# yubster4525/image_compression_2

Measured on AMD Instinct MI355X. Metric: images/sec encode+decode 256px, higher is better.
Workload: dtype f16 (synthesis) / split-bf16 (encoder); 1 GPU; batch=32 256x256 encode+8bit quantize+decode, SG3-T-256 generator; global_batch=32, per_gpu_batch=32, resolution=256, generator=stylegan3-t-256 (random init), encoder=HVAE_VGG_Encoder(img_resolution=1024), quantization_bits=8, parallelism=dp1 (batch-sharded, RCCL metric all_reduce)

## Files before the change

image_compression_2_amd/_native.py:

```python
from __future__ import annotations

import ctypes
import os
import sys
import threading

import torch

_HERE = os.path.dirname(os.path.abspath(__file__))
LIB_PATH = os.path.join(_HERE, "libic2ops.so")
if os.environ.get("IC2_DEV") == "1" and os.environ.get("IC2_DEV_LIB"):
    LIB_PATH = os.environ["IC2_DEV_LIB"]

F32, BF16, F16, BF16X3, F16X2 = 0, 1, 2, 3, 4
F16_IEEE = 5
ACT_LINEAR, ACT_LRELU = 0, 1
NHWC, NCHW, NHWC16 = 0, 1, 2

_P = ctypes.c_void_p
_I = ctypes.c_int
_I64 = ctypes.c_int64
_F = ctypes.c_float

_SIGS = {
    "ic2_abi_version": [],
    "ic2_dev_mode": [],
    "ic2_conv_plan": [_I, _I, _I, _I, _I, _I, _I, _I, _I, _I, _I, _I],
    "ic2_quantize_uniform": [_P, _I64, _I, _P, _P, _P],
    "ic2_quantize_codebook_argmin": [_P, _I64, _P, _I, _P, _P, _P, _P],
    "ic2_codebook_lookup": [_P, _I64, _P, _I, _P, _P, _P],
    "ic2_code_record": [_P, _I, _I, _I, _P, _I64, _P, _P],
    "ic2_gumbel_softmax_quantize": [_P, _I64, _P, _I, _P, _F, _I, ctypes.c_uint64, ctypes.c_uint64, _P, _P, _P, _P,
                                    _P],
    "ic2_gumbel_softmax_quantize_dseed": [_P, _I64, _P, _I, _P, _F, _I, _P, ctypes.c_uint64, _P, _P, _P, _P, _P],
    "ic2_bias_act": [_P, _P, _P, _I, _I64, _I64, _I64, _I, _F, _F, _F, _P],
    "ic2_upfirdn2d": [_P, _P, _I, _I64, _I, _I, _I, _I, _P, _I, _I, _I, _I, _I, _I, _I, _I, _I, _I, _I, _I, _F, _P],
    "ic2_filtered_lrelu": [_P, _P, _I, _I64, _I64, _I, _I, _I, _I, _P, _I, _P, _I, _P, _I, _I, _I, _I, _I, _I, _F, _F,
                           _F, _I, _P],
    "ic2_flrelu_nhwc": [_P, _P, _I, _I, _I, _I, _I, _I, _I, _I, _P, _I, _P, _I, _P, _I, _I, _I, _I, _I, _I, _F, _F, _F,
                        _I, _P, _P],
    "ic2_flrelu_nhwc16": [_P, _P, _I, _I, _I, _I, _I, _I, _I, _I, _P, _I, _P, _I, _P, _I, _I, _I, _I, _I, _I, _F, _F,
                          _F, _I, _P, _P],
    "ic2_fc": [_P, _I64, _P, _P, _P, _I, _I, _I, _F, _F, _I, _F, _F, _P],
    "ic2_pack_weight": [_P, _I, _I, _I, _I, _I, _I, _I, _F, _P, _I, _P, _P],
    "ic2_modconv_prep": [_P, _P, _I, _I, _I, _I, _I, _I, _F, _F, _P, _P, _P, _P],
    "ic2_modconv_prep_batched": [_P, _I64, _I, _I, _I, _P, _P],
    "ic2_conv_igemm": [_P, _P, _P, _I, _I, _I, _I, _I, _I, _I, _I, _I, _I, _I, _I, _I, _P, _P, _I, _F, _F, _F, _F, _I,
                       _P],
    "ic2_conv_igemm_ws_bytes": [_I, _I, _I, _I, _I, _I, _I, _I, _I],
    "ic2_conv_igemm_ws": [_P, _P, _P, _I, _I, _I, _I, _I, _I, _I, _I, _I, _I, _I, _I, _I, _P, _P, _I, _F, _F, _F, _F,
                          _I, _P, _I64, _P],
    "ic2_pack_weight_wino": [_P, _I, _I, _I, _I, _I, _F, _P, _I, _P],
    "ic2_pack_weight_adjoint": [_P, _I, _I, _I, _I, _I, _I, _P, _I, _P],
    "ic2_conv_wino": [_P, _P, _P, _I, _I, _I, _I, _I, _I, _I, _I, _I, _I, _I, _P, _P, _I, _F, _F, _F, _F, _I, _P],
    "ic2_conv_wino_plan": [_I, _I, _I, _I, _I, _I],
    "ic2_conv_wino_preferred": [_I, _I, _I, _I, _I, _I, _I, _I, _I],
    "ic2_conv_wino_stamps": [_P, _I64],
    "ic2_synth_input_features": [_P, _P, _P, _P, _I, _I, _I, _I, _F, _F, _P, _I, _P],
    "ic2_nchw_to_nhwc": [_P, _P, _I, _I, _I, _I, _I, _I, _P, _P],
    "ic2_from_rgb_conv": [_P, _I, _P, _I, _P, _P, _I, _I, _I, _I, _P],
    "ic2_from_rgb_conv_x3": [_P, _I, _P, _I, _P, _P, _I, _I, _I, _I, _P],
    "ic2_from_rgb_conv_f16": [_P, _I, _P, _I, _P, _P, _I, _I, _I, _I, _P],
    "ic2_nhwc_to_nchw": [_P, _I, _P, _I, _I, _I, _I, _I, _P],
    "ic2_group_norm_stats_floats": [_I, _I, _I],
    "ic2_group_norm_stats": [_P, _I, _I, _I, _I, _I, _I, _F, _P, _P],
    "ic2_gn_lrelu_pool": [_P, _P, _I, _I, _I, _I, _I, _I, _I, _I, _P, _P, _P, _F, _I, _P],
    "ic2_global_avg_pool_floats": [_I, _I, _I, _I],
    "ic2_global_avg_pool": [_P, _I, _I, _I, _I, _I, _P, _P],
    "ic2_reparameterize": [_P, _P, _I, _I, _I, _I, _I, _P, _P, _P, _P],
    "ic2_uint8_sse_scratch_doubles": [_I64],
    "ic2_uint8_sse": [_P, _P, _I64, _I64, _P, _P, _P],
    "ic2_resize_bilinear": [_P, _P, _I64, _I, _I, _I, _I, _P],
    "ic2_rc_bound": [_I64, _I64],
    "ic2_rc_encode": [_P, _I64, _I, _I, _I, _P, _I64, _P, _I],
    "ic2_rc_decode": [_P, _P, _I64, _I, _I, _I, _P, _I],
    "ic2_conv_wgrad_ws_floats": [_I, _I, _I, _I, _I, _I, _I, _I],
    "ic2_conv_wgrad": [_P, _P, _P, _I, _I, _I, _I, _I, _I, _I, _I, _I, _P, _I64, _P],
    "ic2_conv_wgrad_oihw": [_P, _P, _P, _I, _I, _I, _I, _I, _I, _I, _I, _I, _I, _I, _P, _I64, _P],
    "ic2_gn_lrelu_pool_bwd_floats": [_I, _I, _I, _I, _I],
    "ic2_gn_lrelu_pool_bwd": [_P, _P, _P, _I, _I, _I, _I, _I, _I, _I, _I, _I, _P, _P, _P, _F, _I, _P, _P, _P, _I64,
                              _P],
    "ic2_gn_lrelu_pool_bwd_db": [_P, _P, _P, _I, _I, _I, _I, _I, _I, _I, _I, _I, _P, _P, _P, _F, _I, _P, _P, _P, _P,
                                 _I64, _P],
    "ic2_gap_bwd": [_P, _P, _I, _I, _I, _I, _I, _P],
    "ic2_flrelu_bwd_ydot_floats": [_I, _I, _I, _I, _I],
    "ic2_flrelu_bwd_nhwc_ex": [_P, _I, _P, _I, _P, _I, _I, _I, _I, _I, _I, _I, _P, _I, _P, _I, _I, _I, _I, _I, _I, _I,
                               _F, _F, _F, _I, _P, _P, _P, _I64, _P],
    "ic2_scale_bwd_part_floats": [_I, _I, _I],
    "ic2_colsum_div": [_P, _I, _I, _I, _P, _P, _P],
    "ic2_scale_bwd_nhwc": [_P, _P, _P, _P, _I, _I, _I, _I, _P, _I64, _P],
    "ic2_scale_nhwc": [_P, _P, _P, _I, _I, _I, _I, _P],
    "ic2_conv3x3_gn_stats_floats": [_I, _I, _I, _I, _I, _I, _I, _I, _I, _I],
    "ic2_conv3x3_gn_fwd": [_P, _P, _P, _I, _I, _I, _I, _I, _I, _I, _I, _I, _I, _P, _I, _F, _P, _I64, _P, _I64, _I,
                           _P],
    "ic2_conv3x3_gn_fwd_scaled": [_P, _P, _P, _I, _I, _I, _I, _I, _I, _I, _I, _I, _I, _P, _F, _I, _F, _P, _I64, _P,
                                  _I64, _I, _P],
    "ic2_conv3x3_gnin_supported": [_I, _I, _I, _I, _I, _I, _I, _I, _I],
    "ic2_conv3x3_gn_fuses": [_I, _I, _I, _I, _I, _I, _I, _I, _I, _I, _I, _I],
    "ic2_gn_affine_table": [_P, _P, _P, _I, _I, _I, _I, _P, _P],
    "ic2_conv3x3_gnin_gn_fwd": [_P, _P, _F, _P, _P, _I, _I, _I, _I, _I, _I, _I, _I, _I, _I, _P, _I, _F, _P, _I64, _P,
                                _I64, _I, _P],
    "ic2_flrelu_bwd_nhwc": [_P, _I, _P, _I, _P, _I, _I, _I, _I, _I, _I, _P, _I, _P, _I, _I, _I, _I, _I, _I, _I, _F, _F,
                            _F, _I, _P],
}
_RESTYPE = {"ic2_conv_plan": ctypes.c_char_p, "ic2_conv_wino_plan": ctypes.c_char_p, "ic2_conv_igemm_ws_bytes": _I64, "ic2_group_norm_stats_floats": _I64, "ic2_global_avg_pool_floats": _I64,
            "ic2_uint8_sse_scratch_doubles": _I64, "ic2_rc_bound": _I64, "ic2_conv_wgrad_ws_floats": _I64,
            "ic2_gn_lrelu_pool_bwd_floats": _I64, "ic2_conv3x3_gn_stats_floats": _I64,
            "ic2_flrelu_bwd_ydot_floats": _I64, "ic2_scale_bwd_part_floats": _I64}

_lib = None
_lock = threading.Lock()


class NativeUnavailable(RuntimeError):
    pass


def load():
    global _lib
    if _lib is not None:
        return _lib
    with _lock:
        if _lib is not None:
            return _lib
        if not os.path.exists(LIB_PATH):
            raise NativeUnavailable(
                f"{LIB_PATH} is missing: build it with `python -m image_compression_2_amd.build_native` "
                "(there is no CPU fallback for the product path)")
        lib = ctypes.CDLL(LIB_PATH)
        lib.ic2_last_error.restype = ctypes.c_char_p
        lib.ic2_last_error.argtypes = []
        for name, args in _SIGS.items():
            fn = getattr(lib, name)
            fn.argtypes = args
            fn.restype = _RESTYPE.get(name, _I)
        _lib = lib
    return _lib


def exported_symbols():
    return ["ic2_last_error"] + list(_SIGS)


def call(name, *args):
    lib = load()
    rc = getattr(lib, name)(*args)
    if rc != 0:
        msg = lib.ic2_last_error().decode(errors="replace")
        raise RuntimeError(f"{name} failed (code {rc}): {msg}")
    return rc


def query(name, *args):
    return getattr(load(), name)(*args)


def conv_plan(dtype, out_dtype, out_layout, n, h, w, cin_p, cout_p, cout_valid, kh, kw, pad):
    return query("ic2_conv_plan", dtype, out_dtype, out_layout, n, h, w, cin_p, cout_p, cout_valid, kh, kw,
                 pad).decode()


def conv_igemm(x, w, y, dtype, out_dtype, n, h, w_, cin_p, cout_p, cout_valid, kh, kw, pad, ho, wo, oscale, bias,
               act, slope, act_gain, clamp, out_mul, out_layout, stream, device):
    nbytes = int(query("ic2_conv_igemm_ws_bytes", dtype, n, h, w_, cin_p, cout_p, kh, kw, pad))
    ws = torch.empty([max(nbytes, 16) // 4], dtype=torch.float32, device=device) if nbytes > 0 else None
    return call("ic2_conv_igemm_ws", x, w, y, dtype, out_dtype, n, h, w_, cin_p, cout_p, cout_valid, kh, kw, pad, ho,
                wo, oscale, bias, act, slope, act_gain, clamp, out_mul, out_layout, ptr(ws), nbytes, stream)


def wino_preferred(dtype, n, h, w, cin_p, cout_p, kh, kw, pad):
    return bool(query("ic2_conv_wino_preferred", dtype, n, h, w, cin_p, cout_p, kh, kw, pad))


def wino_plan(n, h, w, cin_p, cout_p, pad):
    return query("ic2_conv_wino_plan", n, h, w, cin_p, cout_p, pad).decode()


def conv_wino(x, u, y, dtype, out_dtype, n, h, w_, cin_p, cout_p, cout_valid, pad, ho, wo, oscale, bias, act, slope,
              act_gain, clamp, out_mul, out_layout, stream):
    return call("ic2_conv_wino", x, u, y, dtype, out_dtype, n, h, w_, cin_p, cout_p, cout_valid, pad, ho, wo, oscale,
                bias, act, slope, act_gain, clamp, out_mul, out_layout, stream)


_flops_hook = None


def note_flops(alg_flops):
    if _flops_hook is not None:
        _flops_hook(alg_flops)


def knob(name, default):
    v = os.environ.get(name)
    if os.environ.get("IC2_DEV") != "1":
        if v is not None:
            print(f"[ic2] {name}={v} ignored: development knobs need IC2_DEV=1", file=sys.stderr)
        return default
    return default if v is None else type(default)(v)


def require_gpu(*tensors):
    for t in tensors:
        if t is None:
            continue
        if not t.is_cuda:
            raise RuntimeError("image_compression_2_amd runs on ROCm devices only (got a CPU tensor); "
                               "the CPU restatement lives in oracle/ and is test infrastructure")
        if not t.is_contiguous():
            raise RuntimeError("expected a contiguous tensor")


class AutogradUnsupported(RuntimeError):
    pass


def grad_inputs(tensors=(), modules=()):
    if not torch.is_grad_enabled():
        return []
    req = [t for t in tensors if isinstance(t, torch.Tensor) and t.requires_grad]
    return req + [p for m in modules for p in m.parameters() if p.requires_grad]


class _RefuseBackward(torch.autograd.Function):

    @staticmethod
    def forward(ctx, what, n_out, *args):
        ctx.what = what
        return tuple(a.detach() for a in args[:n_out])

    @staticmethod
    def backward(ctx, *grads):
        raise AutogradUnsupported(
            f"{ctx.what}: backward through the HIP path is not implemented for this module (training, SURVEY.md "
            "8(f) #3; the reference trains only the encoder, through a frozen generator).  Freeze the module with "
            ".requires_grad_(False) or detach its inputs")


def refuse_backward(what, outputs, tensors=(), modules=()):
    req = grad_inputs(tensors, modules)
    if not req:
        return outputs
    single = isinstance(outputs, torch.Tensor)
    outs = [outputs] if single else list(outputs)
    fl = [i for i, o in enumerate(outs) if isinstance(o, torch.Tensor) and o.is_floating_point()]
# ... 64 lines not shown
```

image_compression_2_amd/csrc/conv_common.h:

```cpp
#pragma once
#include "common.h"

namespace ic2 {

typedef __attribute__((ext_vector_type(8))) __bf16 bf16x8;
typedef __attribute__((ext_vector_type(8))) _Float16 f16x8;
typedef __attribute__((ext_vector_type(4))) float f32x4;

template <bool F16>
__device__ __forceinline__ f32x4 mfma32(bf16x8 a, bf16x8 b, f32x4 c) {
  if constexpr (F16)
    return __builtin_amdgcn_mfma_f32_16x16x32_f16(__builtin_bit_cast(f16x8, a), __builtin_bit_cast(f16x8, b), c, 0, 0, 0);
  else
    return __builtin_amdgcn_mfma_f32_16x16x32_bf16(a, b, c, 0, 0, 0);
}
__host__ __device__ inline bool is16(int dtype) { return dtype == IC2_BF16 || dtype == IC2_F16; }

struct IgemmArgs {
  const void* x;
  const void* w;
  void* y;
  const float* oscale;
  const float* bias;
  float* ws;
  int n, h, w_, cin_p, cout_p, cout_valid, kh, kw, pad, ho, wo;
  int M;
  int K;
  int nq;
  int tiles_o;
  int nblocks;
  int group;
  int korder;
  int o_base;
  int tile_base;
  int act;
  float slope, act_gain, clamp, out_mul;
  int out_layout, out_dtype;
  double* gn_part;
  int gn_groups, gn_c;
  const float* in_gn;
  float in_slope;
  int x_pix, x_hb32;
  int wx_twp, wx_th, wx_ns, wx_hp, wx_nh, wx_tx, wx_ty;
  int out_ieee;
};
__device__ __forceinline__ int ig_xb32(const IgemmArgs& a, int b) { return b >= a.x_hb32 ? b - a.x_hb32 : b; }

__device__ __forceinline__ float4 ig_load_oscale(const IgemmArgs& a, int nn, int ob) {
  return a.oscale && ob < a.cout_p ? *reinterpret_cast<const float4*>(a.oscale + (int64_t)nn * a.cout_p + ob)
                                   : make_float4(1.f, 1.f, 1.f, 1.f);
}
__device__ __forceinline__ float4 ig_load_bias(const IgemmArgs& a, int ob) {
  return a.bias && ob < a.cout_p ? *reinterpret_cast<const float4*>(a.bias + ob) : make_float4(0.f, 0.f, 0.f, 0.f);
}
__device__ __forceinline__ void ig_preloads_done() { __builtin_amdgcn_s_waitcnt(0x0F70); }

__device__ __forceinline__ void ig_store4v(const IgemmArgs& a, int p, int nn, int pix, int ob, const float (&acc)[4],
                                           float4 sc, float4 bi, float (*vout)[4] = nullptr) {
  const float scv[4] = {sc.x, sc.y, sc.z, sc.w}, biv[4] = {bi.x, bi.y, bi.z, bi.w};
  float v[4];
#pragma unroll
  for (int r = 0; r < 4; ++r) {
    float t = acc[r] * scv[r] + biv[r];
    if (a.act) t = lrelu_gain_clamp(t, a.slope, a.act_gain, a.clamp);
    v[r] = t * a.out_mul;
  }
  if (vout != nullptr) {
#pragma unroll
    for (int r = 0; r < 4; ++r) (*vout)[r] = v[r];
  }
  if (a.out_layout != IC2_LAYOUT_NCHW) {
    const int64_t e = a.out_layout == IC2_LAYOUT_NHWC
                          ? (int64_t)p * a.cout_p + ob
                          : (((int64_t)nn * (a.cout_p >> 4) + (ob >> 4)) * ((int64_t)a.ho * a.wo) + pix) * 16 + (ob & 15);
    if (a.out_dtype == IC2_BF16) {
      uint2 pk;
      pk.x = (uint32_t)f2bf(v[0]) | ((uint32_t)f2bf(v[1]) << 16);
      pk.y = (uint32_t)f2bf(v[2]) | ((uint32_t)f2bf(v[3]) << 16);
      *reinterpret_cast<uint2*>(reinterpret_cast<bf16_t*>(a.y) + e) = pk;
    } else if (a.out_dtype == IC2_F16) {
      typedef _Float16 h2 __attribute__((ext_vector_type(2)));
      float s_[4];
#pragma unroll
      for (int r = 0; r < 4; ++r) s_[r] = a.out_ieee ? v[r] : __builtin_amdgcn_fmed3f(v[r], -65504.f, 65504.f);
      const h2 q0 = h2{(_Float16)s_[0], (_Float16)s_[1]}, q1 = h2{(_Float16)s_[2], (_Float16)s_[3]};
      if (vout != nullptr) {
        (*vout)[0] = (float)q0.x; (*vout)[1] = (float)q0.y; (*vout)[2] = (float)q1.x; (*vout)[3] = (float)q1.y;
      }
      uint2 pk;
      pk.x = __builtin_bit_cast(uint32_t, q0);
      pk.y = __builtin_bit_cast(uint32_t, q1);
      *reinterpret_cast<uint2*>(reinterpret_cast<uint16_t*>(a.y) + e) = pk;
    } else {
      *reinterpret_cast<float4*>(reinterpret_cast<float*>(a.y) + e) = make_float4(v[0], v[1], v[2], v[3]);
    }
  } else {
    float* yo = reinterpret_cast<float*>(a.y);
    const int hw = a.ho * a.wo;
#pragma unroll
    for (int r = 0; r < 4; ++r)
      if (ob + r < a.cout_valid) yo[((int64_t)nn * a.cout_valid + ob + r) * hw + pix] = v[r];
  }
}
__device__ __forceinline__ void ig_store4(const IgemmArgs& a, int p, int nn, int pix, int ob, const float (&acc)[4]) {
  ig_store4v(a, p, nn, pix, ob, acc, ig_load_oscale(a, nn, ob), ig_load_bias(a, ob));
}

__device__ __forceinline__ int xcd_remap(int b, int nblocks) {
  const int xcd = b & 7, loc = b >> 3;
  const int q8 = nblocks >> 3, r8 = nblocks & 7;
  return (xcd < r8 ? xcd * (q8 + 1) : r8 * (q8 + 1) + (xcd - r8) * q8) + loc;
}

constexpr uint32_t kOob = 0x7ffffff0u;
constexpr int kRsrcWord3 = 0x00020000;

}
```

image_compression_2_amd/csrc/flrelu.h:

```cpp
#pragma once
#include "common.h"

namespace ic2 {

struct FlrArgs {
  const void* x;
  void* y;
  const float* bias;
  const float* post_scale;
  int64_t xsn, xsy, xsx, xsc;
  int64_t xcb;
  int64_t ysn, ysy, ysx, ysc;
  int c, c_p;
  int in_h, in_w, out_h, out_w;
  int py0, px0;
  int tiles_x, tiles_y, cblocks, nimg;
  int order;
  int out_f16;
  float slope, lim;
  float gdg[12];
  float gu[24];
  float gd[12];
  float guh[24];
  float gdgl[12];
};

void f16_round_taps(const float* exact, float* out, int n, int stride_groups);

int flrelu_mfma_launch(FlrArgs a, int in_f16, int up, int down, int tu, int td, int delta, int n, hipStream_t s);

}
```

image_compression_2_amd/csrc/flrelu.hip:

```cpp
#include "flrelu.h"

#include <cmath>

#include <cstdlib>
#include <type_traits>

namespace ic2 {

typedef float f2v __attribute__((ext_vector_type(2)));

template <int U, int D, int TU, int TD, int TOY, int TOX>
struct FlrGeom {
  static constexpr int RAY = (TOY - 1) * D + TD;
  static constexpr int RAX = (TOX - 1) * D + TD;
  static constexpr int NINY = (RAY + TU - 2) / U + 1;
  static constexpr int NINX = (RAX + TU - 2) / U + 1;
  static constexpr int NINXP = NINX | 1;
};

template <typename T, bool CHLAST>
__device__ __forceinline__ f2v load2(const T* p, int64_t sc, bool ok, bool ok2);
template <> __device__ __forceinline__ f2v load2<float, true>(const float* p, int64_t, bool ok, bool) {
  const float2 v = *reinterpret_cast<const float2*>(ok ? (const void*)p : zero_line());
  return f2v{v.x, v.y};
// ... 201 lines not shown
  return 2;
}

template <typename TI, typename TO, bool CHLAST, int U, int D, int TU, int TD, int DL>
static int launch_geom(const FlrArgs& a, int geom, int grid, hipStream_t s) {
#define IC2_FLR_LAUNCH(TY, TX, CPB, NT)                                                                            \
  hipLaunchKernelGGL((flrelu_kernel<TI, TO, CHLAST, U, D, TU, TD, DL, TY, TX, CPB, NT>), dim3(grid), dim3(NT), 0, s, a)
  constexpr bool tuned = CHLAST && std::is_same<TI, bf16_t>::value;
  if constexpr (tuned) {
    switch (geom) {
      case 1: IC2_FLR_LAUNCH(16, 8, 16, 256); return IC2_OK;
      case 2: IC2_FLR_LAUNCH(16, 16, 16, 256); return IC2_OK;
      case 3: IC2_FLR_LAUNCH(8, 16, 16, 256); return IC2_OK;
      case 4: IC2_FLR_LAUNCH(12, 16, 16, 256); return IC2_OK;
      case 5: IC2_FLR_LAUNCH(16, 16, 8, 128); return IC2_OK;
      default: break;
    }
  }
  if (geom != 0) return IC2_E_UNSUPPORTED;
  IC2_FLR_LAUNCH(24, 8, 16, 256);
  return IC2_OK;
#undef IC2_FLR_LAUNCH
}

template <typename TI, typename TO, bool CHLAST, int U, int D, int TU, int TD>
static int launch_delta(const FlrArgs& a, int delta, int geom, int grid, hipStream_t s) {
  switch (delta) {
    case 0: return launch_geom<TI, TO, CHLAST, U, D, TU, TD, 0>(a, geom, grid, s);
    case 1: return launch_geom<TI, TO, CHLAST, U, D, TU, TD, 1>(a, geom, grid, s);
    case 2: if constexpr (U > 2) return launch_geom<TI, TO, CHLAST, U, D, TU, TD, 2>(a, geom, grid, s); break;
    case 3: if constexpr (U > 3) return launch_geom<TI, TO, CHLAST, U, D, TU, TD, 3>(a, geom, grid, s); break;
  }
  return IC2_E_UNSUPPORTED;
}

template <typename TI, typename TO, bool CHLAST>
static int launch_cfg(const FlrArgs& a, int up, int down, int tu, int td, int delta, int geom, int grid,
                      hipStream_t s) {
  if (up == 2 && down == 2 && tu == 12 && td == 12)
    return launch_delta<TI, TO, CHLAST, 2, 2, 12, 12>(a, delta, geom, grid, s);
  if (up == 4 && down == 2 && tu == 24 && td == 12)
    return launch_delta<TI, TO, CHLAST, 4, 2, 24, 12>(a, delta, geom, grid, s);
  return IC2_E_UNSUPPORTED;
}

static float f16_nearest(float v) { return (float)(_Float16)v; }
static float f16_step(float r, bool up) {
  uint16_t b = __builtin_bit_cast(uint16_t, (_Float16)r);
  const bool neg = b & 0x8000u;
  if ((b & 0x7fffu) == 0) return up ? 5.96046448e-8f : -5.96046448e-8f;
  b = (up != neg) ? b + 1 : b - 1;
  return (float)__builtin_bit_cast(_Float16, b);
}
void f16_round_taps(const float* exact, float* out, int n, int stride_groups) {
  for (int t = 0; t < n; ++t) out[t] = f16_nearest(exact[t]);
  for (int g = 0; g < stride_groups; ++g) {
    for (int it = 0; it < n; ++it) {
      double e = 0.0;
      for (int t = g; t < n; t += stride_groups) e += (double)out[t] - (double)exact[t];
      double best = std::fabs(e);
      int bi = -1;
      float bc = 0.f;
      for (int t = g; t < n; t += stride_groups) {
        if (exact[t] == 0.f) continue;
        for (int dir = 0; dir < 2; ++dir) {
          const float c = f16_step(out[t], dir == 0);
          if (((double)c - exact[t]) * ((double)out[t] - exact[t]) > 0.0) continue;
          const double e2 = std::fabs(e - (double)out[t] + (double)c);
          if (e2 < best) { best = e2; bi = t; bc = c; }
        }
      }
      if (bi < 0) break;
      out[bi] = bc;
    }
  }
}

static int flrelu_common(const void* x, void* y, int dtype_in, int dtype_out, bool chlast, int n, int c, int c_p,
                         int in_h, int in_w, int out_h, int out_w, const float* fu, int fu_taps, const float* fd,
                         int fd_taps, const float* b, int up, int down, int px0, int px1, int py0, int py1,
                         float gain, float slope, float clamp, int flip, const float* post_scale, void* stream,
                         const char* name, bool in_blocked = false) {
  IC2_CHECK_ARG(x && y, "%s: null pointer", name);
  IC2_CHECK_ARG(n > 0 && c > 0 && in_h > 0 && in_w > 0 && up >= 1 && down >= 1, "%s: bad geometry", name);
  IC2_CHECK_ARG(fu_taps >= 1 && fd_taps >= 1 && fu_taps <= 24 && fd_taps <= 12, "%s: unsupported taps", name);
  const int ew = (in_w * up + (px0 + px1) - (fu_taps - 1) - (fd_taps - 1) + (down - 1)) / down;
  const int eh = (in_h * up + (py0 + py1) - (fu_taps - 1) - (fd_taps - 1) + (down - 1)) / down;
  IC2_CHECK_ARG(out_h == eh && out_w == ew, "%s: output %dx%d, expected %dx%d", name, out_h, out_w, eh, ew);
  IC2_CHECK_ARG(out_h > 0 && out_w > 0, "%s: empty output", name);
  const int dx = ((px0 % up) + up) % up, dy = ((py0 % up) + up) % up;
  if (dx != dy) {
    set_error("%s: px0 and py0 differ mod up", name);
    return IC2_E_UNSUPPORTED;
  }
  if (!(slope >= 0.f && slope <= 1.f && gain > 0.f)) {
    set_error("%s: fused path needs 0 <= slope <= 1 and gain > 0", name);
    return IC2_E_UNSUPPORTED;
  }
  FlrArgs a;
  a.x = x; a.y = y; a.bias = b; a.post_scale = post_scale;
  a.xcb = 16;
  if (in_blocked) {
    a.xsc = 1; a.xsx = 16; a.xsy = (int64_t)in_w * 16; a.xsn = (int64_t)in_h * in_w * c_p;
    a.xcb = (int64_t)in_h * in_w * 16;
    a.ysc = 1; a.ysx = c_p; a.ysy = (int64_t)out_w * c_p; a.ysn = (int64_t)out_h * out_w * c_p;
  } else if (chlast) {
    a.xsc = 1; a.xsx = c_p; a.xsy = (int64_t)in_w * c_p; a.xsn = (int64_t)in_h * in_w * c_p;
    a.ysc = 1; a.ysx = c_p; a.ysy = (int64_t)out_w * c_p; a.ysn = (int64_t)out_h * out_w * c_p;
  } else {
    a.xsx = 1; a.xsy = in_w; a.xsc = (int64_t)in_h * in_w; a.xsn = (int64_t)c * in_h * in_w;
    a.ysx = 1; a.ysy = out_w; a.ysc = (int64_t)out_h * out_w; a.ysn = (int64_t)c * out_h * out_w;
  }
  a.c = chlast ? c_p : c;
  a.c_p = c_p;
  a.in_h = in_h; a.in_w = in_w; a.out_h = out_h; a.out_w = out_w;
  a.py0 = py0; a.px0 = px0;
  hipStream_t s = as_stream(stream);
  static const bool use_mfma = knob("IC2_FLR_MFMA", 1) != 0;
  const bool mfma_ok = chlast && (dtype_in == IC2_BF16 || dtype_in == IC2_F16) &&
                       (dtype_out == IC2_BF16 || dtype_out == IC2_F16) && b == nullptr && dx == dy;
  a.out_f16 = dtype_out == IC2_F16;
  if ((use_mfma || dtype_in == IC2_F16) && mfma_ok) {
    float gu[24] = {}, gd[12] = {}, gdg[12] = {};
    for (int t = 0; t < fu_taps; ++t) gu[t] = (fu ? (flip ? fu[t] : fu[fu_taps - 1 - t]) : 1.f) * (float)up;
    for (int t = 0; t < fd_taps; ++t) gd[t] = fd ? (flip ? fd[t] : fd[fd_taps - 1 - t]) : 1.f;
    for (int t = 0; t < fd_taps; ++t) gdg[t] = gd[t] * gain;
    for (int t = 0; t < 24; ++t) a.gu[t] = 0.f;
    for (int t = 0; t < 12; ++t) a.gd[t] = a.gdg[t] = 0.f;
    f16_round_taps(gu, a.gu, fu_taps, up);
    f16_round_taps(gd, a.gd, fd_taps, 1);
    f16_round_taps(gdg, a.gdg, fd_taps, 1);
    a.slope = slope;
    a.lim = clamp >= 0.f ? clamp / gain : INFINITY;
    for (int t = 0; t < 24; ++t) a.guh[t] = 0.f;
    for (int t = 0; t < 12; ++t) a.gdgl[t] = 0.f;
    if (clamp >= 0.f) {
      float guh[24] = {}, gdgl[12] = {};
      for (int t = 0; t < fu_taps; ++t) guh[t] = gu[t] / a.lim;
      for (int t = 0; t < fd_taps; ++t) gdgl[t] = gdg[t] * a.lim;
      f16_round_taps(guh, a.guh, fu_taps, up);
      f16_round_taps(gdgl, a.gdgl, fd_taps, 1);
    }
    if (flrelu_mfma_launch(a, dtype_in == IC2_F16, up, down, fu_taps, fd_taps, dx, n, s) == IC2_OK) {
      IC2_CHECK_LAUNCH(name);
      return IC2_OK;
    }
  }
  if (in_blocked) {
    set_error("%s: channel-blocked input needs the MFMA instance (f16/bf16 in, bf16/f16 out, no bias, up 2/4 with 6*up "
              "taps, down 2 / 12 taps)", name);
    return IC2_E_UNSUPPORTED;
  }
  if (dtype_in == IC2_F16) {
    set_error("%s: f16 input needs the MFMA instance (NHWC, bf16/f16 out, no bias, up 2/4 with 6*up taps, down 2 / 12 taps)",
              name);
    return IC2_E_UNSUPPORTED;
  }
  const int geom = flr_pick(chlast && dtype_in == IC2_BF16 && dtype_out == IC2_BF16, up);
  const FlrGeomSel fv = kFlrGeoms[geom];
  a.tiles_x = (int)ceil_div(out_w, fv.tox);
  a.tiles_y = (int)ceil_div(out_h, fv.toy);
  a.cblocks = (int)ceil_div(a.c, fv.cpb);
  a.nimg = n;
  a.slope = slope;
  a.lim = clamp >= 0.f ? clamp / gain : INFINITY;
  for (int t = 0; t < 24; ++t) a.gu[t] = 0.f;
  for (int t = 0; t < 12; ++t) a.gd[t] = 0.f;
  for (int t = 0; t < fu_taps; ++t) a.gu[t] = (fu ? (flip ? fu[t] : fu[fu_taps - 1 - t]) : 1.f) * (float)up;
  for (int t = 0; t < fd_taps; ++t) a.gd[t] = fd ? (flip ? fd[t] : fd[fd_taps - 1 - t]) : 1.f;
  for (int t = 0; t < 12; ++t) a.gdg[t] = a.gd[t] * gain;
  const int64_t grid = (int64_t)n * a.tiles_y * a.tiles_x * a.cblocks;
  IC2_CHECK_ARG(grid < (1LL << 31), "%s: grid too large", name);
  int rc;
  if (dtype_in == IC2_BF16 && dtype_out == IC2_BF16)
    rc = chlast ? launch_cfg<bf16_t, bf16_t, true>(a, up, down, fu_taps, fd_taps, dx, geom, (int)grid, s)
                : launch_cfg<bf16_t, bf16_t, false>(a, up, down, fu_taps, fd_taps, dx, geom, (int)grid, s);
  else if (dtype_in == IC2_F32 && dtype_out == IC2_F32)
    rc = chlast ? launch_cfg<float, float, true>(a, up, down, fu_taps, fd_taps, dx, geom, (int)grid, s)
                : launch_cfg<float, float, false>(a, up, down, fu_taps, fd_taps, dx, geom, (int)grid, s);
  else {
    set_error("%s: unsupported dtype pair %d -> %d", name, dtype_in, dtype_out);
    return IC2_E_INVALID;
  }
  if (rc != IC2_OK) {
    set_error("%s: no fused instance for up=%d down=%d taps=%d/%d", name, up, down, fu_taps, fd_taps);
    return rc;
  }
  IC2_CHECK_LAUNCH(name);
  return IC2_OK;
}

}

using namespace ic2;

extern "C" int ic2_filtered_lrelu(const void* x, void* y, int dtype, int64_t n, int64_t c, int in_h, int in_w,
                                  int out_h, int out_w, const float* fu, int fu_taps, const float* fd, int fd_taps,
                                  const float* b, int up, int down, int px0, int px1, int py0, int py1, float gain,
                                  float slope, float clamp, int flip, void* stream) {
  IC2_CHECK_ARG(n < (1 << 30) && c < (1 << 30), "filtered_lrelu: sizes too large");
  return flrelu_common(x, y, dtype, dtype, false, (int)n, (int)c, (int)c, in_h, in_w, out_h, out_w, fu, fu_taps, fd,
                       fd_taps, b, up, down, px0, px1, py0, py1, gain, slope, clamp, flip, nullptr, stream,
                       "filtered_lrelu");
}

extern "C" int ic2_flrelu_nhwc(const void* x, void* y, int dtype_in, int dtype_out, int n, int c_p, int in_h,
                               int in_w, int out_h, int out_w, const float* fu, int fu_taps, const float* fd,
                               int fd_taps, const float* b, int up, int down, int px0, int px1, int py0, int py1,
                               float gain, float slope, float clamp, int flip, const float* post_scale,
                               void* stream) {
  IC2_CHECK_ARG(c_p % 16 == 0, "flrelu_nhwc: c_p must be a multiple of 16");
  return flrelu_common(x, y, dtype_in, dtype_out, true, n, c_p, c_p, in_h, in_w, out_h, out_w, fu, fu_taps, fd,
                       fd_taps, b, up, down, px0, px1, py0, py1, gain, slope, clamp, flip, post_scale, stream,
                       "flrelu_nhwc");
}

extern "C" int ic2_flrelu_nhwc16(const void* x, void* y, int dtype_in, int dtype_out, int n, int c_p, int in_h,
                                 int in_w, int out_h, int out_w, const float* fu, int fu_taps, const float* fd,
                                 int fd_taps, const float* b, int up, int down, int px0, int px1, int py0, int py1,
                                 float gain, float slope, float clamp, int flip, const float* post_scale,
                                 void* stream) {
  IC2_CHECK_ARG(c_p % 16 == 0, "flrelu_nhwc16: c_p must be a multiple of 16");
  IC2_CHECK_ARG(dtype_in == IC2_F16 || dtype_in == IC2_BF16, "flrelu_nhwc16: f16 or bf16 input");
  return flrelu_common(x, y, dtype_in, dtype_out, true, n, c_p, c_p, in_h, in_w, out_h, out_w, fu, fu_taps, fd,
                       fd_taps, b, up, down, px0, px1, py0, py1, gain, slope, clamp, flip, post_scale, stream,
                       "flrelu_nhwc16", true);
}
```

image_compression_2_amd/csrc/flrelu_mfma.h:

```cpp
#pragma once
#include "flrelu.h"

namespace ic2 {

typedef _Float16 fm_h2 __attribute__((ext_vector_type(2)));
typedef _Float16 fm_h4 __attribute__((ext_vector_type(4)));
typedef _Float16 fm_h8 __attribute__((ext_vector_type(8)));
typedef short fm_s4 __attribute__((ext_vector_type(4)));
typedef float fm_f4 __attribute__((ext_vector_type(4)));
typedef float fm_f2 __attribute__((ext_vector_type(2)));
typedef uint32_t v2u32_t __attribute__((ext_vector_type(2)));

constexpr int FM_TAPS = 276;
constexpr int FM_TAPS_CL = 476;
constexpr uint32_t FM_OOB = 0x7ffffff0u;


__device__ __forceinline__ fm_s4 fm_tr_read(const uint32_t* p) {
  return __builtin_amdgcn_ds_read_tr16_b64_v4i16((__attribute__((address_space(3))) fm_s4*)p);
}

__device__ __forceinline__ void fm_dma16(__amdgpu_buffer_rsrc_t rs, uint32_t voff, const uint32_t* lds_dst) {
  const uint32_t m0 = __builtin_amdgcn_readfirstlane(
      (uint32_t)(uintptr_t)(__attribute__((address_space(3))) const uint32_t*)lds_dst);
  asm volatile("s_nop 4\n\tbuffer_load_dwordx4 %0, %1, 0 offen lds" ::"v"(voff), "s"(rs), "{m0}"(m0) : "memory");
}

__device__ __forceinline__ uint32_t fm_h2u(float a, float b) {
  return __builtin_bit_cast(uint32_t, fm_h2{(_Float16)a, (_Float16)b});
}
__device__ __forceinline__ uint2 fm_pack4(float a, float b, float c, float d) {
  return make_uint2(fm_h2u(a, b), fm_h2u(c, d));
}
__device__ __forceinline__ fm_h4 fm_h4_of(uint2 u) { return __builtin_bit_cast(fm_h4, u); }
__device__ __forceinline__ fm_h8 fm_h8_of(uint2 lo, uint2 hi) {
  return __builtin_bit_cast(fm_h8, make_uint4(lo.x, lo.y, hi.x, hi.y));
}

__device__ __forceinline__ int fm_xcd_remap(int b, int nblocks) {
  const int xcd = b & 7, loc = b >> 3;
  const int q8 = nblocks >> 3, r8 = nblocks & 7;
  return (xcd < r8 ? xcd * (q8 + 1) : r8 * (q8 + 1) + (xcd - r8) * q8) + loc;
}

inline int fm_strip_segments(int64_t nstrips, int tiles_y, int resident, bool tune) {
  int64_t nseg = (2 * (int64_t)resident + nstrips - 1) / nstrips;
  nseg = nseg < 1 ? 1 : (nseg > tiles_y ? tiles_y : nseg);
  if (tune && tiles_y <= 40) {
    int64_t best = -1, pick = nseg;
    for (int64_t sg = nseg; sg <= tiles_y && sg <= nseg + 16; ++sg) {
      const int64_t len = (tiles_y + sg - 1) / sg, segs = (tiles_y + len - 1) / len;
      const int64_t cost = (nstrips * segs + resident - 1) / resident * (len + 1);
      if (best < 0 || cost < best) best = cost, pick = segs;
    }
    nseg = pick;
  }
  return (int)nseg;
}

}
```

image_compression_2_amd/csrc/flrelu_mfma.hip:

```cpp
#include "flrelu_mfma.h"

#include <algorithm>
#include <cstdlib>
#include <type_traits>

namespace ic2 {

template <int U>
struct FmGeom {
  static constexpr int TU = 6 * U, TD = 12;
  static constexpr int TO = 16;
  static constexpr int RA = (TO - 1) * 2 + TD;
  static constexpr int NIN = (RA + TU - 2) / U + 1;
  static constexpr int NB = (RA + 15) / 16;
  static constexpr int IN_PITCH = NIN * 8;
  static constexpr int IN_DW = (NIN * NIN * 2 + 63) / 64 * 256;
  static constexpr int V_PITCH = NIN * 8 + 2;
  static constexpr int V_DW = 16 * V_PITCH;
  static constexpr int D_XP = 10;
  static constexpr int D_PITCH = 16 * D_XP + 8;
  static constexpr int D_DW = 16 * D_PITCH;
  static constexpr int LDS_DW = IN_DW + V_DW + D_DW + FM_TAPS;
  static constexpr int VD_DW = V_DW > D_DW ? V_DW : D_DW;
  static constexpr int LDS_DW_ALIAS = IN_DW + VD_DW + FM_TAPS;
// ... 569 lines not shown
          for (int tt = 0; tt < NBX; ++tt) {
            uint2 p, m;
            if constexpr (ABL & 2) { p = make_uint2(fm_h2u(u[tt][0], u[tt][1]), fm_h2u(u[tt][2], u[tt][3])); m = p; }
            else fm_act_split(fm_h2u(u[tt][0], u[tt][1]), fm_h2u(u[tt][2], u[tt][3]), nslope2, p, m);
            q[tt] = fm_h8_of(p, m);
          }
          __builtin_amdgcn_sched_barrier(0);
#pragma unroll
          for (int bi = 0; bi < 3; ++bi)
#pragma unroll
            for (int ob = 0; ob < NOB; ++ob)
              d[ob] = __builtin_amdgcn_mfma_f32_16x16x32_f16(q[2 * ob + bi], gdq[bi],
                                                             bi == 0 ? fm_f4{0.f, 0.f, 0.f, 0.f} : d[ob], 0, 0, 0);
        } else {
          uint2 au[NBX];
#pragma unroll
          for (int tt = 0; tt < NBX; ++tt)
            au[tt] = fm_act_h4(fm_h2u(u[tt][0], u[tt][1]), fm_h2u(u[tt][2], u[tt][3]), slope2, nlim2, lim2);
          __builtin_amdgcn_sched_barrier(0);
#pragma unroll
          for (int ob = 0; ob < NOB; ++ob)
            d[ob] = __builtin_amdgcn_mfma_f32_16x16x32_f16(fm_h8_of(au[2 * ob], au[2 * ob + 1]), gdh01,
                                                           fm_f4{0.f, 0.f, 0.f, 0.f}, 0, 0, 0);
#pragma unroll
          for (int ob = 0; ob < NOB; ++ob)
            d[ob] = __builtin_amdgcn_mfma_f32_16x16x32_f16(fm_h8_of(au[2 * ob + 2], make_uint2(0u, 0u)), gdh2, d[ob],
                                                           0, 0, 0);
        }
        __builtin_amdgcn_sched_barrier(0);
#pragma unroll
        for (int ob = 0; ob < NOB; ++ob)
          *reinterpret_cast<uint2*>(d_img + row * G::D_PITCH + (16 * ob + li) * G::D_XP + 2 * g) =
              fm_pack4(d[ob][0], d[ob][1], d[ob][2], d[ob][3]);
      }
      if constexpr (!(ABL & 1)) __syncthreads();
      if constexpr (!(ABL & 32)) {
        fm_s4 da[OCW];
#pragma unroll
        for (int i = 0; i < OCW; ++i)
          da[i] = fm_tr_read(d_img + (4 * g + tq) * G::D_PITCH + (wave + NW * i) * G::D_XP + 2 * tp);
        __builtin_amdgcn_sched_barrier(0);
#pragma unroll
        for (int i = 0; i < OCW; ++i)
          acc[i] = __builtin_amdgcn_mfma_f32_16x16x16f16(__builtin_bit_cast(fm_h4, da[i]), gdv[b], acc[i], 0, 0, 0);
        __builtin_amdgcn_sched_barrier(0);
      }
    }

    const float ps[4] = {psv.x, psv.y, psv.z, psv.w};
    const __amdgpu_buffer_rsrc_t ors = __builtin_amdgcn_make_buffer_rsrc(
        (void*)(yout + (int64_t)n * a.out_h * a.out_w * a.c_p + c0), 0, FM_OOB, 0x00020000);
    const int gy = oy0 + li;
#pragma unroll
    for (int i = 0; i < OCW; ++i) {
      const int gx = ox0 + wave + NW * i;
      uint32_t off = (gy < a.out_h && gx < a.out_w) ? (uint32_t)(((gy * a.out_w + gx) * a.c_p + 4 * g) * 2) : FM_OOB;
      if constexpr ((ABL & 64) != 0)
        off = (gy < a.out_h && gx < a.out_w)
                  ? (uint32_t)((((c0 >> 4) * a.out_h + gy) * a.out_w + gx) * 32 + 8 * g) - (uint32_t)(c0 * 2)
                  : FM_OOB;
      const uint2 v = fm_out4(a.out_f16, acc[i][0] * ps[0], acc[i][1] * ps[1], acc[i][2] * ps[2], acc[i][3] * ps[3]);
      if constexpr (!(ABL & 8))
        __builtin_amdgcn_raw_buffer_store_b64(__builtin_bit_cast(v2u32_t, v), ors, off, 0, 0);
    }
  }
}

template <int U>
struct FmGeom3 {
  using G2 = FmGeom2<U, 32>;
  static constexpr int NINX = G2::NINX;
  static constexpr int S = 16 / U;
  static constexpr int NG = U + 1;
  static constexpr int IN_PITCH = NINX * 8;
  static constexpr int GCH = S * NINX * 2;
  static constexpr int NGI = (GCH + 63) / 64;
  static constexpr int GRP_DW = NGI * 256;
  static constexpr int RING_DW = NG * GRP_DW;
  static constexpr int LDS_DW = RING_DW + G2::V_DW + G2::DT_DW + 16;
  static_assert(U * S == 16 && NINX % 2 == 1, "geometry");
  static_assert((NG - 1) * GRP_DW + (S - 1) * IN_PITCH + 8 * 8 * ((NINX + 7) / 8) <= RING_DW, "ring bounds");
};

#ifndef IC2_FM3_ABL
#define IC2_FM3_ABL 0
#endif
#ifndef FM3_EARLY
#define FM3_EARLY 1
#endif
#ifndef FM3_DEFER_ST
#define FM3_DEFER_ST 0
#endif
template <int U, int DELTA, int NW, bool CL>
__global__ void __launch_bounds__(64 * NW, 32 / NW) flrelu_mfma3_kernel(FlrArgs a, int nitems, int nseg, int seg_len) {
  constexpr int TOX = 32, NT = 64 * NW, RR = 16 / NW, OCW = TOX / NW;
  using G2 = FmGeom2<U, TOX>;
  using G = FmGeom3<U>;
  constexpr int NINX = G::NINX, NBX = G2::NBX, NOB = G2::NOB, S = G::S, NG = G::NG;
  __shared__ __attribute__((aligned(16))) uint32_t lds[G::LDS_DW];
  uint32_t* const ring = lds;
  uint32_t* const v_img = lds + G::RING_DW;
  uint32_t* const d_img = v_img + G2::V_DW;
  float* const taps = reinterpret_cast<float*>(d_img);
  uint32_t* const ps_lds = d_img + G2::DT_DW;

  const int tid = threadIdx.x;
  const int lane = tid & 63;
  const int wave = __builtin_amdgcn_readfirstlane(tid >> 6);
  const int g = lane >> 4, li = lane & 15;
  const int tq = li >> 2, tp = li & 3;
  const int qoff = (4 * g + tq) / S, roff = (4 * g + tq) % S;

  for (int i = tid; i < FM_TAPS_CL; i += NT) {
    float v = 0.f;
    if (i >= 48 && i < 72) v = a.gu[i - 48];
    else if (i >= 148 && i < 160) v = a.gd[i - 148];
    else if (i >= 228 && i < 240) v = a.gdg[i - 228];
    else if (i >= 328 && i < 352) v = a.guh[i - 328];
    else if (i >= 428 && i < 440) v = a.gdgl[i - 428];
    taps[i] = v;
  }

  const int slot = fm_xcd_remap(blockIdx.x, gridDim.x);
  const uint16_t* xin = reinterpret_cast<const uint16_t*>(a.x);
  auto item_geom = [&](int w, int& n, int& ox0, int& c0, int& t0, int& nt) {
    const int cb = w % a.cblocks;
    w /= a.cblocks;
    const int seg = w % nseg;
    w /= nseg;
    const int tx = w % a.tiles_x;
    n = w / a.tiles_x;
    ox0 = tx * TOX;
    c0 = cb * 16;
    t0 = seg * seg_len;
    nt = min(seg_len, a.tiles_y - t0);
  };
  const int xsy = (int)a.xsy, xsx = (int)a.xsx;
  const int my_dma = wave < G::NGI ? (G::NGI - 1 - wave) / NW + 1 : 0;
  static_assert((G::NGI + NW - 1) / NW <= 2, "ring group DMA per wave");
  auto load_group = [&](int n, int iy0, int sx0, int c0, int q) __attribute__((always_inline)) {
    const __amdgpu_buffer_rsrc_t rs = __builtin_amdgcn_make_buffer_rsrc(
        (void*)(xin + n * a.xsn + (c0 >> 4) * a.xcb), 0, FM_OOB, 0x00020000);
    uint32_t* const dst = ring + (q % NG) * G::GRP_DW;
    int ln = lane;
    asm volatile("" : "+v"(ln));
#pragma unroll
    for (int i = 0; i < (G::NGI + NW - 1) / NW; ++i) {
      const int k = wave + NW * i;
      if (k < G::NGI) {
        const int e = k * 64 + ln;
        const int pix = e >> 1;
        const int row = pix / NINX, x = pix - row * NINX;
        const int iy = iy0 + q * S + row, ix = sx0 + x;
        const bool ok = e < G::GCH && (unsigned)iy < (unsigned)a.in_h && (unsigned)ix < (unsigned)a.in_w;
        const uint32_t off = ok ? (uint32_t)((iy * xsy + ix * xsx + (e & 1) * 8) * 2) : FM_OOB;
        fm_dma16(rs, off, dst + k * 256);
      }
    }
  };
  auto load_item = [&](int w) __attribute__((always_inline)) {
    int n, ox0, c0, t0, nt;
    item_geom(w, n, ox0, c0, t0, nt);
    const int iy0 = (32 * t0 + DELTA - a.py0) / U, sx0 = (ox0 * 2 - a.px0 + DELTA) / U;
#pragma unroll
    for (int q = 0; q < NG; ++q) load_group(n, iy0, sx0, c0, q);
    if (a.post_scale != nullptr && wave == NW - 1 && lane < 4) {
      const __amdgpu_buffer_rsrc_t prs = __builtin_amdgcn_make_buffer_rsrc(
          (void*)(a.post_scale + (int64_t)n * a.c_p + c0), 0, 64, 0x00020000);
      fm_dma16(prs, lane * 16, ps_lds);
    }
  };
  if (slot < nitems) load_item(slot);
  __syncthreads();

  fm_h4 gmy, gmx[NBX];
  {
    float v[4];
#pragma unroll
    for (int j = 0; j < 4; ++j) v[j] = taps[48 + U * (4 * g + j) + DELTA - li];
    gmy = fm_h4_of(fm_pack4(v[0], v[1], v[2], v[3]));
  }
#pragma unroll
  for (int t = 0; t < NBX; ++t) {
    const int w0 = fm_win<U, DELTA, NINX>(16 * t);
    float v[4];
#pragma unroll
    for (int j = 0; j < 4; ++j) v[j] = taps[(CL ? 328 : 48) + U * (w0 + 4 * g + j) + DELTA - (16 * t + li)];
    gmx[t] = fm_h4_of(fm_pack4(v[0], v[1], v[2], v[3]));
  }
  fm_h8 gdh01, gdh2, gdq[3];
  {
    auto tap = [&](int blk, int j) { return taps[(CL ? 428 : 228) + 16 * blk + 4 * g + j - 2 * li]; };
    float v[8];
#pragma unroll
    for (int j = 0; j < 4; ++j) {
      v[j] = tap(0, j);
      v[4 + j] = tap(1, j);
    }
    gdh01 = fm_h8_of(fm_pack4(v[0], v[1], v[2], v[3]), fm_pack4(v[4], v[5], v[6], v[7]));
#pragma unroll
    for (int j = 0; j < 4; ++j) {
      v[j] = tap(2, j);
      v[4 + j] = 0.f;
    }
    gdh2 = fm_h8_of(fm_pack4(v[0], v[1], v[2], v[3]), fm_pack4(v[4], v[5], v[6], v[7]));
#pragma unroll
    for (int bi = 0; bi < 3; ++bi) {
#pragma unroll
      for (int j = 0; j < 4; ++j) {
        v[j] = tap(bi, j);
        v[4 + j] = -tap(bi, j);
      }
      gdq[bi] = fm_h8_of(fm_pack4(v[0], v[1], v[2], v[3]), fm_pack4(v[4], v[5], v[6], v[7]));
    }
  }
  fm_h4 gdv[3];
#pragma unroll
  for (int b = 0; b < 3; ++b) {
    float v[4];
#pragma unroll
    for (int j = 0; j < 4; ++j) v[j] = taps[148 + 16 * b + 4 * g + j - 2 * li];
    gdv[b] = fm_h4_of(fm_pack4(v[0], v[1], v[2], v[3]));
  }
  const float slope = a.slope, lim = CL ? 1.f : a.lim;
  const uint32_t slope2 = fm_h2u(slope, slope), lim2 = fm_h2u(lim, lim), nlim2 = fm_h2u(-lim, -lim);
  const uint32_t nslope2 = fm_h2u(-slope, -slope);
  bf16_t* yout = reinterpret_cast<bf16_t*>(a.y);
  __syncthreads();

  bool first = true;
  for (int w = slot; w < nitems; w += gridDim.x) {
    int n, ox0, c0, t0, nt;
    item_geom(w, n, ox0, c0, t0, nt);
    const int iy0 = (32 * t0 + DELTA - a.py0) / U, sx0 = (ox0 * 2 - a.px0 + DELTA) / U;
    const bool has_next = w + (int)gridDim.x < nitems;
    if (first) asm volatile("s_waitcnt vmcnt(0)" ::: "memory");
    else asm volatile("s_waitcnt vmcnt(%0)" ::"n"(OCW) : "memory");
    first = false;
    __syncthreads();
    float4 psv = make_float4(1.f, 1.f, 1.f, 1.f);
    if (a.post_scale) psv = *reinterpret_cast<const float4*>(ps_lds + 4 * g);
    const float ps[4] = {psv.x, psv.y, psv.z, psv.w};
    const __amdgpu_buffer_rsrc_t ors = __builtin_amdgcn_make_buffer_rsrc(
        (void*)(yout + (int64_t)n * a.out_h * a.out_w * a.c_p + c0), 0, FM_OOB, 0x00020000);
    const int kend = 2 * nt;

    fm_f4 acc_a[OCW], acc_b[OCW];
    auto store_tile = [&](int tt) __attribute__((always_inline)) {
      const int gy = 16 * (t0 + tt) + li;
#pragma unroll
      for (int i = 0; i < OCW; ++i) {
        const int gx = ox0 + wave + NW * i;
        const uint32_t off =
            (gy < a.out_h && gx < a.out_w) ? (uint32_t)(((gy * a.out_w + gx) * a.c_p + 4 * g) * 2) : FM_OOB;
        const uint2 v = fm_out4(a.out_f16, acc_a[i][0] * ps[0], acc_a[i][1] * ps[1], acc_a[i][2] * ps[2], acc_a[i][3] * ps[3]);
        __builtin_amdgcn_raw_buffer_store_b64(__builtin_bit_cast(v2u32_t, v), ors, (IC2_FM3_ABL & 64) ? FM_OOB : off, 0, 0);
      }
    };
    auto block = [&](int k, auto mode_c) __attribute__((always_inline)) {
      constexpr int MODE = decltype(mode_c)::value;
      if constexpr (!(IC2_FM3_ABL & 8)) {
        constexpr int NC = (NINX + NW - 1) / NW;
        const int q = k + qoff;
        const uint32_t* rowp = ring + (q % NG) * G::GRP_DW + roff * G::IN_PITCH + 2 * tp + wave * 8;
        fm_s4 xa[NC];
        fm_f4 vt[NC];
#pragma unroll
        for (int i = 0; i < NC; ++i) xa[i] = fm_tr_read(rowp + i * NW * 8);
        __builtin_amdgcn_sched_barrier(0);
#pragma unroll
        for (int i = 0; i < NC; ++i)
          vt[i] = __builtin_amdgcn_mfma_f32_16x16x16f16(__builtin_bit_cast(fm_h4, xa[i]), gmy,
                                                        fm_f4{0.f, 0.f, 0.f, 0.f}, 0, 0, 0);
        __builtin_amdgcn_sched_barrier(0);
        uint32_t* const vp = v_img + li * G2::V_PITCH + 2 * g + wave * 8;
#pragma unroll
        for (int i = 0; i < NC; ++i)
          if (i < NC - 1 || wave + NW * i < NINX)
            *reinterpret_cast<uint2*>(vp + i * NW * 8) = fm_pack4(vt[i][0], vt[i][1], vt[i][2], vt[i][3]);
      }
      if constexpr (!(IC2_FM3_ABL & 32)) __syncthreads();
      if (k == kend && has_next) load_item(w + gridDim.x);
      const bool dma = !(IC2_FM3_ABL & 2) && k + 2 <= kend;
      if (FM3_EARLY && dma) load_group(n, iy0, sx0, c0, k + U + 1);
      if constexpr (FM3_DEFER_ST && MODE == 1) {
        if (k >= 3) store_tile((k - 3) >> 1);
      }
#pragma unroll
      for (int rr = 0; rr < ((IC2_FM3_ABL & 4) ? 0 : RR); ++rr) {
        const int row = wave + NW * rr;
        fm_s4 vb[NBX];
#pragma unroll
        for (int tt = 0; tt < NBX; ++tt) {
          const int w0 = fm_win<U, DELTA, NINX>(16 * tt);
          vb[tt] = fm_tr_read(v_img + row * G2::V_PITCH + (w0 + 4 * g + tq) * 8 + 2 * tp);
        }
        __builtin_amdgcn_sched_barrier(0);
        fm_f4 u[NBX];
#pragma unroll
        for (int tt = 0; tt < NBX; ++tt)
          u[tt] = __builtin_amdgcn_mfma_f32_16x16x16f16(gmx[tt], __builtin_bit_cast(fm_h4, vb[tt]),
                                                        fm_f4{0.f, 0.f, 0.f, 0.f}, 0, 0, 0);
        __builtin_amdgcn_sched_barrier(0);
        fm_f4 d[NOB];
        if constexpr (CL) {
          fm_h8 qv[NBX];
#pragma unroll
          for (int tt = 0; tt < NBX; ++tt) {
            uint2 p, m;
            fm_act_split(fm_h2u(u[tt][0], u[tt][1]), fm_h2u(u[tt][2], u[tt][3]), nslope2, p, m);
            qv[tt] = fm_h8_of(p, m);
          }
          __builtin_amdgcn_sched_barrier(0);
#pragma unroll
          for (int bi = 0; bi < 3; ++bi)
#pragma unroll
            for (int ob = 0; ob < NOB; ++ob)
              d[ob] = __builtin_amdgcn_mfma_f32_16x16x32_f16(qv[2 * ob + bi], gdq[bi],
                                                             bi == 0 ? fm_f4{0.f, 0.f, 0.f, 0.f} : d[ob], 0, 0, 0);
        } else {
          uint2 au[NBX];
#pragma unroll
          for (int tt = 0; tt < NBX; ++tt)
            au[tt] = fm_act_h4(fm_h2u(u[tt][0], u[tt][1]), fm_h2u(u[tt][2], u[tt][3]), slope2, nlim2, lim2);
          __builtin_amdgcn_sched_barrier(0);
#pragma unroll
          for (int ob = 0; ob < NOB; ++ob)
            d[ob] = __builtin_amdgcn_mfma_f32_16x16x32_f16(fm_h8_of(au[2 * ob], au[2 * ob + 1]), gdh01,
                                                           fm_f4{0.f, 0.f, 0.f, 0.f}, 0, 0, 0);
#pragma unroll
          for (int ob = 0; ob < NOB; ++ob)
            d[ob] = __builtin_amdgcn_mfma_f32_16x16x32_f16(fm_h8_of(au[2 * ob + 2], make_uint2(0u, 0u)), gdh2, d[ob],
                                                           0, 0, 0);
        }
        __builtin_amdgcn_sched_barrier(0);
#pragma unroll
        for (int ob = 0; ob < NOB; ++ob)
          *reinterpret_cast<uint2*>(d_img + row * G2::D_PITCH + (16 * ob + li) * G2::D_XP + 2 * g) =
              fm_pack4(d[ob][0], d[ob][1], d[ob][2], d[ob][3]);
      }
      if (!(IC2_FM3_ABL & 1) && k >= 1 && k < kend) {
        const bool st = (MODE == 1 && k >= 3) || (FM3_DEFER_ST && MODE == 2 && k >= 4);
        const int nd = FM3_EARLY && dma ? my_dma : 0;
        if (nd == 0) {
          if (st) asm volatile("s_waitcnt vmcnt(%0)" ::"n"(OCW) : "memory");
          else asm volatile("s_waitcnt vmcnt(0)" ::: "memory");
        } else if (nd == 1) {
          if (st) asm volatile("s_waitcnt vmcnt(%0)" ::"n"(OCW + 1) : "memory");
          else asm volatile("s_waitcnt vmcnt(1)" ::: "memory");
        } else {
          if (st) asm volatile("s_waitcnt vmcnt(%0)" ::"n"(OCW + 2) : "memory");
          else asm volatile("s_waitcnt vmcnt(2)" ::: "memory");
        }
      }
      if constexpr (!(IC2_FM3_ABL & 32)) __syncthreads();
      if (!FM3_EARLY && dma) load_group(n, iy0, sx0, c0, k + U + 1);
      if constexpr (!(IC2_FM3_ABL & 16)) {
        fm_s4 da[OCW];
#pragma unroll
        for (int i = 0; i < OCW; ++i)
          da[i] = fm_tr_read(d_img + (4 * g + tq) * G2::D_PITCH + (wave + NW * i) * G2::D_XP + 2 * tp);
        __builtin_amdgcn_sched_barrier(0);
        if constexpr (MODE == 0) {
#pragma unroll
          for (int i = 0; i < OCW; ++i)
            acc_b[i] = __builtin_amdgcn_mfma_f32_16x16x16f16(__builtin_bit_cast(fm_h4, da[i]), gdv[0],
                                                             fm_f4{0.f, 0.f, 0.f, 0.f}, 0, 0, 0);
        } else if constexpr (MODE == 1) {
#pragma unroll
          for (int i = 0; i < OCW; ++i)
            acc_a[i] = __builtin_amdgcn_mfma_f32_16x16x16f16(__builtin_bit_cast(fm_h4, da[i]), gdv[1], acc_b[i], 0, 0, 0);
        } else {
#pragma unroll
          for (int i = 0; i < OCW; ++i)
            acc_a[i] = __builtin_amdgcn_mfma_f32_16x16x16f16(__builtin_bit_cast(fm_h4, da[i]), gdv[2], acc_a[i], 0, 0, 0);
          if (k < kend) {
#pragma unroll
            for (int i = 0; i < OCW; ++i)
              acc_b[i] = __builtin_amdgcn_mfma_f32_16x16x16f16(__builtin_bit_cast(fm_h4, da[i]), gdv[0],
                                                               fm_f4{0.f, 0.f, 0.f, 0.f}, 0, 0, 0);
          }
        }
        __builtin_amdgcn_sched_barrier(0);
      }
    };

    block(0, std::integral_constant<int, 0>{});
    for (int t = 0; t < nt; ++t) {
      block(2 * t + 1, std::integral_constant<int, 1>{});
      block(2 * t + 2, std::integral_constant<int, 2>{});
      if (!FM3_DEFER_ST || t == nt - 1) store_tile(t);
    }
  }
}

template <int U, int DELTA, bool CL>
static void fm3_launch_cl(FlrArgs a, int n, hipStream_t s) {
  constexpr int TOX = 32, NW = 8;
  a.tiles_x = (int)ceil_div(a.out_w, TOX);
  a.tiles_y = (int)ceil_div(a.out_h, 16);
  a.cblocks = a.c_p / 16;
  static int resident = 0;
  if (resident == 0) {
    int dev = 0, cus = 0, per_cu = 0;
    (void)hipGetDevice(&dev);
    (void)hipDeviceGetAttribute(&cus, hipDeviceAttributeMultiprocessorCount, dev);
    (void)hipOccupancyMaxActiveBlocksPerMultiprocessor(&per_cu, flrelu_mfma3_kernel<U, DELTA, NW, CL>, 64 * NW, 0);
    resident = (cus > 0 ? cus : 256) * (per_cu > 0 ? per_cu : 1);
  }
  static const int segs_mode = knob("IC2_FLR_SEGS", 1);
  const int64_t nstrips = (int64_t)n * a.tiles_x * a.cblocks;
  int nseg = fm_strip_segments(nstrips, a.tiles_y, resident, segs_mode == 1);
  const int seg_len = (int)ceil_div(a.tiles_y, nseg);
  nseg = (int)ceil_div(a.tiles_y, seg_len);
  const int nitems = (int)(nstrips * nseg);
  const int grid = nitems < resident ? nitems : resident;
  hipLaunchKernelGGL((flrelu_mfma3_kernel<U, DELTA, NW, CL>), dim3((unsigned)grid), dim3(64 * NW), 0, s, a, nitems,
                     nseg, seg_len);
}

template <int U, int DELTA, bool CL, int ABL>
static void fm2_launch_cl(FlrArgs a, int n, hipStream_t s) {
  constexpr int TOX = 32, NW = 8;
  a.tiles_x = (int)ceil_div(a.out_w, TOX);
  a.tiles_y = (int)ceil_div(a.out_h, 16);
  a.cblocks = a.c_p / 16;
  static const int order = knob("IC2_FLR_ORDER", 0);
  a.order = order;
  const int ntiles = n * a.tiles_y * a.tiles_x * a.cblocks;
  static int resident = 0;
  if (resident == 0) {
    int dev = 0, cus = 0, per_cu = 0;
    (void)hipGetDevice(&dev);
    (void)hipDeviceGetAttribute(&cus, hipDeviceAttributeMultiprocessorCount, dev);
    (void)hipOccupancyMaxActiveBlocksPerMultiprocessor(&per_cu, flrelu_mfma2_kernel<U, DELTA, TOX, NW, CL, ABL>, 64 * NW, 0);
    resident = (cus > 0 ? cus : 256) * (per_cu > 0 ? per_cu : 1);
  }
  const int grid = ntiles < resident ? ntiles : resident;
  hipLaunchKernelGGL((flrelu_mfma2_kernel<U, DELTA, TOX, NW, CL, ABL>), dim3((unsigned)grid), dim3(64 * NW), 0, s, a, ntiles);
}

template <int U, int DELTA>
static void fm2_launch(FlrArgs a, int n, hipStream_t s) {
  static const bool split = knob("IC2_FLR_CLSPLIT", 1) != 0;
  static const bool strip = knob("IC2_FLR_STRIP", 1) != 0;
  const bool cl = split && a.lim >= 0.0625f && a.lim <= 4096.f;
  if (strip) {
    if (cl) fm3_launch_cl<U, DELTA, true>(a, n, s);
    else fm3_launch_cl<U, DELTA, false>(a, n, s);
  } else if (cl) {
    fm2_launch_cl<U, DELTA, true, 0>(a, n, s);
  } else {
    fm2_launch_cl<U, DELTA, false, 0>(a, n, s);
  }
}

template <int U, int DELTA, bool IN_F16, bool ALIAS, int NW>
static void fm_launch_alias(const FlrArgs& a, int ntiles, hipStream_t s) {
  static int resident = 0;
  if (resident == 0) {
    int dev = 0, cus = 0, per_cu = 0;
    (void)hipGetDevice(&dev);
    (void)hipDeviceGetAttribute(&cus, hipDeviceAttributeMultiprocessorCount, dev);
    (void)hipOccupancyMaxActiveBlocksPerMultiprocessor(&per_cu, flrelu_mfma_kernel<U, DELTA, IN_F16, ALIAS, NW>, 64 * NW,
                                                       0);
    resident = (cus > 0 ? cus : 256) * (per_cu > 0 ? per_cu : 1);
  }
  const int grid = ntiles < resident ? ntiles : resident;
  hipLaunchKernelGGL((flrelu_mfma_kernel<U, DELTA, IN_F16, ALIAS, NW>), dim3((unsigned)grid), dim3(64 * NW), 0, s, a,
                     ntiles);
}

template <int U, int DELTA, bool IN_F16>
static void fm_launch_one(const FlrArgs& a, int ntiles, hipStream_t s) {
  fm_launch_alias<U, DELTA, IN_F16, false, 4>(a, ntiles, s);
}

template <bool IN_F16>
static void fm_launch(const FlrArgs& a, int up, int delta, int ntiles, hipStream_t s) {
  if (up == 2) {
    if (delta == 0) fm_launch_one<2, 0, IN_F16>(a, ntiles, s);
    else fm_launch_one<2, 1, IN_F16>(a, ntiles, s);
  } else {
    switch (delta) {
      case 0: fm_launch_one<4, 0, IN_F16>(a, ntiles, s); break;
      case 1: fm_launch_one<4, 1, IN_F16>(a, ntiles, s); break;
      case 2: fm_launch_one<4, 2, IN_F16>(a, ntiles, s); break;
      default: fm_launch_one<4, 3, IN_F16>(a, ntiles, s); break;
    }
  }
}

int flrelu_mfma_launch(FlrArgs a, int in_f16, int up, int down, int tu, int td, int delta, int n, hipStream_t s) {
  if (down != 2 || td != 12 || tu != 6 * up || (up != 2 && up != 4) || a.bias != nullptr || a.c_p % 16 != 0)
    return IC2_E_UNSUPPORTED;
  if ((int64_t)a.in_h * a.in_w * a.c_p * 2 >= (int64_t)FM_OOB) return IC2_E_UNSUPPORTED;
  if (a.xsc != 1 || a.xsx % 8 != 0) return IC2_E_UNSUPPORTED;
  if ((int64_t)a.out_h * a.out_w * a.c_p * 2 >= (int64_t)FM_OOB) return IC2_E_UNSUPPORTED;
  static const bool wide = knob("IC2_FLR_WIDE", 1) != 0;
  static const bool wide_all = knob("IC2_FLR_WIDE_ALL", 1) != 0;
  if (in_f16 && wide && (wide_all || ceil_div(a.out_w, 32) * 32 <= ceil_div(a.out_w, 16) * 16) &&
      (int64_t)n * ceil_div(a.out_h, 16) * ceil_div(a.out_w, 32) * (a.c_p / 16) < (1LL << 31)) {
    if (up == 2) {
      if (delta == 0) fm2_launch<2, 0>(a, n, s);
      else fm2_launch<2, 1>(a, n, s);
    } else {
      switch (delta) {
        case 0: fm2_launch<4, 0>(a, n, s); break;
        case 1: fm2_launch<4, 1>(a, n, s); break;
        case 2: fm2_launch<4, 2>(a, n, s); break;
        default: fm2_launch<4, 3>(a, n, s); break;
      }
    }
    return IC2_OK;
  }
  a.tiles_x = (int)ceil_div(a.out_w, 16);
  a.tiles_y = (int)ceil_div(a.out_h, 16);
  a.cblocks = a.c_p / 16;
  const int64_t grid = (int64_t)n * a.tiles_y * a.tiles_x * a.cblocks;
  if (grid >= (1LL << 31)) return IC2_E_UNSUPPORTED;
  if (in_f16) fm_launch<true>(a, up, delta, (int)grid, s);
  else fm_launch<false>(a, up, delta, (int)grid, s);
  return IC2_OK;
}

}
```

image_compression_2_amd/csrc/igemm.hip:

```cpp
#include "conv_common.h"

#include <cstdlib>

namespace ic2 {

template <bool BF16, int BO, int BP, int WGO, int WGP, int NSTAGE>
struct IgCfg {
  static constexpr int NW = WGO * WGP;
  static constexpr int ESZ = BF16 ? 2 : 4;
  static constexpr int EPC = 16 / ESZ;
  static constexpr int ROWB = 32 * ESZ;
  static constexpr int WB = BO * ROWB, XB = BP * ROWB;
  static constexpr int NIW_T = WB / 1024, NIX_T = XB / 1024;
  static constexpr int NIW = (NIW_T + NW - 1) / NW, NIX = (NIX_T + NW - 1) / NW;
  static constexpr int PER = NIW + NIX;
  static constexpr int TO = BO / WGO, TP = BP / WGP;
  static constexpr int I = TO / 16, J = TP / 16;
  static constexpr int STAGEB = WB + XB;
  __device__ static __forceinline__ int swz(int row) { return BF16 ? ((row >> 1) & 3) : ((row >> 1) & 7); }
  __device__ static __forceinline__ int off(int row, int ch) { return row * ROWB + ((ch ^ swz(row)) << 4); }
};

template <int I, int J>
__device__ __forceinline__ void ig_epilogue(const IgemmArgs& a, const f32x4 (&acc)[I][J], int obase, int pbase, int fr,
// ... 471 lines not shown
                      int ntiles = -1) {
  a.o_base = o_base;
  a.tiles_o = ((o_end < 0 ? a.cout_p : o_end) - o_base + G8<OG>::BO - 1) / G8<OG>::BO;
  a.nq = a.K / 64;
  a.nblocks = (int)(ceil_div(a.M, G8<OG>::BP) * a.tiles_o);
  a.tile_base = tile_base;
  const unsigned grid = (unsigned)(ntiles < 0 ? a.nblocks - tile_base : ntiles);
  if constexpr (OG == 2)
    hipLaunchKernelGGL(F16 ? igemm8_og2_f16_kernel : igemm8_og2_kernel, dim3(grid, splits), dim3(512), 0, s, a);
  else
    hipLaunchKernelGGL(F16 ? igemm8_og1_f16_kernel : igemm8_og1_kernel, dim3(grid, splits), dim3(512), 0, s, a);
}

template <int I, int J, int WGO, int WGP, int TW, int NS, bool HB = false>
struct H4 {
  static constexpr int BO = 16 * I * WGO, BP = 16 * J * WGP, TH = BP / TW;
  static constexpr int HW = TW + 2, HH = TH + 2, NH = HH * HW;
  static constexpr int NHI = (NH + 15) / 16;
  static constexpr int HPW = (NHI + 3) / 4;
  static constexpr int HALO_B = NHI * 1024;
  static constexpr int WS_B = BO * 64;
  static constexpr int NWI = (BO / 16 + 3) / 4;
  static constexpr int LDS_B = NS * WS_B + 2 * HALO_B + (HB ? 1024 : 0);
  static_assert(BP % TW == 0 && TW % 16 == 0, "pixel tile");
  static_assert((BO / 16) % 4 == 0 || BO == 96, "weight slab rows over the 4 waves");
  static_assert(HB || HPW <= 8, "halo DMA spread over the first 8 taps");
  static_assert(LDS_B <= 80 * 1024, "two workgroups per CU");
};
__device__ __forceinline__ int h4_off(int row, int chunk) { return row * 64 + ((chunk ^ (((row >> 2) & 1) << 1)) << 4); }

#ifndef IC2_HG4_ABL
#define IC2_HG4_ABL 0
#endif
#ifndef IC2_HG4_PAIR
#define IC2_HG4_PAIR 1
#endif

template <int I, int J, int WGO, int WGP, int TW, int NS, bool HB = false, bool F16 = false, int TPB = 1,
          bool GN = false, bool PAIR = false>
__device__ __forceinline__ void hg4_body(const IgemmArgs& a, int tiles_x, int tiles_y) {
  using G = H4<I, J, WGO, WGP, TW, NS, HB>;
  static_assert(!PAIR || (TPB == 2 && HB), "PAIR: two taps per barrier step with the halo burst");
  static_assert((G::BO / 16) % 4 == 0 || (TPB == 2 && NS == 4), "uneven weight DMAs need the L = 1 multi-tap loop");
  constexpr int LA = NS - 1;
  constexpr int NWI = G::NWI, HPW = G::HPW;
  __shared__ __attribute__((aligned(16))) char lds[G::LDS_B];
  char* const wsl = lds;
  char* const hal = lds + NS * G::WS_B;
  const int tid = threadIdx.x;
  const int lane = tid & 63;
  const int wid = __builtin_amdgcn_readfirstlane(tid >> 6);
  const int og = wid / WGP, pg = wid % WGP;
  const int fr = lane & 15, fh = lane >> 4;

  const int logical = xcd_remap(blockIdx.x, a.nblocks);
  const int o_tile = logical % a.tiles_o;
  int pt = logical / a.tiles_o;
  const int tx = pt % tiles_x;
  pt /= tiles_x;
  const int ty = pt % tiles_y;
  const int nn = pt / tiles_y;
  const int o0 = o_tile * G::BO;
  const int oy0 = ty * G::TH, ox0 = tx * TW;

  const char* __restrict__ xg = reinterpret_cast<const char*>(a.x);
  const char* __restrict__ wg = reinterpret_cast<const char*>(a.w);
  const int lrow = lane >> 2, pch = lane & 3;

  uint32_t w_off[NWI];
#pragma unroll
  for (int k = 0; k < NWI; ++k) {
    const int row = (wid + 4 * k) * 16 + lrow;
    const int o = o0 + row;
    w_off[k] = (row < G::BO && o < a.cout_p) ? (uint32_t)(o * a.K * 2 + ((pch ^ (((row >> 2) & 1) << 1)) << 4)) : kOob;
  }
  uint32_t h_off[HPW];
#pragma unroll
  for (int k = 0; k < HPW; ++k) {
    const int g = wid + 4 * k;
    const int hp = g * 16 + lrow;
    const int hy = hp / G::HW, hx = hp - (hp / G::HW) * G::HW;
    const int iy = oy0 - a.pad + hy, ix = ox0 - a.pad + hx;
    const bool ok = g < G::NHI && hp < G::NH && (unsigned)iy < (unsigned)a.h && (unsigned)ix < (unsigned)a.w_;
    h_off[k] = ok ? (uint32_t)((((nn * a.h + iy) * a.w_ + ix) * a.x_pix + ((pch ^ (((hp >> 2) & 1) << 1)) << 3)) * 2)
                  : kOob;
  }
  int brow[J];
#pragma unroll
  for (int j = 0; j < J; ++j) {
    const int pb = pg * J + j;
    brow[j] = (pb * 16 / TW) * G::HW + (pb * 16) % TW + fr;
  }
  const int obase = og * 16 * I;
  const bool live = o0 + obase < a.cout_p;
  const int CB = a.cin_p >> 5;
  const int nq = CB * 9;
  constexpr int SPB = PAIR ? 18 : 9;
  const int HBK = PAIR ? CB >> 1 : CB;
  auto step_of = [&](int t, int& hbk, int& cb, int& tap) {
    if constexpr (PAIR) {
      hbk = t / 18;
      const int r = t - hbk * 18;
      tap = r >> 1;
      cb = hbk + (r & 1) * (CB >> 1);
    } else {
      cb = t / 9;
      tap = t - cb * 9;
      hbk = cb;
    }
  };

  auto issue_w = [&](int t) {
    int hbk_, cb, tap;
    step_of(t, hbk_, cb, tap);
    const __amdgpu_buffer_rsrc_t rs = __builtin_amdgcn_make_buffer_rsrc(
        (void*)(wg + ((int64_t)tap * a.cin_p + cb * 32) * 2), 0, t < nq ? kOob : 0, kRsrcWord3);
    char* dst = wsl + (t % NS) * G::WS_B;
#pragma unroll
    for (int k = 0; k < NWI; ++k)
      if ((G::BO / 16) % 4 == 0 || wid + 4 * k < G::BO / 16)
        __builtin_amdgcn_raw_ptr_buffer_load_lds(
            rs, (__attribute__((address_space(3))) void*)(dst + (wid + 4 * k) * 1024), 16, w_off[k], 0, 0, 0);
  };
  auto issue_hb = [&](int cb) {
    const __amdgpu_buffer_rsrc_t rs =
        __builtin_amdgcn_make_buffer_rsrc((void*)(xg + (int64_t)ig_xb32(a, cb) * 64), 0, kOob, kRsrcWord3);
#pragma unroll
    for (int k = 0; k < HPW; ++k) {
      char* dst = wid + 4 * k < G::NHI ? hal + (cb & 1) * G::HALO_B + (wid + 4 * k) * 1024 : hal + 2 * G::HALO_B;
      __builtin_amdgcn_raw_ptr_buffer_load_lds(rs, (__attribute__((address_space(3))) void*)dst, 16, h_off[k], 0, 0, 0);
    }
  };
  auto issue_h1 = [&](int cb, int k) {
    const __amdgpu_buffer_rsrc_t rs =
        __builtin_amdgcn_make_buffer_rsrc((void*)(xg + (int64_t)ig_xb32(a, cb) * 64), 0, kOob, kRsrcWord3);
    __builtin_amdgcn_raw_ptr_buffer_load_lds(
        rs, (__attribute__((address_space(3))) void*)(hal + (cb & 1) * G::HALO_B + (wid + 4 * k) * 1024), 16, h_off[k],
        0, 0, 0);
  };

  f32x4 acc[I][J];
#pragma unroll
  for (int i = 0; i < I; ++i)
#pragma unroll
    for (int j = 0; j < J; ++j) acc[i][j] = f32x4{0.f, 0.f, 0.f, 0.f};

#pragma unroll
  for (int k = 0; k < HPW; ++k)
    if (wid + 4 * k < G::NHI) issue_h1(0, k);
  if constexpr (TPB > 1) {
    static_assert(HB && NS % TPB == 0 && NS >= 2 * TPB && (TPB == 2 || TPB == 3), "TPB: halo burst, ring of steps");
    constexpr int L = NS / TPB - 1;
    const int nst = (nq + TPB - 1) / TPB;
    auto burst_at = [&](int st) {
      const int t0 = TPB * st, cb0 = t0 / SPB;
      return t0 - cb0 * SPB < TPB && cb0 + 1 < HBK;
    };
#pragma unroll
    for (int t = 0; t < TPB * L; ++t) issue_w(t);
    asm volatile("s_waitcnt vmcnt(%0)" ::"n"((L - 1) * TPB * NWI) : "memory");
    bf16x8 af[TPB][I], bfr[TPB][J];
    for (int s = 0; s < nst; ++s) {
      if constexpr (!(IC2_HG4_ABL & 2)) __builtin_amdgcn_s_barrier();
      __builtin_amdgcn_sched_barrier(0);
      const int t0 = TPB * s;
      if (!(IC2_HG4_ABL & 16) || s == 0) {
#pragma unroll
        for (int u = 0; u < TPB; ++u) issue_w(t0 + u + TPB * L);
      }
      const bool burst = burst_at(s);
      if (burst) issue_hb(t0 / SPB + 1);
      __builtin_amdgcn_sched_barrier(0);
#pragma unroll
      for (int u = 0; u < TPB; ++u) {
        if ((IC2_HG4_ABL & 4) && s > 0) break;
        const int t = t0 + u;
        int hbk, cb, tap;
        step_of(t, hbk, cb, tap);
        const int sh = (tap / 3) * G::HW + tap % 3;
        const char* hb = hal + (hbk & 1) * G::HALO_B;
        const char* wl = wsl + (t % NS) * G::WS_B;
        if (!PAIR || u == 0) {
#pragma unroll
          for (int j = 0; j < J; ++j) bfr[u][j] = *reinterpret_cast<const bf16x8*>(hb + h4_off(brow[j] + sh, fh));
        }
#pragma unroll
        for (int i = 0; i < I; ++i) af[u][i] = *reinterpret_cast<const bf16x8*>(wl + h4_off(obase + i * 16 + fr, fh));
      }
      __builtin_amdgcn_sched_barrier(0);
      __builtin_amdgcn_s_setprio(1);
      if (live) {
#pragma unroll
        for (int u = 0; u < TPB; ++u) {
          if (u == 0 || t0 + u < nq) {
#pragma unroll
            for (int i = 0; i < I; ++i)
#pragma unroll
              for (int j = 0; j < J; ++j) {
                if constexpr (IC2_HG4_ABL & 8) asm volatile("" ::"v"(af[u][i]), "v"(bfr[PAIR ? 0 : u][j]));
                else acc[i][j] = mfma32<F16>(af[u][i], bfr[PAIR ? 0 : u][j], acc[i][j]);
              }
          }
        }
      }
      __builtin_amdgcn_s_setprio(0);
      __builtin_amdgcn_sched_barrier(0);
      const bool recent = burst || (L > 1 && s > 0 && burst_at(s - 1));
      if constexpr (!(IC2_HG4_ABL & 1)) {
        if (recent) asm volatile("s_waitcnt vmcnt(%0)" ::"n"((L - 1) * TPB * NWI + HPW) : "memory");
        else asm volatile("s_waitcnt vmcnt(%0)" ::"n"((L - 1) * TPB * NWI) : "memory");
      }
    }
  } else {
#pragma unroll
  for (int t = 0; t < LA; ++t) issue_w(t);
  asm volatile("s_waitcnt vmcnt(%0)" ::"n"((LA - 1) * NWI) : "memory");
  for (int t = 0; t < nq; ++t) {
    __builtin_amdgcn_s_barrier();
// ... 472 lines not shown
#pragma unroll
        for (int r = 0; r < GL; ++r)
#pragma unroll
          for (int off = 1; off < 16; off <<= 1) {
            gs[i][r] += __shfl_xor(gs[i][r], off, 64);
            gq[i][r] += __shfl_xor(gq[i][r], off, 64);
          }
      __syncthreads();
      float* red = reinterpret_cast<float*>(halo);
      if (fr == 0) {
#pragma unroll
        for (int i = 0; i < C::OB; ++i)
#pragma unroll
          for (int r = 0; r < GL; ++r) {
            const int g = (16 * i + 4 * fh) / CPG + r;
            red[wave * 32 + g] = gs[i][r];
            red[(8 + wave) * 32 + g] = gq[i][r];
          }
      }
      __syncthreads();
      if (tid < 32) {
        double sg = 0.0, qg = 0.0;
#pragma unroll
        for (int w8 = 0; w8 < 8; ++w8) {
          sg += (double)red[w8 * 32 + tid];
          qg += (double)red[(8 + w8) * 32 + tid];
        }
        double* o = a.gn_part + (((int64_t)nn * 32 + tid) * (tiles_x * tiles_y) + (ty * tiles_x + tx)) * 2;
        o[0] = sg;
        o[1] = qg;
      }
    }
  }
}

template <int CINP, int COUTP, bool GN = false, bool F16 = false>
static void launch_hconv(const IgemmArgs& a, hipStream_t s) {
  constexpr int TH = CINP > 64 ? 4 : 8;
  const int tiles_x = (int)ceil_div(a.wo, 32), tiles_y = (int)ceil_div(a.ho, TH);
  const int ntiles = a.n * tiles_x * tiles_y;
  static int resident = 0;
  if (resident == 0) {
    int dev = 0, cus = 0, per_cu = 0;
    (void)hipGetDevice(&dev);
    (void)hipDeviceGetAttribute(&cus, hipDeviceAttributeMultiprocessorCount, dev);
    (void)hipOccupancyMaxActiveBlocksPerMultiprocessor(&per_cu, hconv_kernel<CINP, COUTP, TH, GN, F16>, 512, 0);
    resident = (cus > 0 ? cus : 256) * (per_cu > 0 ? per_cu : 1);
  }
  const int grid = ntiles < resident ? ntiles : resident;
  hipLaunchKernelGGL((hconv_kernel<CINP, COUTP, TH, GN, F16>), dim3((unsigned)grid), dim3(512), 0, s, a, tiles_x,
                     tiles_y, ntiles);
}

static bool hconv_eligible(int dtype, int64_t M, int cin_p, int cout_p, int kh, int kw) {
  static const bool on = knob("IC2_HCONV", 1) != 0;
  return on && is16(dtype) && kh == 3 && kw == 3 && (cin_p == 32 || cin_p == 64 || cin_p == 96) &&
         (cout_p == 32 || cout_p == 64) && M >= 65536;
}

template <bool F16>
__device__ __forceinline__ float h2f(uint32_t bits16) {
  if constexpr (F16) return (float)__builtin_bit_cast(_Float16, (uint16_t)bits16);
  else return __uint_as_float(bits16 << 16);
}

template <int L, int CV, bool F16 = false>
__global__ void __launch_bounds__(256) torgb_kernel(IgemmArgs a) {
  const int tid = blockIdx.x * 256 + threadIdx.x;
  const int sub = threadIdx.x & (L - 1);
  const int hw = a.ho * a.wo;
  float wv[CV][16];
  const uint16_t* wg = reinterpret_cast<const uint16_t*>(a.w);
#pragma unroll
  for (int o = 0; o < CV; ++o)
#pragma unroll
    for (int k = 0; k < 16; ++k) wv[o][k] = h2f<F16>(wg[(int64_t)o * a.cin_p + sub * 16 + k]);
  float bi[CV];
#pragma unroll
  for (int o = 0; o < CV; ++o) bi[o] = a.bias ? a.bias[o] : 0.f;
  const uint16_t* xg = reinterpret_cast<const uint16_t*>(a.x);
  float* yo = reinterpret_cast<float*>(a.y);
  const int stride = gridDim.x * (256 / L);
  for (int p = tid / L; p < a.M; p += stride) {
    const uint4* src = reinterpret_cast<const uint4*>(xg + (int64_t)p * a.cin_p + sub * 16);
    const uint4 u0 = src[0], u1 = src[1];
    const uint32_t w32[8] = {u0.x, u0.y, u0.z, u0.w, u1.x, u1.y, u1.z, u1.w};
    float acc[CV];
#pragma unroll
    for (int o = 0; o < CV; ++o) acc[o] = 0.f;
#pragma unroll
    for (int k = 0; k < 8; ++k) {
      const float lo = h2f<F16>(w32[k] & 0xffffu), hi = h2f<F16>(w32[k] >> 16);
#pragma unroll
      for (int o = 0; o < CV; ++o) acc[o] = fmaf(wv[o][2 * k + 1], hi, fmaf(wv[o][2 * k], lo, acc[o]));
    }
#pragma unroll
    for (int m = 1; m < L; m <<= 1)
#pragma unroll
      for (int o = 0; o < CV; ++o) acc[o] += __shfl_xor(acc[o], m, 64);
    if (sub == 0) {
      const int nn = p / hw, pix = p - nn * hw;
#pragma unroll
      for (int o = 0; o < CV; ++o) {
        if (o >= a.cout_valid) break;
        float t = acc[o] * (a.oscale ? a.oscale[(int64_t)nn * a.cout_p + o] : 1.f) + bi[o];
        if (a.act) t = lrelu_gain_clamp(t, a.slope, a.act_gain, a.clamp);
        yo[((int64_t)nn * a.cout_valid + o) * hw + pix] = t * a.out_mul;
      }
    }
  }
}

static bool torgb_eligible(int dtype, int cin_p, int cout_valid, int kh, int kw, int pad, int out_layout,
                           int out_dtype) {
  static const bool on = knob("IC2_TORGB", 1) != 0;
  return on && is16(dtype) && kh == 1 && kw == 1 && pad == 0 && cout_valid <= 4 && out_layout == IC2_LAYOUT_NCHW &&
         out_dtype == IC2_F32 && (cin_p == 32 || cin_p == 64 || cin_p == 128);
}

template <bool F16>
static void launch_torgb(const IgemmArgs& a, hipStream_t s) {
  const int L = a.cin_p / 16;
  const int64_t need = ceil_div((int64_t)a.M * L, 256);
  const unsigned grid = (unsigned)(need < 8192 ? need : 8192);
  if (L == 2) hipLaunchKernelGGL((torgb_kernel<2, 4, F16>), dim3(grid), dim3(256), 0, s, a);
  else if (L == 4) hipLaunchKernelGGL((torgb_kernel<4, 4, F16>), dim3(grid), dim3(256), 0, s, a);
  else hipLaunchKernelGGL((torgb_kernel<8, 4, F16>), dim3(grid), dim3(256), 0, s, a);
}

static int g8_tail_first(int64_t M, int cout_p) {
  const int64_t g6 = ceil_div(M, 256) * ((cout_p + 255) / 256);
  return (int)(g6 - g6 % 256);
}
template <bool F16>
static void launch_igemm16(const IgemmArgs& a, hipStream_t s, const IgPlan& pl, bool split384, int cout_p) {
  switch (pl.tile) {
    case 6:
      if (pl.tail) {
        const int full = g8_tail_first(a.M, a.cout_p);
        launch_g8<2, F16>(a, s, 0, -1, 1, 0, full);
        launch_g8<2, F16>(a, s, 0, -1, 2, full, -1);
      } else {
        launch_g8<2, F16>(a, s, 0, -1, pl.splits);
      }
      break;
    case 7:
      if (split384) {
        launch_g8<2, F16>(a, s, 0, cout_p - 128, pl.splits);
        launch_g8<1, F16>(a, s, cout_p - 128, cout_p, pl.splits);
      } else {
        launch_g8<1, F16>(a, s, 0, -1, pl.splits);
      }
      break;
    case 1: launch_igemm<true, 256, 256, 2, 4, 4, F16>(a, pl.splits, s); break;
    case 2: launch_igemm<true, 32, 256, 1, 4, 4, F16>(a, pl.splits, s); break;
    case 3: launch_igemm<true, 128, 256, 2, 4, 4, F16>(a, pl.splits, s); break;
    case 5: launch_igemm<true, 64, 256, 1, 4, 4, F16>(a, pl.splits, s); break;
    default: launch_igemm<true, 128, 128, 2, 2, 4, F16>(a, pl.splits, s); break;
  }
}
template <bool F16>
static void launch_hconv_cfg(const IgemmArgs& a, hipStream_t s, int cin_p, int cout_p) {
  if (cin_p == 32 && cout_p == 32) launch_hconv<32, 32, false, F16>(a, s);
  else if (cin_p == 32) launch_hconv<32, 64, false, F16>(a, s);
  else if (cin_p == 64 && cout_p == 32) launch_hconv<64, 32, false, F16>(a, s);
  else if (cin_p == 64) launch_hconv<64, 64, false, F16>(a, s);
  else if (cout_p == 32) launch_hconv<96, 32, false, F16>(a, s);
  else launch_hconv<96, 64, false, F16>(a, s);
}

static int x_pix_of(int dtype, int cin_p) {
  return dtype == IC2_BF16X3 ? cin_p / 3 * 2 : dtype == IC2_F16X2 ? cin_p / 2 : cin_p;
}
static int x_hb32_of(int dtype, int cin_p) { return dtype == IC2_BF16X3 ? cin_p / 96 : dtype == IC2_F16X2 ? cin_p / 64 : 0; }

enum ConvKind { CK_TORGB, CK_HG4, CK_HCONV, CK_IGEMM };
struct ConvChoice {
  ConvKind kind;
  IgPlan pl;
  bool split384;
};

static ConvChoice conv_choice(int dtype, int out_layout, int out_dtype, int n, int h, int w_, int cin_p, int cout_p,
                              int cout_valid, int kh, int kw, int pad) {
  const int ho = h + 2 * pad - kh + 1, wo = w_ + 2 * pad - kw + 1;
  const int64_t M = (int64_t)n * ho * wo;
  const int64_t x_elems = (int64_t)n * h * w_ * x_pix_of(dtype, cin_p);
  ConvChoice c;
  const bool x3 = dtype == IC2_BF16X3 || dtype == IC2_F16X2;
  const bool x8 = dtype != IC2_F16X2 || (cin_p / 2) % 64 == 0;
  if (x3) dtype = dtype == IC2_F16X2 ? IC2_F16 : IC2_BF16;
  c.pl = ig_plan(dtype, M, cout_p, cin_p, kh, kw, x_elems, x8);
  c.split384 = false;
  if (!x3 && torgb_eligible(dtype, cin_p, cout_valid, kh, kw, pad, out_layout, out_dtype)) {
    c.kind = CK_TORGB;
    c.pl.splits = 1;
    return c;
  }
  static const int hg4_over_hconv = knob("IC2_HG4_HCONV", -1);
  const bool hg4_ok = hg4_eligible(dtype, cin_p, cout_p, kh, kw, x_elems, n, ho, wo);
  const bool hg4_pref = hg4_over_hconv == 1 || (hg4_over_hconv < 0 && cin_p >= 96);
  if (hg4_ok && hg4_pref) c.kind = CK_HG4;
  else if (!x3 && hconv_eligible(dtype, M, cin_p, cout_p, kh, kw)) c.kind = CK_HCONV;
  else if (hg4_ok) c.kind = CK_HG4;
  else c.kind = CK_IGEMM;
  if (c.kind != CK_IGEMM) {
    c.pl.splits = 1;
    return c;
  }
  static const bool split = knob("IC2_IGEMM_SPLIT", 1) != 0;
  c.split384 = is16(dtype) && c.pl.tile == 7 && split && cout_p % 256 == 128 && cout_p > 128 &&
               ceil_div(M, 256) >= 240;
  return c;
}

static const char* conv_choice_name(const ConvChoice& c, int dtype, int n, int ho, int wo, int cin_p, int cout_p) {
  static thread_local char buf[64];
  switch (c.kind) {
    case CK_TORGB: return "torgb";
    case CK_HCONV:
      snprintf(buf, sizeof(buf), "hconv_%d_%d", cin_p, cout_p);
      return buf;
    case CK_HG4: {
      const H4Plan p = h4_plan(n, ho, wo, cout_p);
      snprintf(buf, sizeof(buf), "hg4_o%d_w%s", p.bo, !p.tw32 ? "16_s4" : p.bo == 64 ? "32_p3" : "32_p2");
      return buf;
    }
    default: break;
  }
  if (dtype == IC2_F32) {
    snprintf(buf, sizeof(buf), "igemm_f32_128x128%s", c.pl.splits > 1 ? "_splitk" : "");
    return buf;
  }
  if (c.pl.tile == 6) return c.pl.splits > 1 ? "igemm8_og2_splitk" : c.pl.tail ? "igemm8_og2_tail" : "igemm8_og2";
  if (c.pl.tile == 7) return c.split384 ? "igemm8_og2+og1" : "igemm8_og1";
  snprintf(buf, sizeof(buf), "igemm_%dx%d%s", c.pl.bo, c.pl.bp, c.pl.splits > 1 ? "_splitk" : "");
  return buf;
}

static int conv_chunk_n(int dtype, int n, int h, int w_, int cin_p) {
  const int64_t per_img = (int64_t)h * w_ * x_pix_of(dtype, cin_p) * (dtype == IC2_F32 ? 4 : 2);
  if ((int64_t)n * per_img < (int64_t)kOob || per_img >= (int64_t)kOob) return n;
  const int64_t c = ((int64_t)kOob - 1) / per_img;
  const int64_t chunks = ceil_div(n, c);
  return (int)ceil_div(n, chunks);
}

}

using namespace ic2;

extern "C" const char* ic2_conv_plan(int dtype, int out_dtype, int out_layout, int n, int h, int w_, int cin_p,
                                     int cout_p, int cout_valid, int kh, int kw, int pad) {
  const int ho = h + 2 * pad - kh + 1, wo = w_ + 2 * pad - kw + 1;
  if (n <= 0 || ho <= 0 || wo <= 0 || cin_p <= 0 || cout_p <= 0) return "invalid";
  const int nc = conv_chunk_n(dtype, n, h, w_, cin_p);
  const ConvChoice c = conv_choice(dtype, out_layout, out_dtype, nc, h, w_, cin_p, cout_p, cout_valid, kh, kw, pad);
  const char* name = conv_choice_name(c, dtype, nc, ho, wo, cin_p, cout_p);
  if (dtype != IC2_F16 && dtype != IC2_F16X2) return name;
  static thread_local char f16_name[80];
  snprintf(f16_name, sizeof(f16_name), "%s_f16", name);
  return f16_name;
}

extern "C" int64_t ic2_conv_igemm_ws_bytes(int dtype, int n, int h, int w_, int cin_p, int cout_p, int kh, int kw,
                                           int pad) {
  const int ho = h + 2 * pad - kh + 1, wo = w_ + 2 * pad - kw + 1;
  if (n <= 0 || h <= 0 || w_ <= 0 || ho <= 0 || wo <= 0 || cin_p <= 0 || cout_p <= 0 || kh <= 0 || kw <= 0) return 0;
  const int nc = conv_chunk_n(dtype, n, h, w_, cin_p);
  const ConvChoice c = conv_choice(dtype, IC2_LAYOUT_NHWC, dtype, nc, h, w_, cin_p, cout_p, cout_p, kh, kw, pad);
  if (c.kind != CK_IGEMM || (c.pl.splits == 1 && !c.pl.tail)) return 0;
  return (int64_t)(c.pl.tail ? 2 : c.pl.splits) * nc * ho * wo * cout_p * 4;
}

extern "C" int ic2_conv_igemm_ws(const void* x, const void* w, void* y, int dtype, int out_dtype, int n, int h, int w_,
                                 int cin_p, int cout_p, int cout_valid, int kh, int kw, int pad, int ho, int wo,
                                 const float* oscale, const float* bias, int act, float slope, float act_gain,
                                 float clamp, float out_mul, int out_layout, void* workspace, int64_t ws_bytes,
                                 void* stream) {
  IC2_CHECK_ARG(x && w && y, "conv_igemm: null pointer");
  IC2_CHECK_ARG(dtype == IC2_F32 || dtype == IC2_BF16 || dtype == IC2_F16 || dtype == IC2_BF16X3 || dtype == IC2_F16X2,
                "conv_igemm: bad dtype %d", dtype);
  IC2_CHECK_ARG(dtype != IC2_BF16X3 || (cin_p % 96 == 0 && out_layout == IC2_LAYOUT_NHWC),
                "conv_igemm: split-bf16 input needs cin_p = 3 x a multiple of 32 and NHWC output (cin_p=%d)", cin_p);
  IC2_CHECK_ARG(dtype != IC2_F16X2 || (cin_p % 64 == 0 && out_layout == IC2_LAYOUT_NHWC),
                "conv_igemm: split-weight f16 input needs cin_p = 2 x a multiple of 32 and NHWC output (cin_p=%d)", cin_p);
  IC2_CHECK_ARG(out_dtype == IC2_F32 || out_dtype == IC2_BF16 ||
                    ((out_dtype == IC2_F16 || out_dtype == IC2_F16_IEEE) && out_layout != IC2_LAYOUT_NCHW),
                "conv_igemm: bad out dtype %d", out_dtype);
  IC2_CHECK_ARG(cin_p > 0 && cin_p % 32 == 0 && cout_p > 0 && cout_p % 32 == 0,
                "conv_igemm: channel strides must be positive multiples of 32 (cin_p=%d cout_p=%d)", cin_p, cout_p);
  IC2_CHECK_ARG(n > 0 && h > 0 && w_ > 0 && kh > 0 && kw > 0 && pad >= 0, "conv_igemm: bad geometry");
  IC2_CHECK_ARG(ho == h + 2 * pad - kh + 1 && wo == w_ + 2 * pad - kw + 1,
                "conv_igemm: output size %dx%d does not match input %dx%d, k=%dx%d, pad=%d", ho, wo, h, w_, kh, kw, pad);
  IC2_CHECK_ARG(out_layout == IC2_LAYOUT_NHWC || out_layout == IC2_LAYOUT_NHWC16 ||
                    (out_layout == IC2_LAYOUT_NCHW && out_dtype == IC2_F32 && cout_valid > 0 && cout_valid <= cout_p),
                "conv_igemm: NCHW output needs f32 and 0 < cout_valid <= cout_p (layout %d)", out_layout);
  IC2_CHECK_ARG(((uintptr_t)oscale | (uintptr_t)bias | (uintptr_t)workspace) % 16 == 0,
                "conv_igemm: oscale/bias/workspace must be 16-byte aligned");
  const int nc = conv_chunk_n(dtype, n, h, w_, cin_p);
  if (nc < n) {
    const int64_t x_img = (int64_t)h * w_ * x_pix_of(dtype, cin_p) * (dtype == IC2_F32 ? 4 : 2);
    const int64_t y_img = out_layout == IC2_LAYOUT_NCHW ? (int64_t)cout_valid * ho * wo * 4
                                                        : (int64_t)ho * wo * cout_p * (out_dtype == IC2_F32 ? 4 : 2);
    for (int n0 = 0; n0 < n; n0 += nc) {
      const int nn = n - n0 < nc ? n - n0 : nc;
      const int rc = ic2_conv_igemm_ws(reinterpret_cast<const char*>(x) + n0 * x_img, w,
                                       reinterpret_cast<char*>(y) + n0 * y_img, dtype, out_dtype, nn, h, w_, cin_p,
                                       cout_p, cout_valid, kh, kw, pad, ho, wo,
                                       oscale ? oscale + (int64_t)n0 * cout_p : nullptr, bias, act, slope, act_gain,
                                       clamp, out_mul, out_layout, workspace, ws_bytes, stream);
      if (rc != IC2_OK) return rc;
    }
    return IC2_OK;
  }
  const int64_t M = (int64_t)n * ho * wo;
  IC2_CHECK_ARG(M < (1LL << 30), "conv_igemm: too many output pixels");
  const int out_ieee = out_dtype == IC2_F16_IEEE;
  if (out_ieee) out_dtype = IC2_F16;
  IgemmArgs a;
  a.x = x; a.w = w; a.y = y; a.oscale = oscale; a.bias = bias; a.ws = reinterpret_cast<float*>(workspace);
  a.n = n; a.h = h; a.w_ = w_; a.cin_p = cin_p; a.cout_p = cout_p; a.cout_valid = cout_valid;
  a.kh = kh; a.kw = kw; a.pad = pad; a.ho = ho; a.wo = wo;
  a.M = (int)M; a.K = kh * kw * cin_p; a.nq = a.K / 32;
  a.act = act; a.slope = slope; a.act_gain = act_gain; a.clamp = clamp; a.out_mul = out_mul;
  a.out_layout = out_layout; a.out_dtype = out_dtype; a.out_ieee = out_ieee;
  a.gn_part = nullptr; a.gn_groups = 0; a.gn_c = 0;
  a.in_gn = nullptr; a.in_slope = 0.f;
  a.x_pix = x_pix_of(dtype, cin_p);
  a.x_hb32 = x_hb32_of(dtype, cin_p);
  const int kdt = dtype == IC2_BF16X3 ? IC2_BF16 : dtype == IC2_F16X2 ? IC2_F16 : dtype;
  static const int group = [] {
    const int g = knob("IC2_IGEMM_GROUP", 1);
    return g >= 1 ? g : 1;
  }();
  a.group = group;
  static const int korder = knob("IC2_IGEMM_KORDER", 1);
  a.korder = korder;
  a.o_base = 0;
  hipStream_t s = as_stream(stream);
  ConvChoice c = conv_choice(dtype, out_layout, out_dtype, n, h, w_, cin_p, cout_p, cout_valid, kh, kw, pad);
  dtype = kdt;
  IgPlan& pl = c.pl;
  if (pl.splits > 1 && (workspace == nullptr || ws_bytes < (int64_t)pl.splits * M * cout_p * 4)) pl.splits = 1;
  if (pl.tail && (workspace == nullptr || ws_bytes < 2 * M * cout_p * 4 || a.group != 1)) pl.tail = 0;
  switch (c.kind) {
    case CK_TORGB:
      if (dtype == IC2_F16) launch_torgb<true>(a, s);
      else launch_torgb<false>(a, s);
      break;
    case CK_HG4: hg4_dispatch(a, s, dtype == IC2_F16); break;
    case CK_HCONV:
      if (dtype == IC2_F16) launch_hconv_cfg<true>(a, s, cin_p, cout_p);
      else launch_hconv_cfg<false>(a, s, cin_p, cout_p);
      break;
    case CK_IGEMM:
      if (dtype == IC2_F32) launch_igemm<false, 128, 128, 2, 2, 2>(a, pl.splits, s);
      else if (dtype == IC2_F16) launch_igemm16<true>(a, s, pl, c.split384, cout_p);
      else launch_igemm16<false>(a, s, pl, c.split384, cout_p);
      if (pl.splits > 1 || pl.tail) {
        const int p_lo = pl.tail ? g8_tail_first(M, cout_p) / ((cout_p + 255) / 256) * 256 : 0;
        const int64_t total = (M - p_lo) * (cout_p / 4);
        const int grid = (int)(ceil_div(total, 256) < 4096 ? ceil_div(total, 256) : 4096);
        hipLaunchKernelGGL(igemm_splitk_reduce_kernel, dim3(grid), dim3(256), 0, s, a, pl.tail ? 2 : pl.splits, p_lo);
      }
      break;
  }
  IC2_CHECK_LAUNCH("conv_igemm");
  return IC2_OK;
}

namespace ic2 {
bool conv_gn_in_supported(int dtype, int n, int h, int w_, int cin_p, int cout_p, int kh, int kw, int pad) {
  const int ho = h + 2 * pad - kh + 1, wo = w_ + 2 * pad - kw + 1;
  if (dtype != IC2_BF16 || cin_p != 64 || ho <= 0 || wo <= 0) return false;
  return hconv_eligible(dtype, (int64_t)n * ho * wo, cin_p, cout_p, kh, kw);
}

static int conv_chunk_n(int dtype, int n, int h, int w_, int cin_p);

static bool x3_gn_hg4(int dtype, int n, int h, int w_, int cin_p, int cout_p, int cout_valid, int kh, int kw, int pad,
                      int groups, H4Plan* plan) {
  const int ho = h + 2 * pad - kh + 1, wo = w_ + 2 * pad - kw + 1;
  if (ho <= 0 || wo <= 0 || groups != 32 || cout_valid != cout_p || (cout_p != 64 && cout_p != 128)) return false;
  const int nc = conv_chunk_n(dtype, n, h, w_, cin_p);
  const ConvChoice c = conv_choice(dtype, IC2_LAYOUT_NHWC, IC2_F32, nc, h, w_, cin_p, cout_p, cout_valid, kh, kw, pad);
  if (c.kind != CK_HG4) return false;
  const H4Plan p = h4_plan(nc, ho, wo, cout_p);
  if (!p.tw32 || p.bo != cout_p) return false;
  if (plan) *plan = p;
  return true;
}

static int x3_gn_th(int cout_p) {
  static const bool t12 = knob("IC2_X3_GN_T12", 1) != 0;
  return cout_p == 64 && t12 ? 12 : 8;
}
static int64_t x3_gn_part_doubles(int dtype, int n, int h, int w_, int cin_p, int cout_p, int cout_valid, int kh, int kw,
                                  int pad, int groups) {
  if (!x3_gn_hg4(dtype, n, h, w_, cin_p, cout_p, cout_valid, kh, kw, pad, groups, nullptr)) return 0;
  const int ho = h + 2 * pad - kh + 1, wo = w_ + 2 * pad - kw + 1;
  return (int64_t)n * groups * ceil_div(wo, 32) * ceil_div(ho, x3_gn_th(cout_p)) * 2;
}

bool conv_gn_fuses(int dtype, int n, int h, int w_, int cin_p, int cout_p, int cout_valid, int kh, int kw, int pad,
                   int groups, int fuse_mode) {
  static const bool x3_env = knob("IC2_X3_GN", 1) == 1;
  if (dtype == IC2_BF16X3 || dtype == IC2_F16X2)
    return (fuse_mode > 0 || (fuse_mode < 0 && x3_env)) &&
           x3_gn_hg4(dtype, n, h, w_, cin_p, cout_p, cout_valid, kh, kw, pad, groups, nullptr);
  const int ho = h + 2 * pad - kh + 1, wo = w_ + 2 * pad - kw + 1;
  if (ho <= 0 || wo <= 0) return false;
  static const bool fuse_env = knob("IC2_CONV_GN", 0) == 1;
  const bool fuse_req = fuse_mode < 0 ? fuse_env : fuse_mode > 0;
  return fuse_req && dtype == IC2_BF16 && hconv_eligible(dtype, (int64_t)n * ho * wo, cin_p, cout_p, kh, kw) &&
         groups == 32 && cout_valid == cout_p;
}

int conv_gn_fused(const void* x, const void* w, void* y, int dtype, int n, int h, int w_, int cin_p, int cout_p,
                  int cout_valid, int kh, int kw, int pad, const float* bias, int groups, double* part,
                  int64_t part_doubles, void* workspace, int64_t ws_bytes, int fuse_mode, hipStream_t s,
                  const float* in_gn, float in_slope, float out_mul) {
  const int ho = h + 2 * pad - kh + 1, wo = w_ + 2 * pad - kw + 1;
  const int64_t M = (int64_t)n * ho * wo;
  if (dtype == IC2_BF16X3 || dtype == IC2_F16X2) {
    const int ydt = dtype == IC2_F16X2 ? IC2_F16 : IC2_F32;
    H4Plan p;
    const bool fuse = conv_gn_fuses(dtype, n, h, w_, cin_p, cout_p, cout_valid, kh, kw, pad, groups, fuse_mode) &&
                      in_gn == nullptr && bias != nullptr && part != nullptr &&
                      x3_gn_hg4(dtype, n, h, w_, cin_p, cout_p, cout_valid, kh, kw, pad, groups, &p) &&
                      part_doubles >= x3_gn_part_doubles(dtype, n, h, w_, cin_p, cout_p, cout_valid, kh, kw, pad, groups);
    if (in_gn != nullptr) {
      set_error("conv3x3_gnin_gn_fwd: no input GroupNorm fusion in the split modes");
      return -2;
    }
    if (!fuse) {
      const int rc = ic2_conv_igemm_ws(x, w, y, dtype, ydt, n, h, w_, cin_p, cout_p, cout_valid, kh, kw, pad, ho, wo,
                                       nullptr, bias, 0, 0.f, 1.f, -1.f, out_mul, IC2_LAYOUT_NHWC, workspace,
                                       ws_bytes, s);
      return rc == IC2_OK ? 0 : -1;
    }
    IgemmArgs a;
    a.x = x; a.w = w; a.y = y; a.oscale = nullptr; a.bias = bias; a.ws = nullptr;
    a.n = n; a.h = h; a.w_ = w_; a.cin_p = cin_p; a.cout_p = cout_p; a.cout_valid = cout_valid;
    a.kh = kh; a.kw = kw; a.pad = pad; a.ho = ho; a.wo = wo;
    a.M = (int)M; a.K = kh * kw * cin_p; a.nq = a.K / 32;
    a.act = 0; a.slope = 0.f; a.act_gain = 1.f; a.clamp = -1.f; a.out_mul = out_mul;
    a.out_layout = IC2_LAYOUT_NHWC; a.out_dtype = ydt; a.out_ieee = 0;
    a.gn_part = part; a.gn_groups = groups; a.gn_c = cout_valid;
    a.group = 1; a.korder = 0; a.o_base = 0;
    a.in_gn = nullptr; a.in_slope = 0.f;
    a.x_pix = x_pix_of(dtype, cin_p);
    a.x_hb32 = x_hb32_of(dtype, cin_p);
    const bool f16 = dtype == IC2_F16X2;
    const int nc = conv_chunk_n(dtype, n, h, w_, cin_p);
    const int64_t ntile = ceil_div(wo, 32) * ceil_div(ho, x3_gn_th(cout_p));
    for (int i0 = 0; i0 < n; i0 += nc) {
      const int cnt = n - i0 < nc ? n - i0 : nc;
      a.x = reinterpret_cast<const char*>(x) + (int64_t)i0 * h * w_ * a.x_pix * 2;
      a.y = reinterpret_cast<char*>(y) + (int64_t)i0 * ho * wo * cout_p * (ydt == IC2_F16 ? 2 : 4);
      a.gn_part = part + (int64_t)i0 * groups * ntile * 2;
      a.n = cnt;
      a.M = (int)((int64_t)cnt * ho * wo);
      if (p.bo == 64 && x3_gn_th(64) == 12)
        launch_hg4<4, 6, 1, 4, 32>(a, s, f16 ? hg4_o64_w32_t12_gn_kernel_f16 : hg4_o64_w32_t12_gn_kernel);
      else if (p.bo == 64) launch_hg4<4, 4, 1, 4, 32>(a, s, f16 ? hg4_o64_w32_p3_gn_kernel_f16 : hg4_o64_w32_p3_gn_kernel);
      else launch_hg4<8, 4, 1, 4, 32>(a, s, f16 ? hg4_o128_w32_p2_gn_kernel_f16 : hg4_o128_w32_p2_gn_kernel);
    }
    return (int)ntile;
  }
  const bool hconv = hconv_eligible(dtype, M, cin_p, cout_p, kh, kw);
  const int th = cin_p > 64 ? 4 : 8;
  const int64_t nch = ceil_div(wo, 32) * ceil_div(ho, th);
  static const bool fuse_env = knob("IC2_CONV_GN", 0) == 1;
  const bool fuse_req = fuse_mode < 0 ? fuse_env : fuse_mode > 0;
  const bool fuse = fuse_req && hconv && dtype == IC2_BF16 && part != nullptr && part_doubles >= (int64_t)n * groups * nch * 2 &&
                    groups == 32 && cout_valid == cout_p && bias != nullptr;
  if (in_gn != nullptr && !conv_gn_in_supported(dtype, n, h, w_, cin_p, cout_p, kh, kw, pad)) {
    set_error("conv3x3_gn_fwd: input GroupNorm fusion needs the halo conv (bf16, cin_p 64)");
    return -2;
  }
  if (!fuse && in_gn == nullptr) {
    const int rc = ic2_conv_igemm_ws(x, w, y, dtype, dtype, n, h, w_, cin_p, cout_p, cout_valid, kh, kw, pad, ho, wo,
                                     nullptr, bias, 0, 0.f, 1.f, -1.f, 1.f, IC2_LAYOUT_NHWC, workspace, ws_bytes, s);
    return rc == IC2_OK ? 0 : -1;
  }
  IgemmArgs a;
  a.x = x; a.w = w; a.y = y; a.oscale = nullptr; a.bias = bias; a.ws = nullptr;
  a.n = n; a.h = h; a.w_ = w_; a.cin_p = cin_p; a.cout_p = cout_p; a.cout_valid = cout_valid;
  a.kh = kh; a.kw = kw; a.pad = pad; a.ho = ho; a.wo = wo;
  a.M = (int)M; a.K = kh * kw * cin_p; a.nq = a.K / 32;
  a.act = 0; a.slope = 0.f; a.act_gain = 1.f; a.clamp = -1.f; a.out_mul = 1.f;
  a.out_layout = IC2_LAYOUT_NHWC; a.out_dtype = dtype; a.out_ieee = 0;
  a.gn_part = fuse ? part : nullptr; a.gn_groups = groups; a.gn_c = cout_valid;
  a.group = 1;
  a.korder = 0;
  a.o_base = 0;
  a.in_gn = in_gn; a.in_slope = in_slope;
  a.x_pix = cin_p; a.x_hb32 = 0;
  if (fuse) {
    if (cin_p == 32 && cout_p == 32) launch_hconv<32, 32, true>(a, s);
    else if (cin_p == 32) launch_hconv<32, 64, true>(a, s);
    else if (cin_p == 64 && cout_p == 32) launch_hconv<64, 32, true>(a, s);
    else if (cin_p == 64) launch_hconv<64, 64, true>(a, s);
    else if (cout_p == 32) launch_hconv<96, 32, true>(a, s);
    else launch_hconv<96, 64, true>(a, s);
    return (int)nch;
  }
  if (cin_p == 32 && cout_p == 32) launch_hconv<32, 32>(a, s);
  else if (cin_p == 32) launch_hconv<32, 64>(a, s);
  else if (cin_p == 64 && cout_p == 32) launch_hconv<64, 32>(a, s);
  else launch_hconv<64, 64>(a, s);
  return 0;
}

int64_t conv_gn_fused_part_doubles(int dtype, int n, int h, int w_, int cin_p, int cout_p, int kh, int kw, int pad,
                                   int groups) {
  if (dtype == IC2_BF16X3 || dtype == IC2_F16X2)
    return x3_gn_part_doubles(dtype, n, h, w_, cin_p, cout_p, cout_p, kh, kw, pad, groups);
  const int ho = h + 2 * pad - kh + 1, wo = w_ + 2 * pad - kw + 1;
  if (dtype != IC2_BF16 || !hconv_eligible(dtype, (int64_t)n * ho * wo, cin_p, cout_p, kh, kw)) return 0;
  const int th = cin_p > 64 ? 4 : 8;
  return (int64_t)n * groups * ceil_div(wo, 32) * ceil_div(ho, th) * 2;
}
}

extern "C" int ic2_conv_igemm(const void* x, const void* w, void* y, int dtype, int out_dtype, int n, int h, int w_,
                              int cin_p, int cout_p, int cout_valid, int kh, int kw, int pad, int ho, int wo,
                              const float* oscale, const float* bias, int act, float slope, float act_gain,
                              float clamp, float out_mul, int out_layout, void* stream) {
  return ic2_conv_igemm_ws(x, w, y, dtype, out_dtype, n, h, w_, cin_p, cout_p, cout_valid, kh, kw, pad, ho, wo, oscale,
                           bias, act, slope, act_gain, clamp, out_mul, out_layout, nullptr, 0, stream);
}
```

image_compression_2_amd/csrc/wino.hip:

```cpp
#include "conv_common.h"

namespace ic2 {

constexpr int WX_BO = 128, WX_NW = 8, WX_NS = 3;
constexpr int WX_SLAB = 4 * WX_BO * 64;
constexpr int WX_HROWS = 384, WX_HALO = WX_HROWS * 64;
constexpr int WX_HPW = WX_HROWS / 16 / WX_NW;
constexpr int WX_SLACK = 8 * 1024;
constexpr int WX_LDS = WX_NS * WX_SLAB + 2 * WX_HALO + WX_SLACK;
static_assert(WX_LDS <= 160 * 1024, "LDS");

typedef __attribute__((ext_vector_type(4))) uint32_t wx_u4;
__device__ __forceinline__ f16x8 wx_sub(f16x8 a, f16x8 b) {
  const wx_u4 x = __builtin_bit_cast(wx_u4, a), y = __builtin_bit_cast(wx_u4, b);
  wx_u4 r;
#pragma unroll
  for (int i = 0; i < 4; ++i) asm("v_pk_add_f16 %0, %1, %2 neg_lo:[0,1] neg_hi:[0,1]" : "=v"(r[i]) : "v"(x[i]), "v"(y[i]));
  return __builtin_bit_cast(f16x8, r);
}
__device__ __forceinline__ f16x8 wx_add(f16x8 a, f16x8 b) {
  const wx_u4 x = __builtin_bit_cast(wx_u4, a), y = __builtin_bit_cast(wx_u4, b);
  wx_u4 r;
#pragma unroll
  for (int i = 0; i < 4; ++i) asm("v_pk_add_f16 %0, %1, %2" : "=v"(r[i]) : "v"(x[i]), "v"(y[i]));
  return __builtin_bit_cast(f16x8, r);
}

__device__ __forceinline__ int wx_off(int row, int chunk) { return row * 64 + ((chunk ^ (((row >> 2) & 1) << 1)) << 4); }
__device__ __forceinline__ int wx_hoff(int line, int hp, int idx, int chunk) {
  return (line * hp + idx) * 64 + ((chunk ^ (((idx >> 2) & 1) << 1)) << 4);
}

#ifndef IC2_WX_ABL
#define IC2_WX_ABL 0
#endif
#ifndef IC2_WX_STAMP
#define IC2_WX_STAMP 0
#endif
#ifndef IC2_WX_SCHED
#define IC2_WX_SCHED 0
#endif
#ifndef IC2_WX_PRIO
#define IC2_WX_PRIO 0
#endif

__global__ void __launch_bounds__(512, 1) wino_fx_f16_kernel(IgemmArgs a) {
  __shared__ __attribute__((aligned(16))) char lds[WX_LDS];
  char* const wsl = lds;
  char* const hal = lds + WX_NS * WX_SLAB;
  const int tid = threadIdx.x;
  const int lane = tid & 63;
  const int wid = __builtin_amdgcn_readfirstlane(tid >> 6);
  const int half = wid >> 2;
  const int pg = wid & 3;
  const int fr = lane & 15, fh = lane >> 4;

  const int logical = xcd_remap(blockIdx.x, a.nblocks);
  const int per_group = a.group * (a.nblocks / a.tiles_o);
  const int gi = logical / per_group, grem = logical - gi * per_group;
  const int o_tile = gi * a.group + grem % a.group;
  int pt = grem / a.group;
  const int tx = pt % a.wx_tx;
  pt /= a.wx_tx;
  const int ty = pt % a.wx_ty;
  const int nn = pt / a.wx_ty;
  const int o0 = o_tile * WX_BO;
  const int twp = a.wx_twp, hp = a.wx_hp;
  const int oy0 = ty * a.wx_th, px0 = tx * twp;

  const char* __restrict__ xg = reinterpret_cast<const char*>(a.x);
  const char* __restrict__ ug = reinterpret_cast<const char*>(a.w);
  const int lrow = lane >> 2, pch = lane & 3;

  uint32_t w_off[2][2];
#pragma unroll
  for (int h = 0; h < 2; ++h)
#pragma unroll
    for (int k = 0; k < 2; ++k) {
      const int row = (wid + WX_NW * k) * 16 + lrow;
      const int nu = row >> 6, ol = h * 64 + (row & 63), o = o0 + ol;
      w_off[h][k] =
          o < a.cout_p ? (uint32_t)(((ol * 12 + nu) * a.cin_p) * 2 + ((pch ^ (((row >> 2) & 1) << 1)) << 4)) : kOob;
    }
  const char* const ug0 = ug + (int64_t)o0 * 12 * a.cin_p * 2;
  uint32_t h_off[WX_HPW];
#pragma unroll
  for (int k = 0; k < WX_HPW; ++k) {
    const int l = (wid + WX_NW * k) * 16 + lrow;
    const int line = l / hp, idx = l - line * hp;
    const int iy = oy0 - a.pad + (line >> 1), ix = 2 * px0 - a.pad + 2 * idx + (line & 1);
    const bool ok = l < a.wx_nh && (unsigned)iy < (unsigned)a.h && (unsigned)ix < (unsigned)a.w_;
    h_off[k] = ok ? (uint32_t)((((nn * a.h + iy) * a.w_ + ix) * a.cin_p + ((pch ^ (((idx >> 2) & 1) << 1)) << 3)) * 2)
                  : kOob;
  }
  int boff[2][3];
  const int ns = a.wx_ns;
#pragma unroll
  for (int jb = 0; jb < 2; ++jb) {
    const int b = pg * 2 + jb;
    const int rr = min(b / ns, a.wx_th - 1), t = (b % ns) * 16 + fr;
#pragma unroll
    for (int m = 0; m < 3; ++m) {
      const int j = half + m;
      boff[jb][m] = wx_hoff(rr * 2 + (j & 1), hp, t + (j >> 1), fh);
    }
  }
  const int ky_step = 2 * hp * 64;
  const int aoff = wx_off(fr, fh) + half * 2 * 64 * 64;
  const int CB = a.cin_p >> 5;

  auto issue_hs = [&](int cb, int j) {
    const __amdgpu_buffer_rsrc_t rs = __builtin_amdgcn_make_buffer_rsrc(
        (void*)(ug0 + ((int64_t)(4 * (j >> 1)) * a.cin_p + cb * 32) * 2), 0, cb < CB ? kOob : 0, kRsrcWord3);
    char* dst = wsl + j * (WX_SLAB / 2);
#pragma unroll
    for (int k = 0; k < 2; ++k)
      __builtin_amdgcn_raw_ptr_buffer_load_lds(
          rs, (__attribute__((address_space(3))) void*)(dst + (wid + WX_NW * k) * 1024), 16, w_off[j & 1][k], 0, 0, 0);
  };
  auto issue_hp = [&](int cb, int k) {
    const __amdgpu_buffer_rsrc_t rs =
        __builtin_amdgcn_make_buffer_rsrc((void*)(xg + (int64_t)cb * 64), 0, cb < CB ? kOob : 0, kRsrcWord3);
    __builtin_amdgcn_raw_ptr_buffer_load_lds(
        rs, (__attribute__((address_space(3))) void*)(hal + (cb & 1) * WX_HALO + (wid + WX_NW * k) * 1024), 16,
        h_off[k], 0, 0, 0);
  };

  f32x4 acc[2][8][2];
#pragma unroll
  for (int nl = 0; nl < 2; ++nl)
#pragma unroll
    for (int i = 0; i < 8; ++i)
#pragma unroll
      for (int jb = 0; jb < 2; ++jb) acc[nl][i][jb] = f32x4{0.f, 0.f, 0.f, 0.f};

  f16x8 d[2][3];
  f16x8 v[2][2];
  auto read_d = [&](const char* hl) {
#pragma unroll
    for (int jb = 0; jb < 2; ++jb)
#pragma unroll
      for (int m = 0; m < 3; ++m) d[jb][m] = *reinterpret_cast<const f16x8*>(hl + boff[jb][m]);
  };
  auto make_v = [&]() {
    if (half == 0) {
#pragma unroll
      for (int jb = 0; jb < 2; ++jb) {
        v[0][jb] = wx_sub(d[jb][0], d[jb][2]);
        v[1][jb] = wx_add(d[jb][1], d[jb][2]);
      }
    } else {
#pragma unroll
      for (int jb = 0; jb < 2; ++jb) {
        v[0][jb] = wx_sub(d[jb][1], d[jb][0]);
        v[1][jb] = wx_sub(d[jb][0], d[jb][2]);
      }
    }
  };

  issue_hp(0, 0);
  issue_hp(0, 1);
  issue_hp(0, 2);
#pragma unroll
  for (int j = 0; j < 5; ++j) issue_hs(0, j);
  issue_hp(1, 0);
  if constexpr (IC2_WX_SCHED == 2) {
    asm volatile("s_waitcnt vmcnt(5)" ::: "memory");
  } else {
    issue_hp(1, 1);
    asm volatile("s_waitcnt vmcnt(6)" ::: "memory");
  }
  __builtin_amdgcn_s_barrier();
  read_d(hal);
  bf16x8 af[2][4];
  auto read_a = [&](const char* wl, int nl) {
#pragma unroll
    for (int i = 0; i < 4; ++i) af[nl][i] = *reinterpret_cast<const bf16x8*>(wl + (nl * 64 + i * 16) * 64);
  };
  if (half == 1) __builtin_amdgcn_s_barrier();
  __builtin_amdgcn_sched_barrier(0);

  uint64_t st[7] = {0, 0, 0, 0, 0, 0, 0};
  uint64_t t_prev = 0, t_loop = 0;
  auto stamp = [&](int k) {
    if constexpr (IC2_WX_STAMP) {
      const uint64_t t = __builtin_amdgcn_s_memtime();
      st[k] += t - t_prev;
      t_prev = t;
    }
  };
  if constexpr (IC2_WX_STAMP) t_loop = t_prev = __builtin_amdgcn_s_memtime();
  for (int cb = 0; cb < CB; ++cb) {
    const char* hb_cur = hal + (cb & 1) * WX_HALO;
    const char* hb_nxt = hal + ((cb + 1) & 1) * WX_HALO;
#pragma unroll
    for (int j = 0; j < 6; ++j) {
      const int ky = j >> 1, hx = j & 1;
      const char* wl = wsl + j * (WX_SLAB / 2) + aoff;
      auto r_dma = [&]() {
        if (!(IC2_WX_ABL & 1) || cb == 0) issue_hs(cb + (j + 5) / 6, (j + 5) % 6);
        if constexpr (IC2_WX_SCHED == 2) {
          if (j == 0) issue_hp(cb + 1, 1);
          if (j == 1) issue_hp(cb + 1, 2);
          if (j == 5) issue_hp(cb + 2, 0);
        } else {
// ... 192 lines not shown
  int64_t best_rounds = -1;
  for (int ns = 1; ns <= 8; ns *= 2)
    for (int th = 1; th * ns <= 8; ++th) {
      if (force_th && th != force_th) continue;
      for (int twp = 1; twp <= 16 * ns; ++twp) {
        if (force_twp && twp != force_twp) continue;
        const int hp = twp + 1, nh = (th + 2) * 2 * hp;
        if (nh > WX_HROWS) break;
        WxTile t;
        t.twp = twp; t.th = th; t.ns = ns; t.hp = hp; t.nh = nh;
        t.tx = (int)ceil_div(pairs, twp);
        t.ty = (int)ceil_div(ho, th);
        t.to = (int)ceil_div(cout_p, WX_BO);
        t.blocks = (int64_t)n * t.tx * t.ty * t.to;
        const int64_t rounds = ceil_div(t.blocks, 256);
        const bool full = twp % 16 == 0, best_full = best.twp % 16 == 0;
        if (best_rounds < 0 || rounds < best_rounds ||
            (rounds == best_rounds && (t.blocks < best.blocks || (t.blocks == best.blocks && full && !best_full)))) {
          best = t;
          best_rounds = rounds;
        }
      }
    }
  return best;
}

static int wx_chunk_n(int n, int h, int w_, int cin_p) {
  const int64_t per_img = (int64_t)h * w_ * cin_p * 2;
  if ((int64_t)n * per_img < (int64_t)kOob || per_img >= (int64_t)kOob) return n;
  const int64_t c = ((int64_t)kOob - 1) / per_img;
  return (int)ceil_div(n, ceil_div(n, c));
}

static void* g_wx_stamp = nullptr;
static int64_t g_wx_stamp_bytes = 0;

}

using namespace ic2;

extern "C" int ic2_conv_wino_stamps(void* buf, int64_t bytes) {
  IC2_CHECK_ARG(IC2_WX_STAMP, "conv_wino_stamps: not a stamp build (IC2_WX_STAMP)");
  g_wx_stamp = buf;
  g_wx_stamp_bytes = bytes;
  return IC2_OK;
}

extern "C" int ic2_pack_weight_wino(const float* w, int cout, int cin, int cout_p, int cin_p, int prenorm,
                                    float scale, void* u_out, int dtype, void* stream) {
  IC2_CHECK_ARG(w && u_out && cout > 0 && cin > 0 && cout_p >= cout && cin_p >= cin, "pack_weight_wino: bad arguments");
  IC2_CHECK_ARG(dtype == IC2_F16, "pack_weight_wino: only f16 U (dtype %d)", dtype);
  hipLaunchKernelGGL(pack_wino_kernel, dim3(cout_p), dim3(256), 0, as_stream(stream), w, cout, cin, cout_p, cin_p,
                     prenorm, scale, (_Float16*)u_out);
  IC2_CHECK_LAUNCH("pack_weight_wino");
  return IC2_OK;
}

extern "C" int ic2_conv_wino_preferred(int dtype, int n, int h, int w_, int cin_p, int cout_p, int kh, int kw,
                                       int pad) {
  static const int mode = knob("IC2_WINO", 1);
  const int ho = h + 2 * pad - kh + 1, wo = w_ + 2 * pad - kw + 1;
  const bool legal = dtype == IC2_F16 && kh == 3 && kw == 3 && n > 0 && ho > 0 && wo > 0 && cin_p % 32 == 0 &&
                     cout_p % 32 == 0 && (int64_t)cout_p * 12 * cin_p * 2 < (int64_t)kOob;
  if (!legal || mode == 0) return 0;
  if (mode == 2) return 1;
  return cin_p >= 256 && cout_p >= 256 && ho >= 50 && wo >= 50;
}

extern "C" const char* ic2_conv_wino_plan(int n, int h, int w_, int cin_p, int cout_p, int pad) {
  const int ho = h + 2 * pad - 2, wo = w_ + 2 * pad - 2;
  if (n <= 0 || ho <= 0 || wo <= 0 || cin_p <= 0 || cin_p % 32 || cout_p <= 0 || cout_p % 32) return "invalid";
  const WxTile t = wx_tile(wx_chunk_n(n, h, w_, cin_p), ho, wo, cout_p);
  static thread_local char buf[64];
  snprintf(buf, sizeof(buf), "wino_fx_o128_p%dx%d_f16", t.twp, t.th);
  return buf;
}

extern "C" int ic2_conv_wino(const void* x, const void* u, void* y, int dtype, int out_dtype, int n, int h, int w_,
                             int cin_p, int cout_p, int cout_valid, int pad, int ho, int wo, const float* oscale,
                             const float* bias, int act, float slope, float act_gain, float clamp, float out_mul,
                             int out_layout, void* stream) {
  IC2_CHECK_ARG(x && u && y, "conv_wino: null pointer");
  IC2_CHECK_ARG(dtype == IC2_F16, "conv_wino: f16 operands only (dtype %d)", dtype);
  IC2_CHECK_ARG(out_dtype == IC2_F32 || out_dtype == IC2_BF16 ||
                    ((out_dtype == IC2_F16 || out_dtype == IC2_F16_IEEE) && out_layout != IC2_LAYOUT_NCHW),
                "conv_wino: bad out dtype %d", out_dtype);
  IC2_CHECK_ARG(cin_p > 0 && cin_p % 32 == 0 && cout_p > 0 && cout_p % 32 == 0,
                "conv_wino: channel strides must be positive multiples of 32 (cin_p=%d cout_p=%d)", cin_p, cout_p);
  IC2_CHECK_ARG(n > 0 && h > 0 && w_ > 0 && pad >= 0, "conv_wino: bad geometry");
  IC2_CHECK_ARG(ho == h + 2 * pad - 2 && wo == w_ + 2 * pad - 2 && ho > 0 && wo > 0,
                "conv_wino: output size %dx%d does not match input %dx%d, k=3x3, pad=%d", ho, wo, h, w_, pad);
  IC2_CHECK_ARG(out_layout == IC2_LAYOUT_NHWC || out_layout == IC2_LAYOUT_NHWC16 ||
                    (out_layout == IC2_LAYOUT_NCHW && out_dtype == IC2_F32 && cout_valid > 0 && cout_valid <= cout_p),
                "conv_wino: NCHW output needs f32 and 0 < cout_valid <= cout_p (layout %d)", out_layout);
  IC2_CHECK_ARG(((uintptr_t)oscale | (uintptr_t)bias) % 16 == 0, "conv_wino: oscale/bias must be 16-byte aligned");
  IC2_CHECK_ARG((int64_t)cout_p * 12 * cin_p * 2 < (int64_t)kOob, "conv_wino: weights too large");
  const int nc = wx_chunk_n(n, h, w_, cin_p);
  if (nc < n) {
    const int64_t x_img = (int64_t)h * w_ * cin_p * 2;
    const int64_t y_img = out_layout == IC2_LAYOUT_NCHW ? (int64_t)cout_valid * ho * wo * 4
                                                        : (int64_t)ho * wo * cout_p * (out_dtype == IC2_F32 ? 4 : 2);
    for (int n0 = 0; n0 < n; n0 += nc) {
      const int nn = n - n0 < nc ? n - n0 : nc;
      const int rc = ic2_conv_wino(reinterpret_cast<const char*>(x) + n0 * x_img, u,
                                   reinterpret_cast<char*>(y) + n0 * y_img, dtype, out_dtype, nn, h, w_, cin_p, cout_p,
                                   cout_valid, pad, ho, wo, oscale ? oscale + (int64_t)n0 * cout_p : nullptr, bias, act,
                                   slope, act_gain, clamp, out_mul, out_layout, stream);
      if (rc != IC2_OK) return rc;
    }
    return IC2_OK;
  }
  const WxTile t = wx_tile(n, ho, wo, cout_p);
  IC2_CHECK_ARG(t.blocks > 0 && t.blocks < (1LL << 31), "conv_wino: bad tile plan");
  const int out_ieee = out_dtype == IC2_F16_IEEE;
  if (out_ieee) out_dtype = IC2_F16;
  IgemmArgs a{};
  a.x = x; a.w = u; a.y = y; a.oscale = oscale; a.bias = bias;
  a.ws = IC2_WX_STAMP && (int64_t)t.blocks * 8 * 8 * 8 <= g_wx_stamp_bytes ? reinterpret_cast<float*>(g_wx_stamp)
                                                                          : nullptr;
  IC2_CHECK_ARG(!IC2_WX_STAMP || a.ws, "conv_wino: stamp build without a large enough ic2_conv_wino_stamps buffer");
  a.n = n; a.h = h; a.w_ = w_; a.cin_p = cin_p; a.cout_p = cout_p; a.cout_valid = cout_valid;
  a.kh = 3; a.kw = 3; a.pad = pad; a.ho = ho; a.wo = wo;
  a.M = n * ho * wo; a.K = 9 * cin_p; a.nq = 3 * (cin_p / 32);
  static const int og_knob = knob("IC2_WINO_OGROUP", 1);
  int og = og_knob < 1 ? 1 : og_knob > t.to ? t.to : og_knob;
  while (t.to % og) --og;
  a.tiles_o = t.to; a.nblocks = (int)t.blocks; a.group = og; a.korder = 1; a.o_base = 0;
  a.act = act; a.slope = slope; a.act_gain = act_gain; a.clamp = clamp; a.out_mul = out_mul;
  a.out_layout = out_layout; a.out_dtype = out_dtype; a.out_ieee = out_ieee;
  a.gn_part = nullptr; a.gn_groups = 0; a.gn_c = 0; a.in_gn = nullptr; a.in_slope = 0.f;
  a.x_pix = cin_p; a.x_hb32 = 0;
  a.wx_twp = t.twp; a.wx_th = t.th; a.wx_ns = t.ns; a.wx_hp = t.hp; a.wx_nh = t.nh; a.wx_tx = t.tx; a.wx_ty = t.ty;
  hipLaunchKernelGGL(wino_fx_f16_kernel, dim3((unsigned)t.blocks), dim3(64 * WX_NW), 0, as_stream(stream), a);
  IC2_CHECK_LAUNCH("conv_wino");
  return IC2_OK;
}
```

image_compression_2_amd/networks_stylegan3.py:

```python
from __future__ import annotations

import ctypes
import math

import numpy as np
import scipy.signal
import torch
import torch.nn.functional as F

from . import _native as nv
from . import autograd_ops as ao
from . import sg3_ops

_FLR_BLOCKED = nv.knob("IC2_FLR_BLOCKED", 1) != 0
_MOD_BATCH_MAX = 512


def _train_mode(module, *tensors):
    if not torch.is_grad_enabled():
        return False
    if any(p.requires_grad for p in module.parameters()):
        return False
    return any(t is not None and t.requires_grad for t in tensors)


def _refuse(module, out, *tensors):
    return nv.refuse_backward(type(module).__name__ + ".forward", out, tensors, (module,))


def _version_key(*tensors):
    return tuple((t.data_ptr(), t._version, t.device) for t in tensors)


class FullyConnectedLayer(torch.nn.Module):

    def __init__(self, in_features, out_features, activation="linear", bias=True, lr_multiplier=1, weight_init=1,
                 bias_init=0):
        super().__init__()
        self.in_features = in_features
        self.out_features = out_features
        self.activation = activation
        self.weight = torch.nn.Parameter(torch.randn([out_features, in_features]) * (weight_init / lr_multiplier))
        bias_init = np.broadcast_to(np.asarray(bias_init, dtype=np.float32), [out_features])
        self.bias = torch.nn.Parameter(torch.from_numpy(bias_init / lr_multiplier)) if bias else None
        self.weight_gain = lr_multiplier / np.sqrt(in_features)
        self.bias_gain = lr_multiplier

    def run(self, x, out=None, ldx=None, n=None):
        n = x.shape[0] if n is None else n
        ldx = self.in_features if ldx is None else ldx
        if out is None:
            out = torch.empty([n, self.out_features], dtype=torch.float32, device=x.device)
        act = nv.ACT_LRELU if self.activation == "lrelu" else nv.ACT_LINEAR
        nv.call("ic2_fc", nv.ptr(x), ldx, nv.ptr(self.weight), nv.ptr(self.bias), nv.ptr(out), n, self.in_features,
                self.out_features, float(self.weight_gain), float(self.bias_gain), act, 0.2,
                float(np.sqrt(2)) if act == nv.ACT_LRELU else 1.0, nv.stream_of(x))
        return out

    def forward(self, x):
        xin = x
        x = x.to(torch.float32).contiguous()
        nv.require_gpu(x)
        if self.activation not in ("linear", "lrelu"):
            raise NotImplementedError(self.activation)
        return _refuse(self, self.run(x), xin)

    def extra_repr(self):
        return f"in_features={self.in_features:d}, out_features={self.out_features:d}, activation={self.activation:s}"


class MappingNetwork(torch.nn.Module):

    def __init__(self, z_dim, c_dim, w_dim, num_ws, num_layers=2, lr_multiplier=0.01, w_avg_beta=0.998):
        super().__init__()
        if c_dim:
            raise NotImplementedError("conditional mapping (c_dim > 0) is not on the path")
        self.z_dim, self.c_dim, self.w_dim, self.num_ws = z_dim, c_dim, w_dim, num_ws
        self.num_layers, self.w_avg_beta = num_layers, w_avg_beta
        features = [z_dim] + [w_dim] * num_layers
        for idx, in_f, out_f in zip(range(num_layers), features[:-1], features[1:]):
            setattr(self, f"fc{idx}", FullyConnectedLayer(in_f, out_f, activation="lrelu", lr_multiplier=lr_multiplier))
        self.register_buffer("w_avg", torch.zeros([w_dim]))

    def forward(self, z, c=None, truncation_psi=1, truncation_cutoff=None, update_emas=False):
        if update_emas:
            raise NotImplementedError("update_emas is a training feature (out of scope)")
        x = z.to(torch.float32).contiguous()
        nv.require_gpu(x)
        x = x * (x.square().mean(1, keepdim=True) + 1e-8).rsqrt()
        for idx in range(self.num_layers):
            x = getattr(self, f"fc{idx}").run(x.contiguous())
        x = x.unsqueeze(1).repeat([1, self.num_ws, 1])
        if truncation_psi != 1:
            cut = self.num_ws if truncation_cutoff is None else truncation_cutoff
            x[:, :cut] = self.w_avg.lerp(x[:, :cut], truncation_psi)
        return _refuse(self, x, z)

# ... 139 lines not shown
        self.down_taps = filter_size * self.down_factor if self.down_factor > 1 and not self.is_torgb else 1
        self.down_radial = use_radial_filters and not self.is_critically_sampled
        self.register_buffer("down_filter", self.design_lowpass_filter(
            numtaps=self.down_taps, cutoff=self.out_cutoff, width=self.out_half_width * 2, fs=self.tmp_sampling_rate))

        pad_total = (self.out_size - 1) * self.down_factor + 1
        pad_total -= (self.in_size + self.conv_kernel - 1) * self.up_factor
        pad_total += self.up_taps + self.down_taps - 2
        pad_lo = (pad_total + self.up_factor) // 2
        pad_hi = pad_total - pad_lo
        self.padding = [int(pad_lo[0]), int(pad_hi[0]), int(pad_lo[1]), int(pad_hi[1])]

        self.act_gain = 1.0 if self.is_torgb else float(np.sqrt(2))
        self._fu = None if self.up_filter is None else np.ascontiguousarray(self.up_filter.numpy(), np.float32)
        self._fd = None if self.down_filter is None else np.ascontiguousarray(self.down_filter.numpy(), np.float32)
        self._cache = {}
        self._ig_cache = None

    @property
    def cin_p(self):
        return nv.pad_synth(self.in_channels)

    @property
    def cout_p(self):
        return nv.pad_synth(self.out_channels)

    def input_gain(self):
        key = _version_key(self.magnitude_ema)
        if self._ig_cache is None or self._ig_cache[0] != key:
            self._ig_cache = (key, float(self.magnitude_ema.detach().float().rsqrt().cpu()))
        return self._ig_cache[1]

    def packed(self, dt):
        key = (dt, _version_key(self.weight, self.bias))
        hit = self._cache.get(dt)
        if hit is not None and hit[0] == key:
            return hit[1]
        w = self.weight.detach().to(torch.float32).contiguous()
        k = self.conv_kernel
        wp = torch.empty([self.cout_p, k, k, self.cin_p], dtype=dt, device=w.device)
        wsq = torch.empty([self.out_channels, self.in_channels], dtype=torch.float32, device=w.device)
        nv.call("ic2_pack_weight", nv.ptr(w), self.out_channels, self.in_channels, k, k, self.cout_p, self.cin_p,
                int(not self.is_torgb), 1.0, nv.ptr(wp), nv.dtype_code(dt), nv.ptr(wsq), nv.stream_of(w))
        bp = torch.zeros([self.cout_p], dtype=torch.float32, device=w.device)
        bp[: self.out_channels] = self.bias.detach().float()
        val = (wp, wsq, bp)
        self._cache[dt] = (key, val)
        return val

    def mod_record(self, dt, ws_off, styles, xs, os_):
        _, wsq, _ = self.packed(dt)
        fc = self.affine
        style_gain = float(1 / np.sqrt(self.in_channels * (self.conv_kernel ** 2))) if self.is_torgb else 1.0
        f32 = lambda v: int(np.float32(v).view(np.uint32))
        dp = lambda t: 0 if t is None else t.data_ptr()
        return [dp(fc.weight), dp(fc.bias), dp(wsq), dp(styles), dp(xs), dp(os_), ws_off, self.in_channels, self.cin_p,
                self.out_channels, self.cout_p, int(not self.is_torgb), f32(fc.weight_gain), f32(fc.bias_gain),
                f32(style_gain), f32(self.input_gain())]

    def batchable(self):
        return self.in_channels <= _MOD_BATCH_MAX and self.affine.in_features <= _MOD_BATCH_MAX

    def scales(self, ws, ldx, n, dt, unbatched=False):
        dev = ws.device
        styles = torch.empty([n, self.in_channels], dtype=torch.float32, device=dev)
        xs = torch.empty([n, self.cin_p], dtype=torch.float32, device=dev)
        os_ = torch.empty([n, self.cout_p], dtype=torch.float32, device=dev)
        if unbatched or not self.batchable():
            _, wsq, _ = self.packed(dt)
            fc = self.affine
            stream = nv.stream_of(ws)
            nv.call("ic2_fc", nv.ptr(ws), ldx, nv.ptr(fc.weight), nv.ptr(fc.bias), nv.ptr(styles), n, fc.in_features,
                    self.in_channels, float(fc.weight_gain), float(fc.bias_gain), nv.ACT_LINEAR, 0.0, 1.0, stream)
            style_gain = float(1 / np.sqrt(self.in_channels * (self.conv_kernel ** 2))) if self.is_torgb else 1.0
            nv.call("ic2_modconv_prep", nv.ptr(styles), nv.ptr(wsq), n, self.in_channels, self.out_channels,
                    self.cin_p, self.cout_p, int(not self.is_torgb), style_gain, float(self.input_gain()), nv.ptr(xs),
                    nv.ptr(os_), None, stream)
            return xs, os_
        rec = np.asarray([self.mod_record(dt, 0, styles, xs, os_)], dtype=np.int64)
        nv.call("ic2_modconv_prep_batched", nv.ptr(ws), ldx, n, self.affine.in_features, 1,
                rec.ctypes.data_as(ctypes.c_void_p), nv.stream_of(ws))
        return xs, os_

    def run_nhwc(self, x, n, dt, oscale, post_scale, final_scale=None):
        s_in = int(self.in_size[0])
        k = self.conv_kernel
        pad = k - 1
        conv = s_in + 2 * pad - k + 1
        wp, _, bp = self.packed(dt)
        stream = nv.stream_of(x)
        nv.note_flops(2 * n * conv * conv * self.out_channels * self.in_channels * k * k)
        if self.is_torgb:
            assert self.up_factor == 1 and self.down_factor == 1 and self.padding == [0, 0, 0, 0]
            out = torch.empty([n, self.out_channels, conv, conv], dtype=torch.float32, device=x.device)
            clamp = float(self.conv_clamp) if self.conv_clamp is not None else -1.0
            nv.conv_igemm(nv.ptr(x), nv.ptr(wp), nv.ptr(out), nv.dtype_code(dt), nv.F32, n, s_in, s_in, self.cin_p,
                          self.cout_p, self.out_channels, k, k, pad, conv, conv, nv.ptr(oscale), nv.ptr(bp),
                          nv.ACT_LRELU, 1.0, 1.0, clamp, float(1.0 if final_scale is None else final_scale), nv.NCHW,
                          stream, x.device)
            return out
        y, blocked = self.conv_nhwc(x, n, dt, oscale)
        return self.flrelu_nhwc(y, dt, post_scale, blocked=blocked)

    def conv_nhwc(self, x, n, dt, oscale):
        s_in = int(self.in_size[0])
        k = self.conv_kernel
        pad = k - 1
        conv = s_in + 2 * pad - k + 1
        wp, _, bp = self.packed(dt)
        stream = nv.stream_of(x)
        ydt = torch.float16 if dt in (torch.bfloat16, torch.float16) else dt
        blocked = ydt == torch.float16 and _FLR_BLOCKED
        if blocked:
            y = torch.empty([n, self.cout_p // 16, conv, conv, 16], dtype=ydt, device=x.device)
        else:
            y = torch.empty([n, conv, conv, self.cout_p], dtype=ydt, device=x.device)
        layout = nv.NHWC16 if blocked else nv.NHWC
        if nv.wino_preferred(nv.dtype_code(dt), n, s_in, s_in, self.cin_p, self.cout_p, k, k, pad):
            nv.conv_wino(nv.ptr(x), nv.ptr(self.packed_wino()), nv.ptr(y), nv.F16, nv.dtype_code(ydt), n, s_in, s_in,
                         self.cin_p, self.cout_p, self.out_channels, pad, conv, conv, nv.ptr(oscale), nv.ptr(bp), 0,
                         0.0, 1.0, -1.0, 1.0, layout, stream)
        else:
            nv.conv_igemm(nv.ptr(x), nv.ptr(wp), nv.ptr(y), nv.dtype_code(dt), nv.dtype_code(ydt), n, s_in, s_in,
                          self.cin_p, self.cout_p, self.out_channels, k, k, pad, conv, conv, nv.ptr(oscale),
                          nv.ptr(bp), 0, 0.0, 1.0, -1.0, 1.0, layout, stream, x.device)
        return y, blocked

    def packed_wino(self):
        key = _version_key(self.weight)
        hit = self._cache.get("wino")
        if hit is not None and hit[0] == key:
            return hit[1]
        w = self.weight.detach().to(torch.float32).contiguous()
        u = torch.empty([self.cout_p, 3, 4, self.cin_p], dtype=torch.float16, device=w.device)
        nv.call("ic2_pack_weight_wino", nv.ptr(w), self.out_channels, self.in_channels, self.cout_p, self.cin_p,
                int(not self.is_torgb), 1.0, nv.ptr(u), nv.F16, nv.stream_of(w))
        self._cache["wino"] = (key, u)
        return u

    def flrelu_nhwc(self, y, dt_out, post_scale=None, blocked=False):
        n, conv = y.shape[0], y.shape[2 if blocked else 1]
        s_out = int(self.out_size[0])
        out = torch.empty([n, s_out, s_out, self.cout_p], dtype=dt_out, device=y.device)
        fu = self._fu
        fd = self._fd
        px0, px1, py0, py1 = self.padding
        clamp = float(self.conv_clamp) if self.conv_clamp is not None else -1.0
        nv.call("ic2_flrelu_nhwc16" if blocked else "ic2_flrelu_nhwc", nv.ptr(y), nv.ptr(out), nv.dtype_code(y.dtype),
                nv.dtype_code(dt_out), n,
                self.cout_p, conv, conv, s_out, s_out, None if fu is None else fu.ctypes.data_as(ctypes.c_void_p),
                1 if fu is None else fu.shape[0], None if fd is None else fd.ctypes.data_as(ctypes.c_void_p),
                1 if fd is None else fd.shape[0], None, self.up_factor, self.down_factor, px0, px1, py0, py1,
                float(self.act_gain), 0.2, clamp, 0, nv.ptr(post_scale), nv.stream_of(y))
        return out

    def packed_adjoint(self, dt):
        key = (dt, _version_key(self.weight))
        hit = self._cache.get(("adj", dt))
        if hit is not None and hit[0] == key:
            return hit[1]
        w = self.weight.detach().to(torch.float32)
        if not self.is_torgb:
            w = w * w.square().mean(dim=[1, 2, 3], keepdim=True).rsqrt()
        wt = ao.pack_conv_weight(w.transpose(0, 1).flip(2, 3), self.cout_p, self.cin_p, dt)
        self._cache[("adj", dt)] = (key, wt)
        return wt

    def packed_adjoint_wino(self, scale=1.0):
        key = (_version_key(self.weight), scale)
        hit = self._cache.get(("adj_wino", scale))
        if hit is not None and hit[0] == key:
            return hit[1]
        w = self.weight.detach().to(torch.float32)
        if not self.is_torgb:
            w = w * w.square().mean(dim=[1, 2, 3], keepdim=True).rsqrt()
        wa = w.transpose(0, 1).flip(2, 3).contiguous()
        u = torch.empty([self.cin_p, 3, 4, self.cout_p], dtype=torch.float16, device=w.device)
        nv.call("ic2_pack_weight_wino", nv.ptr(wa), self.in_channels, self.out_channels, self.cin_p, self.cout_p, 0,
                float(scale), nv.ptr(u), nv.F16, nv.stream_of(wa))
        self._cache[("adj_wino", scale)] = (key, u)
        return u

    def modulation_train(self, w):
        A = self.affine
        styles = F.linear(w, A.weight * float(A.weight_gain), A.bias * float(A.bias_gain))
        ig = self.input_gain()
        if self.is_torgb:
            s = styles * float(1 / np.sqrt(self.in_channels * (self.conv_kernel ** 2)))
            d = torch.full([w.shape[0], self.out_channels], ig, dtype=torch.float32, device=w.device)
        else:
            s = styles * styles.square().mean().rsqrt()
            _, wsq, _ = self.packed(torch.float32)
            d = (s.square() @ wsq.t() + 1e-8).rsqrt() * ig
        return F.pad(s, (0, self.cin_p - self.in_channels)), F.pad(d, (0, self.cout_p - self.out_channels))

    def forward_train_nhwc(self, x, w, dt, final_scale=None):
        xs, os_ = self.modulation_train(w)
        if not self.is_torgb:
            return ao.SynthLayerNHWC.apply(x.contiguous(), xs.contiguous(), os_.contiguous(), self, dt)
        return self.torgb_train_nhwc(ao.ScaleNHWC.apply(x, xs), os_, dt, final_scale)

    def torgb_train_nhwc(self, a, os_, dt, final_scale=None):
        wp, _, bp = self.packed(dt)
        c = ao.FrozenConvNHWC.apply(a, wp, self.packed_adjoint(dt), 1, 0, self.out_channels, self.in_channels)
        y = c * os_[:, None, None, :] + bp
        if self.conv_clamp is not None:
            y = y.clamp(-float(self.conv_clamp), float(self.conv_clamp))
        img = y[..., : self.out_channels].permute(0, 3, 1, 2)
        return img if final_scale is None else img * float(final_scale)

    def forward(self, x, w, noise_mode="random", force_fp32=False, update_emas=False):
        assert noise_mode in ("random", "const", "none")
        if update_emas:
            raise NotImplementedError("update_emas is a training feature (out of scope)")
        if _train_mode(self, x, w):
            return self.forward_train(x, w)
        x_in, w_in = x, w
        x = x.to(torch.float32).contiguous()
        w = w.to(torch.float32).contiguous()
        nv.require_gpu(x, w)
        n = x.shape[0]
        assert list(x.shape) == [n, self.in_channels, int(self.in_size[1]), int(self.in_size[0])], x.shape
        dt = torch.float32
        xs, os_ = self.scales(w, self.w_dim, n, dt)
        s_in = int(self.in_size[0])
        xn = torch.empty([n, s_in, s_in, self.cin_p], dtype=dt, device=x.device)
        nv.call("ic2_nchw_to_nhwc", nv.ptr(x), nv.ptr(xn), nv.F32, n, self.in_channels, s_in, s_in, self.cin_p,
                nv.ptr(xs), nv.stream_of(x))
        out = self.run_nhwc(xn, n, dt, os_, None)
        if self.is_torgb:
            return _refuse(self, out, x_in, w_in)
        s_out = int(self.out_size[0])
# ... 22 lines not shown
        f = scipy.signal.firwin(numtaps=numtaps, cutoff=cutoff, width=width, fs=fs)
        return torch.as_tensor(f, dtype=torch.float32)

    def extra_repr(self):
        return "\n".join([
            f"w_dim={self.w_dim:d}, is_torgb={self.is_torgb},",
            f"is_critically_sampled={self.is_critically_sampled}, use_fp16={self.use_fp16},",
            f"in_sampling_rate={self.in_sampling_rate:g}, out_sampling_rate={self.out_sampling_rate:g},",
            f"in_cutoff={self.in_cutoff:g}, out_cutoff={self.out_cutoff:g},",
            f"in_half_width={self.in_half_width:g}, out_half_width={self.out_half_width:g},",
            f"in_size={list(self.in_size)}, out_size={list(self.out_size)},",
            f"in_channels={self.in_channels:d}, out_channels={self.out_channels:d}"])


class SynthesisNetwork(torch.nn.Module):

    def __init__(self, w_dim, img_resolution, img_channels, channel_base=32768, channel_max=512, num_layers=14,
                 num_critical=2, first_cutoff=2, first_stopband=2 ** 2.1, last_stopband_rel=2 ** 0.3, margin_size=10,
                 output_scale=0.25, num_fp16_res=4, precision="fp32", **layer_kwargs):
        super().__init__()
        self.w_dim = w_dim
        self.num_ws = num_layers + 2
        self.img_resolution = img_resolution
        self.img_channels = img_channels
        self.num_layers = num_layers
        self.num_critical = num_critical
        self.margin_size = margin_size
        self.output_scale = output_scale
        self.num_fp16_res = num_fp16_res
        self.precision = precision
        nv.torch_dtype(precision)
        self.train_f16 = False

        last_cutoff = self.img_resolution / 2
        last_stopband = last_cutoff * last_stopband_rel
        exponents = np.minimum(np.arange(self.num_layers + 1) / (self.num_layers - self.num_critical), 1)
        cutoffs = first_cutoff * (last_cutoff / first_cutoff) ** exponents
        stopbands = first_stopband * (last_stopband / first_stopband) ** exponents
        sampling_rates = np.exp2(np.ceil(np.log2(np.minimum(stopbands * 2, self.img_resolution))))
        half_widths = np.maximum(stopbands, sampling_rates / 2) - cutoffs
        sizes = sampling_rates + self.margin_size * 2
        sizes[-2:] = self.img_resolution
        channels = np.rint(np.minimum((channel_base / 2) / cutoffs, channel_max))
        channels[-1] = self.img_channels

        self.input = SynthesisInput(w_dim=self.w_dim, channels=int(channels[0]), size=int(sizes[0]),
                                    sampling_rate=sampling_rates[0], bandwidth=cutoffs[0])
        self.layer_names = []
        for idx in range(self.num_layers + 1):
            prev = max(idx - 1, 0)
            is_torgb = idx == self.num_layers
            is_critically_sampled = idx >= self.num_layers - self.num_critical
            use_fp16 = sampling_rates[idx] * (2 ** self.num_fp16_res) > self.img_resolution
            layer = SynthesisLayer(
                w_dim=self.w_dim, is_torgb=is_torgb, is_critically_sampled=is_critically_sampled, use_fp16=use_fp16,
                in_channels=int(channels[prev]), out_channels=int(channels[idx]), in_size=int(sizes[prev]),
                out_size=int(sizes[idx]), in_sampling_rate=int(sampling_rates[prev]),
                out_sampling_rate=int(sampling_rates[idx]), in_cutoff=cutoffs[prev], out_cutoff=cutoffs[idx],
                in_half_width=half_widths[prev], out_half_width=half_widths[idx], **layer_kwargs)
            name = f"L{idx}_{layer.out_size[0]}_{layer.out_channels}"
            setattr(self, name, layer)
            self.layer_names.append(name)

    def layers(self):
        return [getattr(self, name) for name in self.layer_names]

    def forward(self, ws, noise_mode="const", force_fp32=False, update_emas=False, **layer_kwargs):
        assert noise_mode in ("random", "const", "none")
        if update_emas:
            raise NotImplementedError("update_emas is a training feature (out of scope)")
        assert ws.ndim == 3 and ws.shape[1] == self.num_ws and ws.shape[2] == self.w_dim, ws.shape
        dt = torch.float32 if force_fp32 else nv.torch_dtype(self.precision)
        if _train_mode(self, ws):
            tdt = dt if dt != torch.float16 or self.train_f16 else torch.bfloat16
            return self.forward_train(ws, tdt)
        ws_in = ws
        ws = ws.to(torch.float32).contiguous()
        nv.require_gpu(ws)
        n = ws.shape[0]
        ldx = self.num_ws * self.w_dim
        layers = self.layers()
        sc = self.scales_batched(ws, ldx, n, dt)
        x = self.input.run_nhwc(ws, ldx, n, dt, sc[0][0])
        for i, L in enumerate(layers):
            post = sc[i + 1][0] if i + 1 < len(layers) else None
            x = L.run_nhwc(x, n, dt, sc[i][1], post, final_scale=self.output_scale if L.is_torgb else None)
        return _refuse(self, x, ws_in)

    def scales_batched(self, ws, ldx, n, dt):
        layers = self.layers()
        if not all(L.batchable() for L in layers):
            flat = ws.view(-1)
            return [L.scales(flat[(i + 1) * self.w_dim:], ldx, n, dt) for i, L in enumerate(layers)]
        sizes = [(n * L.in_channels + 3) // 4 * 4 + n * L.cin_p + n * L.cout_p for L in layers]
        buf = torch.empty([sum(sizes)], dtype=torch.float32, device=ws.device)
        rec = np.zeros([len(layers), 16], dtype=np.int64)
        out, off = [], 0
        for i, L in enumerate(layers):
            ns = (n * L.in_channels + 3) // 4 * 4
            styles = buf[off:off + ns]
            xs = buf[off + ns:off + ns + n * L.cin_p].view(n, L.cin_p)
            os_ = buf[off + ns + n * L.cin_p:off + sizes[i]].view(n, L.cout_p)
            off += sizes[i]
            rec[i] = L.mod_record(dt, (i + 1) * self.w_dim, styles, xs, os_)
            out.append((xs, os_))
        nv.call("ic2_modconv_prep_batched", nv.ptr(ws), ldx, n, self.w_dim, len(layers),
                rec.ctypes.data_as(ctypes.c_void_p), nv.stream_of(ws))
        return out

    def _train_mod_pack(self, convs, device):
        key = (device,) + tuple(k for L in convs for k in _version_key(L.affine.weight, L.affine.bias, L.weight,
                                                                        L.magnitude_ema))
        hit = getattr(self, "_mod_pack_cache", None)
        if hit is not None and hit[0] == key:
            return hit[1]
        nl = len(convs)
        cm, om = max(L.cin_p for L in convs), max(L.cout_p for L in convs)
        wst = torch.zeros([nl, cm, self.w_dim], dtype=torch.float32, device=device)
        bst = torch.zeros([nl, cm], dtype=torch.float32, device=device)
        wsq = torch.zeros([nl, om, cm], dtype=torch.float32, device=device)
        igm = torch.zeros([nl, 1, om], dtype=torch.float32, device=device)
        with torch.no_grad():
            for i, L in enumerate(convs):
                A = L.affine
                wst[i, : L.in_channels] = A.weight.float() * float(A.weight_gain)
                bst[i, : L.in_channels] = A.bias.float() * float(A.bias_gain)
                wsq[i, : L.out_channels, : L.in_channels] = L.packed(torch.float32)[1]
                igm[i, 0, : L.out_channels] = L.input_gain()
        cin = torch.tensor([float(L.in_channels) for L in convs], dtype=torch.float32).to(device)
        pack = (wst, bst, wsq, igm, cin)
        self._mod_pack_cache = (key, pack)
        return pack

    def forward_train(self, ws, dt):
        ws = ws.to(torch.float32)
        nv.require_gpu(ws.contiguous())
        C = self.input.channels
        x = self.input.forward_train_nhwc(ws[:, 0], dt)
        layers = self.layers()
        x = F.pad(x, (0, layers[0].cin_p - C)).to(dt)
        convs = [L for L in layers if not L.is_torgb]
        assert all(not L.is_torgb for L in layers[: len(convs)]), "modulated layers first, ToRGB last"
        wst, bst, wsq, igm, cin = self._train_mod_pack(convs, ws.device)
        n = ws.shape[0]
        wl = ws[:, 1: 1 + len(convs)].transpose(0, 1)
        st = torch.baddbmm(bst.unsqueeze(1), wl, wst.transpose(1, 2))
        s = st * (st.square().sum(dim=(1, 2)) / (cin * n)).rsqrt()[:, None, None]
        d = (torch.bmm(s.square(), wsq.transpose(1, 2)) + 1e-8).rsqrt() * igm
        xss = ao.SplitRows.apply(s, tuple(L.cin_p for L in convs))
        oss = ao.SplitRows.apply(d, tuple(L.cout_p for L in convs))
        rgb = layers[len(convs)]
        xs_rgb, os_rgb = rgb.modulation_train(ws[:, len(convs) + 1])
        x = ao.ScaleNHWC.apply(x, xss[0])
        for i, L in enumerate(convs):
            xs_next = xss[i + 1] if i + 1 < len(convs) else xs_rgb
            x = ao.SynthLayerScaledNHWC.apply(x, oss[i], xs_next, L, dt)
        return rgb.torgb_train_nhwc(x, os_rgb, dt, final_scale=self.output_scale)

    def extra_repr(self):
        return "\n".join([
            f"w_dim={self.w_dim:d}, num_ws={self.num_ws:d},",
            f"img_resolution={self.img_resolution:d}, img_channels={self.img_channels:d},",
            f"num_layers={self.num_layers:d}, num_critical={self.num_critical:d},",
            f"margin_size={self.margin_size:d}, num_fp16_res={self.num_fp16_res:d}, precision={self.precision}"])


class Generator(torch.nn.Module):

    def __init__(self, z_dim=512, c_dim=0, w_dim=512, img_resolution=256, img_channels=3, mapping_kwargs={},
# ... 33 lines not shown
```

include/ic2ops.h:

```cpp
#ifndef IC2OPS_H_
#define IC2OPS_H_

#include <stdint.h>
#include <stddef.h>

#ifdef __cplusplus
extern "C" {
#endif

enum { IC2_OK = 0, IC2_E_INVALID = 1, IC2_E_UNSUPPORTED = 2, IC2_E_LAUNCH = 3 };
enum { IC2_F32 = 0, IC2_BF16 = 1, IC2_F16 = 2, IC2_BF16X3 = 3, IC2_F16X2 = 4,
       IC2_F16_IEEE = 5 };
enum { IC2_ACT_LINEAR = 0, IC2_ACT_LRELU = 1 };
enum { IC2_LAYOUT_NHWC = 0, IC2_LAYOUT_NCHW = 1, IC2_LAYOUT_NHWC16 = 2 };

const char* ic2_last_error(void);
int ic2_abi_version(void);


int ic2_quantize_uniform(const float* w, int64_t n, int bits, float* q_out, int32_t* idx_out, void* stream);

int ic2_quantize_codebook_argmin(const float* z, int64_t n, const float* codebook, int k, int64_t* idx_out,
                                 float* zq_out, uint32_t* hist_out, void* stream);

int ic2_codebook_lookup(const int64_t* codes, int64_t n, const float* codebook, int k, float* w_out,
                        int32_t* oob_flag, void* stream);

int ic2_gumbel_softmax_quantize(const float* z, int64_t n, const float* codebook, int k, const float* log_tau,
                                float tau, int hard, uint64_t seed, uint64_t offset, const float* gumbel_noise,
                                float* disc_out, int64_t* idx_out, float* prob_sum_out, void* stream);
int ic2_gumbel_softmax_quantize_dseed(const float* z, int64_t n, const float* codebook, int k, const float* log_tau,
                                      float tau, int hard, const int64_t* seed_dev, uint64_t offset,
                                      const float* gumbel_noise, float* disc_out, int64_t* idx_out,
                                      float* prob_sum_out, void* stream);

int ic2_code_record(const void* codes, int kind, int k, int bits, const void* golden, int64_t n, uint32_t* counts,
                    void* stream);


int ic2_bias_act(const void* x, const float* b, void* y, int dtype, int64_t outer, int64_t c, int64_t inner,
                 int act, float alpha, float gain, float clamp, void* stream);

int ic2_upfirdn2d(const void* x, void* y, int dtype, int64_t nc, int in_h, int in_w, int out_h, int out_w,
                  const float* f, int f_ndim, int f_h, int f_w, int up_x, int up_y, int down_x, int down_y,
                  int px0, int px1, int py0, int py1, int flip, float gain, void* stream);

int ic2_filtered_lrelu(const void* x, void* y, int dtype, int64_t n, int64_t c, int in_h, int in_w, int out_h,
                       int out_w, const float* fu, int fu_taps, const float* fd, int fd_taps, const float* b,
                       int up, int down, int px0, int px1, int py0, int py1, float gain, float slope,
                       float clamp, int flip, void* stream);

int ic2_flrelu_nhwc(const void* x, void* y, int dtype_in, int dtype_out, int n, int c_p, int in_h, int in_w,
                    int out_h, int out_w, const float* fu, int fu_taps, const float* fd, int fd_taps, const float* b,
                    int up, int down, int px0, int px1, int py0, int py1, float gain, float slope, float clamp,
                    int flip, const float* post_scale, void* stream);

int ic2_flrelu_nhwc16(const void* x, void* y, int dtype_in, int dtype_out, int n, int c_p, int in_h, int in_w,
                      int out_h, int out_w, const float* fu, int fu_taps, const float* fd, int fd_taps, const float* b,
                      int up, int down, int px0, int px1, int py0, int py1, float gain, float slope, float clamp,
                      int flip, const float* post_scale, void* stream);


int ic2_fc(const float* x, int64_t ldx, const float* w, const float* b, float* y, int n, int in_f, int out_f,
           float w_gain, float b_gain, int act, float alpha, float act_gain, void* stream);

int ic2_pack_weight(const float* w, int cout, int cin, int kh, int kw, int cout_p, int cin_p, int prenorm,
                    float scale, void* w_out, int dtype, float* wsq_out, void* stream);

int ic2_pack_weight_adjoint(const float* w, int cout, int cin, int kh, int kw, int cin_p, int cout_p, void* w_out,
                            int dtype, void* stream);

int ic2_modconv_prep(const float* styles, const float* wsq, int n, int cin, int cout, int cin_p, int cout_p,
                     int demod, float style_gain, float input_gain, float* xscale_out, float* oscale_out,
                     float* scratch, void* stream);

int ic2_modconv_prep_batched(const float* ws, int64_t ldx, int n, int w_dim, int nl, const int64_t* layers,
                             void* stream);

const char* ic2_conv_plan(int dtype, int out_dtype, int out_layout, int n, int h, int w, int cin_p, int cout_p,
                          int cout_valid, int kh, int kw, int pad);

int ic2_dev_mode(void);

int ic2_conv_igemm(const void* x, const void* w, void* y, int dtype, int out_dtype, int n, int h, int w_,
                   int cin_p, int cout_p, int cout_valid, int kh, int kw, int pad, int ho, int wo,
                   const float* oscale, const float* bias, int act, float slope, float act_gain, float clamp,
                   float out_mul, int out_layout, void* stream);

int64_t ic2_conv_igemm_ws_bytes(int dtype, int n, int h, int w_, int cin_p, int cout_p, int kh, int kw, int pad);
int ic2_conv_igemm_ws(const void* x, const void* w, void* y, int dtype, int out_dtype, int n, int h, int w_,
                      int cin_p, int cout_p, int cout_valid, int kh, int kw, int pad, int ho, int wo,
                      const float* oscale, const float* bias, int act, float slope, float act_gain, float clamp,
                      float out_mul, int out_layout, void* workspace, int64_t ws_bytes, void* stream);

int ic2_pack_weight_wino(const float* w, int cout, int cin, int cout_p, int cin_p, int prenorm, float scale,
                         void* u_out, int dtype, void* stream);

int ic2_conv_wino(const void* x, const void* u, void* y, int dtype, int out_dtype, int n, int h, int w_, int cin_p,
                  int cout_p, int cout_valid, int pad, int ho, int wo, const float* oscale, const float* bias, int act,
                  float slope, float act_gain, float clamp, float out_mul, int out_layout, void* stream);

int ic2_conv_wino_preferred(int dtype, int n, int h, int w_, int cin_p, int cout_p, int kh, int kw, int pad);

int ic2_conv_wino_stamps(void* buf, int64_t bytes);

const char* ic2_conv_wino_plan(int n, int h, int w_, int cin_p, int cout_p, int pad);

int ic2_synth_input_features(const float* t, const float* freqs, const float* phases, const float* transform,
                             int n, int c, int c_p, int size, float sampling_rate, float bandwidth, void* x_out,
                             int dtype, void* stream);


int ic2_from_rgb_conv(const float* x, int cin, const void* w, int cin_p, const float* bias, void* y, int n, int h,
                      int w_, int cout_p, void* stream);

int ic2_from_rgb_conv_x3(const float* x, int cin, const float* w, int cout, const float* bias, void* y, int n, int h,
                         int w_, int cout_p, void* stream);
int ic2_from_rgb_conv_f16(const float* x, int cin, const float* w, int cout, const float* bias, void* y, int n, int h,
                          int w_, int cout_p, void* stream);

int ic2_nchw_to_nhwc(const float* x, void* y, int dtype, int n, int c, int h, int w, int c_p, const float* scale,
                     void* stream);

int ic2_nhwc_to_nchw(const void* x, int dtype, float* y, int n, int c, int h, int w, int c_p, void* stream);

int64_t ic2_group_norm_stats_floats(int n, int hw, int groups);
int ic2_group_norm_stats(const void* y, int dtype, int n, int hw, int c_p, int c, int groups, float eps,
                         float* stats_out, void* stream);

int ic2_gn_lrelu_pool(const void* y, void* out, int dtype_in, int dtype_out, int n, int h, int w, int c_p, int c,
                      int groups, const float* stats, const float* gamma, const float* beta, float slope,
                      int pool, void* stream);

int64_t ic2_global_avg_pool_floats(int n, int hw, int c_p, int c);
int ic2_global_avg_pool(const void* x, int dtype, int n, int hw, int c_p, int c, float* out, void* stream);

int ic2_reparameterize(const float* params, const float* eps, int n, int num_ws, int w_dim, int ws_total,
                       int ws_off, float* w_out, float* mean_out, float* logvar_out, void* stream);


int64_t ic2_uint8_sse_scratch_doubles(int64_t n_img);
int ic2_uint8_sse(const float* a, const float* b, int64_t n_img, int64_t per_img, double* sse_out, double* scratch,
                  void* stream);

int ic2_resize_bilinear(const float* x, float* y, int64_t nc, int h, int w, int oh, int ow, void* stream);

int64_t ic2_rc_bound(int64_t n_streams, int64_t per_stream);
int ic2_rc_encode(const int32_t* codes, int64_t n_streams, int num_ws, int w_dim, int n_symbols, uint8_t* out,
                  int64_t out_cap, int64_t* stream_bytes, int n_threads);
int ic2_rc_decode(const uint8_t* in, const int64_t* stream_bytes, int64_t n_streams, int num_ws, int w_dim,
                  int n_symbols, int32_t* codes_out, int n_threads);


int64_t ic2_conv_wgrad_ws_floats(int n, int h, int w, int cin_p, int cout_p, int kh, int kw, int pad);
int ic2_conv_wgrad(const void* x, const void* dy, float* dw, int dtype, int n, int h, int w, int cin_p, int cout_p,
                   int kh, int kw, int pad, float* workspace, int64_t ws_floats, void* stream);
int ic2_conv_wgrad_oihw(const void* x, const void* dy, float* dw, int dtype, int n, int h, int w, int cin_p,
                        int cout_p, int cout, int cin, int kh, int kw, int pad, float* workspace, int64_t ws_floats,
                        void* stream);

int64_t ic2_gn_lrelu_pool_bwd_floats(int n, int h, int w, int c_p, int groups);
int ic2_gn_lrelu_pool_bwd(const void* y, const void* dout, void* dy, int dtype_y, int dtype_dout, int dtype_dy, int n,
                          int h, int w, int c_p, int c, int groups, const float* stats, const float* gamma,
// ... 54 lines not shown
```

Baseline: 1519 images/s.

## Chain synthesis layers in channel-blocked NHWC16 activations between flrelu and conv

Lets the strip MFMA filtered-lrelu kernel write its output in a channel-blocked NHWC16 layout, using a DPP quad transpose and permlane16 swaps so each lane issues 128-bit stores. The following igemm, Winograd or toRGB conv reads that layout directly through a new halo offset computation. The generator loop picks blocked output only when the next layer reports it can accept it. The aim is better store and halo-load locality per 16-channel block, at the cost of more layout plumbing and extra template instances.

```diff
diff --git a/image_compression_2_amd/_native.py b/image_compression_2_amd/_native.py
--- a/image_compression_2_amd/_native.py
+++ b/image_compression_2_amd/_native.py
@@ -17,6 +17,15 @@
 ACT_LINEAR, ACT_LRELU = 0, 1
 NHWC, NCHW, NHWC16 = 0, 1, 2
 
+
+def act_in_layout(layout):
+    return layout << 4
+
+
+def flr_out_layout(layout):
+    return layout << 4
+
+
 _P = ctypes.c_void_p
 _I = ctypes.c_int
 _I64 = ctypes.c_int64
@@ -26,6 +35,7 @@
     "ic2_abi_version": [],
     "ic2_dev_mode": [],
     "ic2_conv_plan": [_I, _I, _I, _I, _I, _I, _I, _I, _I, _I, _I, _I],
+    "ic2_conv_accepts_nhwc16": [_I, _I, _I, _I, _I, _I, _I, _I, _I, _I, _I, _I],
     "ic2_quantize_uniform": [_P, _I64, _I, _P, _P, _P],
     "ic2_quantize_codebook_argmin": [_P, _I64, _P, _I, _P, _P, _P, _P],
     "ic2_codebook_lookup": [_P, _I64, _P, _I, _P, _P, _P],
@@ -160,6 +170,11 @@
                  pad).decode()
 
 
+def conv_accepts_nhwc16(dtype, out_dtype, out_layout, n, h, w, cin_p, cout_p, cout_valid, kh, kw, pad):
+    return bool(query("ic2_conv_accepts_nhwc16", dtype, out_dtype, out_layout, n, h, w, cin_p, cout_p, cout_valid, kh,
+                      kw, pad))
+
+
 def conv_igemm(x, w, y, dtype, out_dtype, n, h, w_, cin_p, cout_p, cout_valid, kh, kw, pad, ho, wo, oscale, bias,
                act, slope, act_gain, clamp, out_mul, out_layout, stream, device):
     nbytes = int(query("ic2_conv_igemm_ws_bytes", dtype, n, h, w_, cin_p, cout_p, kh, kw, pad))
diff --git a/image_compression_2_amd/csrc/conv_common.h b/image_compression_2_amd/csrc/conv_common.h
--- a/image_compression_2_amd/csrc/conv_common.h
+++ b/image_compression_2_amd/csrc/conv_common.h
@@ -41,10 +41,19 @@
   const float* in_gn;
   float in_slope;
   int x_pix, x_hb32;
+  int x_img, x_plane;
   int wx_twp, wx_th, wx_ns, wx_hp, wx_nh, wx_tx, wx_ty;
   int out_ieee;
 };
 __device__ __forceinline__ int ig_xb32(const IgemmArgs& a, int b) { return b >= a.x_hb32 ? b - a.x_hb32 : b; }
+__device__ __forceinline__ uint32_t ig_halo_off(const IgemmArgs& a, int nn, int iy, int ix, int chunk) {
+  return (uint32_t)((nn * a.x_img + (iy * a.w_ + ix) * a.x_pix) * 2 + (chunk >> 1) * a.x_plane + (chunk & 1) * 16);
+}
+inline void ig_set_input_layout(IgemmArgs& a, bool blocked) {
+  if (blocked) a.x_pix = 16;
+  a.x_img = blocked ? a.cin_p * a.h * a.w_ : a.x_pix * a.h * a.w_;
+  a.x_plane = blocked ? a.h * a.w_ * 32 : 32;
+}
 
 __device__ __forceinline__ float4 ig_load_oscale(const IgemmArgs& a, int nn, int ob) {
   return a.oscale && ob < a.cout_p ? *reinterpret_cast<const float4*>(a.oscale + (int64_t)nn * a.cout_p + ob)
diff --git a/image_compression_2_amd/csrc/flrelu.h b/image_compression_2_amd/csrc/flrelu.h
--- a/image_compression_2_amd/csrc/flrelu.h
+++ b/image_compression_2_amd/csrc/flrelu.h
@@ -17,6 +17,7 @@
   int tiles_x, tiles_y, cblocks, nimg;
   int order;
   int out_f16;
+  int out_blocked;
   float slope, lim;
   float gdg[12];
   float gu[24];
diff --git a/image_compression_2_amd/csrc/flrelu.hip b/image_compression_2_amd/csrc/flrelu.hip
--- a/image_compression_2_amd/csrc/flrelu.hip
+++ b/image_compression_2_amd/csrc/flrelu.hip
@@ -307,6 +307,11 @@
                          float gain, float slope, float clamp, int flip, const float* post_scale, void* stream,
                          const char* name, bool in_blocked = false) {
   IC2_CHECK_ARG(x && y, "%s: null pointer", name);
+  const int out_layout = IC2_FLR_OUT_LAYOUT_OF(dtype_out);
+  dtype_out = IC2_FLR_DTYPE_OF(dtype_out);
+  IC2_CHECK_ARG(out_layout == IC2_LAYOUT_NHWC || (out_layout == IC2_LAYOUT_NHWC16 && chlast),
+                "%s: output layout %d (NHWC, or NHWC16 from the NHWC / NHWC16 entry points)", name, out_layout);
+  const bool out_blocked = out_layout == IC2_LAYOUT_NHWC16;
   IC2_CHECK_ARG(n > 0 && c > 0 && in_h > 0 && in_w > 0 && up >= 1 && down >= 1, "%s: bad geometry", name);
   IC2_CHECK_ARG(fu_taps >= 1 && fd_taps >= 1 && fu_taps <= 24 && fd_taps <= 12, "%s: unsupported taps", name);
   const int ew = (in_w * up + (px0 + px1) - (fu_taps - 1) - (fd_taps - 1) + (down - 1)) / down;
@@ -345,6 +350,7 @@
   const bool mfma_ok = chlast && (dtype_in == IC2_BF16 || dtype_in == IC2_F16) &&
                        (dtype_out == IC2_BF16 || dtype_out == IC2_F16) && b == nullptr && dx == dy;
   a.out_f16 = dtype_out == IC2_F16;
+  a.out_blocked = out_blocked;
   if ((use_mfma || dtype_in == IC2_F16) && mfma_ok) {
     float gu[24] = {}, gd[12] = {}, gdg[12] = {};
     for (int t = 0; t < fu_taps; ++t) gu[t] = (fu ? (flip ? fu[t] : fu[fu_taps - 1 - t]) : 1.f) * (float)up;
@@ -370,6 +376,11 @@
       IC2_CHECK_LAUNCH(name);
       return IC2_OK;
     }
+  }
+  if (out_blocked) {
+    set_error("%s: channel-blocked output needs the strip MFMA instance (f16 input, bf16/f16 out, no bias, up 2/4 with "
+              "6*up taps, down 2 / 12 taps)", name);
+    return IC2_E_UNSUPPORTED;
   }
   if (in_blocked) {
     set_error("%s: channel-blocked input needs the MFMA instance (f16/bf16 in, bf16/f16 out, no bias, up 2/4 with 6*up "
diff --git a/image_compression_2_amd/csrc/flrelu_mfma.h b/image_compression_2_amd/csrc/flrelu_mfma.h
--- a/image_compression_2_amd/csrc/flrelu_mfma.h
+++ b/image_compression_2_amd/csrc/flrelu_mfma.h
@@ -10,6 +10,7 @@
 typedef float fm_f4 __attribute__((ext_vector_type(4)));
 typedef float fm_f2 __attribute__((ext_vector_type(2)));
 typedef uint32_t v2u32_t __attribute__((ext_vector_type(2)));
+typedef uint32_t v4u32_t __attribute__((ext_vector_type(4)));
 
 constexpr int FM_TAPS = 276;
 constexpr int FM_TAPS_CL = 476;
diff --git a/image_compression_2_amd/csrc/flrelu_mfma.hip b/image_compression_2_amd/csrc/flrelu_mfma.hip
--- a/image_compression_2_amd/csrc/flrelu_mfma.hip
+++ b/image_compression_2_amd/csrc/flrelu_mfma.hip
@@ -675,6 +675,29 @@
   static_assert((NG - 1) * GRP_DW + (S - 1) * IN_PITCH + 8 * 8 * ((NINX + 7) / 8) <= RING_DW, "ring bounds");
 };
 
+__device__ __forceinline__ void fm_quad_transpose(uint2 (&v)[4], int p) {
+  const bool b0 = (p & 1) != 0, b1 = (p & 2) != 0;
+  auto swap = [](uint32_t& lo, uint32_t& hi, bool up, auto ctrl) {
+    constexpr int CTRL = decltype(ctrl)::value;
+    const uint32_t send = up ? lo : hi;
+    const uint32_t recv = (uint32_t)__builtin_amdgcn_mov_dpp((int)send, CTRL, 0xf, 0xf, true);
+    lo = up ? recv : lo;
+    hi = up ? hi : recv;
+  };
+  using X1 = std::integral_constant<int, 0xB1>;
+  using X2 = std::integral_constant<int, 0x4E>;
+#pragma unroll
+  for (int i = 0; i < 4; i += 2) {
+    swap(v[i].x, v[i + 1].x, b0, X1{});
+    swap(v[i].y, v[i + 1].y, b0, X1{});
+  }
+#pragma unroll
+  for (int i = 0; i < 2; ++i) {
+    swap(v[i].x, v[i + 2].x, b1, X2{});
+    swap(v[i].y, v[i + 2].y, b1, X2{});
+  }
+}
+
 #ifndef IC2_FM3_ABL
 #define IC2_FM3_ABL 0
 #endif
@@ -684,9 +707,13 @@
 #ifndef FM3_DEFER_ST
 #define FM3_DEFER_ST 0
 #endif
-template <int U, int DELTA, int NW, bool CL>
+#ifndef FM3_BLK16
+#define FM3_BLK16 1
+#endif
+template <int U, int DELTA, int NW, bool CL, bool BLK>
 __global__ void __launch_bounds__(64 * NW, 32 / NW) flrelu_mfma3_kernel(FlrArgs a, int nitems, int nseg, int seg_len) {
   constexpr int TOX = 32, NT = 64 * NW, RR = 16 / NW, OCW = TOX / NW;
+  constexpr int NST = BLK && FM3_BLK16 ? OCW / 2 : OCW;
   using G2 = FmGeom2<U, TOX>;
   using G = FmGeom3<U>;
   constexpr int NINX = G::NINX, NBX = G2::NBX, NOB = G2::NOB, S = G::S, NG = G::NG;
@@ -828,18 +855,49 @@
     const int iy0 = (32 * t0 + DELTA - a.py0) / U, sx0 = (ox0 * 2 - a.px0 + DELTA) / U;
     const bool has_next = w + (int)gridDim.x < nitems;
     if (first) asm volatile("s_waitcnt vmcnt(0)" ::: "memory");
-    else asm volatile("s_waitcnt vmcnt(%0)" ::"n"(OCW) : "memory");
+    else asm volatile("s_waitcnt vmcnt(%0)" ::"n"(NST) : "memory");
     first = false;
     __syncthreads();
     float4 psv = make_float4(1.f, 1.f, 1.f, 1.f);
     if (a.post_scale) psv = *reinterpret_cast<const float4*>(ps_lds + 4 * g);
     const float ps[4] = {psv.x, psv.y, psv.z, psv.w};
     const __amdgpu_buffer_rsrc_t ors = __builtin_amdgcn_make_buffer_rsrc(
-        (void*)(yout + (int64_t)n * a.out_h * a.out_w * a.c_p + c0), 0, FM_OOB, 0x00020000);
+        (void*)(yout + (int64_t)n * a.out_h * a.out_w * a.c_p + (BLK ? (int64_t)c0 * a.out_h * a.out_w : (int64_t)c0)), 0,
+        FM_OOB, 0x00020000);
     const int kend = 2 * nt;
 
     fm_f4 acc_a[OCW], acc_b[OCW];
     auto store_tile = [&](int tt) __attribute__((always_inline)) {
+      if constexpr (BLK) {
+        static_assert(OCW == 4, "quad transpose: 4 columns per wave");
+        uint2 v[OCW];
+#pragma unroll
+        for (int i = 0; i < OCW; ++i)
+          v[i] = fm_out4(a.out_f16, acc_a[i][0] * ps[0], acc_a[i][1] * ps[1], acc_a[i][2] * ps[2], acc_a[i][3] * ps[3]);
+        fm_quad_transpose(v, tp);
+        const int gy0 = 16 * (t0 + tt) + 4 * tq, gx = ox0 + 4 * wave + tp;
+        if constexpr (FM3_BLK16) {
+#pragma unroll
+          for (int h = 0; h < 2; ++h) {
+            const auto x = __builtin_amdgcn_permlane16_swap(v[2 * h].x, v[2 * h + 1].x, false, false);
+            const auto y = __builtin_amdgcn_permlane16_swap(v[2 * h].y, v[2 * h + 1].y, false, false);
+            const int gy = gy0 + 2 * h + (g & 1);
+            const uint32_t off =
+                (gy < a.out_h && gx < a.out_w) ? (uint32_t)((gy * a.out_w + gx) * 32 + 16 * (g >> 1)) : FM_OOB;
+            const v4u32_t q = {x[0], y[0], x[1], y[1]};
+            __builtin_amdgcn_raw_buffer_store_b128(q, ors, (IC2_FM3_ABL & 64) ? FM_OOB : off, 0, 0);
+          }
+          return;
+        }
+#pragma unroll
+        for (int i = 0; i < OCW; ++i) {
+          const int gy = gy0 + i;
+          const uint32_t off = (gy < a.out_h && gx < a.out_w) ? (uint32_t)((gy * a.out_w + gx) * 32 + 8 * g) : FM_OOB;
+          __builtin_amdgcn_raw_buffer_store_b64(__builtin_bit_cast(v2u32_t, v[i]), ors, (IC2_FM3_ABL & 64) ? FM_OOB : off,
+                                                0, 0);
+        }
+        return;
+      }
       const int gy = 16 * (t0 + tt) + li;
 #pragma unroll
       for (int i = 0; i < OCW; ++i) {
@@ -936,13 +994,13 @@
         const bool st = (MODE == 1 && k >= 3) || (FM3_DEFER_ST && MODE == 2 && k >= 4);
         const int nd = FM3_EARLY && dma ? my_dma : 0;
         if (nd == 0) {
-          if (st) asm volatile("s_waitcnt vmcnt(%0)" ::"n"(OCW) : "memory");
+          if (st) asm volatile("s_waitcnt vmcnt(%0)" ::"n"(NST) : "memory");
           else asm volatile("s_waitcnt vmcnt(0)" ::: "memory");
         } else if (nd == 1) {
-          if (st) asm volatile("s_waitcnt vmcnt(%0)" ::"n"(OCW + 1) : "memory");
+          if (st) asm volatile("s_waitcnt vmcnt(%0)" ::"n"(NST + 1) : "memory");
           else asm volatile("s_waitcnt vmcnt(1)" ::: "memory");
         } else {
-          if (st) asm volatile("s_waitcnt vmcnt(%0)" ::"n"(OCW + 2) : "memory");
+          if (st) asm volatile("s_waitcnt vmcnt(%0)" ::"n"(NST + 2) : "memory");
           else asm volatile("s_waitcnt vmcnt(2)" ::: "memory");
         }
       }
@@ -952,7 +1010,7 @@
         fm_s4 da[OCW];
 #pragma unroll
         for (int i = 0; i < OCW; ++i)
-          da[i] = fm_tr_read(d_img + (4 * g + tq) * G2::D_PITCH + (wave + NW * i) * G2::D_XP + 2 * tp);
+          da[i] = fm_tr_read(d_img + (4 * g + tq) * G2::D_PITCH + (BLK ? 4 * wave + i : wave + NW * i) * G2::D_XP + 2 * tp);
         __builtin_amdgcn_sched_barrier(0);
         if constexpr (MODE == 0) {
 #pragma unroll
@@ -987,7 +1045,7 @@
   }
 }
 
-template <int U, int DELTA, bool CL>
+template <int U, int DELTA, bool CL, bool BLK>
 static void fm3_launch_cl(FlrArgs a, int n, hipStream_t s) {
   constexpr int TOX = 32, NW = 8;
   a.tiles_x = (int)ceil_div(a.out_w, TOX);
@@ -998,7 +1056,7 @@
     int dev = 0, cus = 0, per_cu = 0;
     (void)hipGetDevice(&dev);
     (void)hipDeviceGetAttribute(&cus, hipDeviceAttributeMultiprocessorCount, dev);
-    (void)hipOccupancyMaxActiveBlocksPerMultiprocessor(&per_cu, flrelu_mfma3_kernel<U, DELTA, NW, CL>, 64 * NW, 0);
+    (void)hipOccupancyMaxActiveBlocksPerMultiprocessor(&per_cu, flrelu_mfma3_kernel<U, DELTA, NW, CL, BLK>, 64 * NW, 0);
     resident = (cus > 0 ? cus : 256) * (per_cu > 0 ? per_cu : 1);
   }
   static const int segs_mode = knob("IC2_FLR_SEGS", 1);
@@ -1008,7 +1066,7 @@
   nseg = (int)ceil_div(a.tiles_y, seg_len);
   const int nitems = (int)(nstrips * nseg);
   const int grid = nitems < resident ? nitems : resident;
-  hipLaunchKernelGGL((flrelu_mfma3_kernel<U, DELTA, NW, CL>), dim3((unsigned)grid), dim3(64 * NW), 0, s, a, nitems,
+  hipLaunchKernelGGL((flrelu_mfma3_kernel<U, DELTA, NW, CL, BLK>), dim3((unsigned)grid), dim3(64 * NW), 0, s, a, nitems,
                      nseg, seg_len);
 }
 
@@ -1034,18 +1092,23 @@
 }
 
 template <int U, int DELTA>
-static void fm2_launch(FlrArgs a, int n, hipStream_t s) {
+static int fm2_launch(FlrArgs a, int n, hipStream_t s) {
   static const bool split = knob("IC2_FLR_CLSPLIT", 1) != 0;
   static const bool strip = knob("IC2_FLR_STRIP", 1) != 0;
   const bool cl = split && a.lim >= 0.0625f && a.lim <= 4096.f;
-  if (strip) {
-    if (cl) fm3_launch_cl<U, DELTA, true>(a, n, s);
-    else fm3_launch_cl<U, DELTA, false>(a, n, s);
+  if (a.out_blocked) {
+    if (!strip) return IC2_E_UNSUPPORTED;
+    if (cl) fm3_launch_cl<U, DELTA, true, true>(a, n, s);
+    else fm3_launch_cl<U, DELTA, false, true>(a, n, s);
+  } else if (strip) {
+    if (cl) fm3_launch_cl<U, DELTA, true, false>(a, n, s);
+    else fm3_launch_cl<U, DELTA, false, false>(a, n, s);
   } else if (cl) {
     fm2_launch_cl<U, DELTA, true, 0>(a, n, s);
   } else {
     fm2_launch_cl<U, DELTA, false, 0>(a, n, s);
   }
+  return IC2_OK;
 }
 
 template <int U, int DELTA, bool IN_F16, bool ALIAS, int NW>
@@ -1094,19 +1157,15 @@
   static const bool wide_all = knob("IC2_FLR_WIDE_ALL", 1) != 0;
   if (in_f16 && wide && (wide_all || ceil_div(a.out_w, 32) * 32 <= ceil_div(a.out_w, 16) * 16) &&
       (int64_t)n * ceil_div(a.out_h, 16) * ceil_div(a.out_w, 32) * (a.c_p / 16) < (1LL << 31)) {
-    if (up == 2) {
-      if (delta == 0) fm2_launch<2, 0>(a, n, s);
-      else fm2_launch<2, 1>(a, n, s);
-    } else {
-      switch (delta) {
-        case 0: fm2_launch<4, 0>(a, n, s); break;
-        case 1: fm2_launch<4, 1>(a, n, s); break;
-        case 2: fm2_launch<4, 2>(a, n, s); break;
-        default: fm2_launch<4, 3>(a, n, s); break;
-      }
-    }
-    return IC2_OK;
-  }
+    if (up == 2) return delta == 0 ? fm2_launch<2, 0>(a, n, s) : fm2_launch<2, 1>(a, n, s);
+    switch (delta) {
+      case 0: return fm2_launch<4, 0>(a, n, s);
+      case 1: return fm2_launch<4, 1>(a, n, s);
+      case 2: return fm2_launch<4, 2>(a, n, s);
+      default: return fm2_launch<4, 3>(a, n, s);
+    }
+  }
+  if (a.out_blocked) return IC2_E_UNSUPPORTED;
   a.tiles_x = (int)ceil_div(a.out_w, 16);
   a.tiles_y = (int)ceil_div(a.out_h, 16);
   a.cblocks = a.c_p / 16;
diff --git a/image_compression_2_amd/csrc/igemm.hip b/image_compression_2_amd/csrc/igemm.hip
--- a/image_compression_2_amd/csrc/igemm.hip
+++ b/image_compression_2_amd/csrc/igemm.hip
@@ -577,9 +577,9 @@
     const int hy = hp / G::HW, hx = hp - (hp / G::HW) * G::HW;
     const int iy = oy0 - a.pad + hy, ix = ox0 - a.pad + hx;
     const bool ok = g < G::NHI && hp < G::NH && (unsigned)iy < (unsigned)a.h && (unsigned)ix < (unsigned)a.w_;
-    h_off[k] = ok ? (uint32_t)((((nn * a.h + iy) * a.w_ + ix) * a.x_pix + ((pch ^ (((hp >> 2) & 1) << 1)) << 3)) * 2)
-                  : kOob;
-  }
+    h_off[k] = ok ? ig_halo_off(a, nn, iy, ix, pch ^ (((hp >> 2) & 1) << 1)) : kOob;
+  }
+  const int x_cb = 2 * a.x_plane;
   int brow[J];
 #pragma unroll
   for (int j = 0; j < J; ++j) {
@@ -619,7 +619,7 @@
   };
   auto issue_hb = [&](int cb) {
     const __amdgpu_buffer_rsrc_t rs =
-        __builtin_amdgcn_make_buffer_rsrc((void*)(xg + (int64_t)ig_xb32(a, cb) * 64), 0, kOob, kRsrcWord3);
+        __builtin_amdgcn_make_buffer_rsrc((void*)(xg + (int64_t)ig_xb32(a, cb) * x_cb), 0, kOob, kRsrcWord3);
 #pragma unroll
     for (int k = 0; k < HPW; ++k) {
       char* dst = wid + 4 * k < G::NHI ? hal + (cb & 1) * G::HALO_B + (wid + 4 * k) * 1024 : hal + 2 * G::HALO_B;
@@ -628,7 +628,7 @@
   };
   auto issue_h1 = [&](int cb, int k) {
     const __amdgpu_buffer_rsrc_t rs =
-        __builtin_amdgcn_make_buffer_rsrc((void*)(xg + (int64_t)ig_xb32(a, cb) * 64), 0, kOob, kRsrcWord3);
+        __builtin_amdgcn_make_buffer_rsrc((void*)(xg + (int64_t)ig_xb32(a, cb) * x_cb), 0, kOob, kRsrcWord3);
     __builtin_amdgcn_raw_ptr_buffer_load_lds(
         rs, (__attribute__((address_space(3))) void*)(hal + (cb & 1) * G::HALO_B + (wid + 4 * k) * 1024), 16, h_off[k],
         0, 0, 0);
@@ -1267,7 +1267,9 @@
   float* yo = reinterpret_cast<float*>(a.y);
   const int stride = gridDim.x * (256 / L);
   for (int p = tid / L; p < a.M; p += stride) {
-    const uint4* src = reinterpret_cast<const uint4*>(xg + (int64_t)p * a.cin_p + sub * 16);
+    const uint4* src = reinterpret_cast<const uint4*>(
+        a.x_pix == 16 ? xg + (int64_t)(p / hw) * a.x_img + ((int64_t)sub * hw + p % hw) * 16
+                               : xg + (int64_t)p * a.cin_p + sub * 16);
     const uint4 u0 = src[0], u1 = src[1];
     const uint32_t w32[8] = {u0.x, u0.y, u0.z, u0.w, u1.x, u1.y, u1.z, u1.w};
     float acc[CV];
@@ -1423,6 +1425,10 @@
   return buf;
 }
 
+static bool conv_kind_reads_blocked(ConvKind kind, int dtype) {
+  return (kind == CK_HG4 || kind == CK_TORGB) && (dtype == IC2_BF16 || dtype == IC2_F16);
+}
+
 static int conv_chunk_n(int dtype, int n, int h, int w_, int cin_p) {
   const int64_t per_img = (int64_t)h * w_ * x_pix_of(dtype, cin_p) * (dtype == IC2_F32 ? 4 : 2);
   if ((int64_t)n * per_img < (int64_t)kOob || per_img >= (int64_t)kOob) return n;
@@ -1448,6 +1454,19 @@
   return f16_name;
 }
 
+extern "C" int ic2_conv_accepts_nhwc16(int dtype, int out_dtype, int out_layout, int n, int h, int w_, int cin_p,
+                                       int cout_p, int cout_valid, int kh, int kw, int pad) {
+  static const bool on_wino = knob("IC2_ACT_BLOCKED_WINO", 1) != 0, on_hg4 = knob("IC2_ACT_BLOCKED_HG4", 1) != 0,
+                    on_torgb = knob("IC2_ACT_BLOCKED_TORGB", 0) != 0;
+  const int ho = h + 2 * pad - kh + 1, wo = w_ + 2 * pad - kw + 1;
+  if (n <= 0 || ho <= 0 || wo <= 0 || cin_p <= 0 || cin_p % 32 || cout_p <= 0 || cout_p % 32) return 0;
+  if (ic2_conv_wino_preferred(dtype, n, h, w_, cin_p, cout_p, kh, kw, pad)) return on_wino;
+  const int nc = conv_chunk_n(dtype, n, h, w_, cin_p);
+  const ConvChoice c = conv_choice(dtype, out_layout, out_dtype, nc, h, w_, cin_p, cout_p, cout_valid, kh, kw, pad);
+  if (!conv_kind_reads_blocked(c.kind, dtype)) return 0;
+  return c.kind == CK_HG4 ? on_hg4 : on_torgb;
+}
+
 extern "C" int64_t ic2_conv_igemm_ws_bytes(int dtype, int n, int h, int w_, int cin_p, int cout_p, int kh, int kw,
                                            int pad) {
   const int ho = h + 2 * pad - kh + 1, wo = w_ + 2 * pad - kw + 1;
@@ -1464,6 +1483,11 @@
                                  float clamp, float out_mul, int out_layout, void* workspace, int64_t ws_bytes,
                                  void* stream) {
   IC2_CHECK_ARG(x && w && y, "conv_igemm: null pointer");
+  const int act_flags = act, in_layout = IC2_ACT_IN_LAYOUT_OF(act_flags);
+  act = IC2_ACT_OF(act_flags);
+  IC2_CHECK_ARG(in_layout == IC2_LAYOUT_NHWC || in_layout == IC2_LAYOUT_NHWC16, "conv_igemm: bad input layout %d",
+                in_layout);
+  const bool in_blocked = in_layout == IC2_LAYOUT_NHWC16;
   IC2_CHECK_ARG(dtype == IC2_F32 || dtype == IC2_BF16 || dtype == IC2_F16 || dtype == IC2_BF16X3 || dtype == IC2_F16X2,
                 "conv_igemm: bad dtype %d", dtype);
   IC2_CHECK_ARG(dtype != IC2_BF16X3 || (cin_p % 96 == 0 && out_layout == IC2_LAYOUT_NHWC),
@@ -1493,8 +1517,8 @@
       const int rc = ic2_conv_igemm_ws(reinterpret_cast<const char*>(x) + n0 * x_img, w,
                                        reinterpret_cast<char*>(y) + n0 * y_img, dtype, out_dtype, nn, h, w_, cin_p,
                                        cout_p, cout_valid, kh, kw, pad, ho, wo,
-                                       oscale ? oscale + (int64_t)n0 * cout_p : nullptr, bias, act, slope, act_gain,
-                                       clamp, out_mul, out_layout, workspace, ws_bytes, stream);
+                                       oscale ? oscale + (int64_t)n0 * cout_p : nullptr, bias, act_flags, slope,
+                                       act_gain, clamp, out_mul, out_layout, workspace, ws_bytes, stream);
       if (rc != IC2_OK) return rc;
     }
     return IC2_OK;
@@ -1514,6 +1538,7 @@
   a.in_gn = nullptr; a.in_slope = 0.f;
   a.x_pix = x_pix_of(dtype, cin_p);
   a.x_hb32 = x_hb32_of(dtype, cin_p);
+  ig_set_input_layout(a, in_blocked);
   const int kdt = dtype == IC2_BF16X3 ? IC2_BF16 : dtype == IC2_F16X2 ? IC2_F16 : dtype;
   static const int group = [] {
     const int g = knob("IC2_IGEMM_GROUP", 1);
@@ -1525,6 +1550,10 @@
   a.o_base = 0;
   hipStream_t s = as_stream(stream);
   ConvChoice c = conv_choice(dtype, out_layout, out_dtype, n, h, w_, cin_p, cout_p, cout_valid, kh, kw, pad);
+  IC2_CHECK_ARG(!in_blocked || conv_kind_reads_blocked(c.kind, dtype),
+                "conv_igemm: channel-blocked (NHWC16) input is read by the hg4 halo kernels and ToRGB only, with plain "
+                "bf16 / f16 operands; this geometry runs as %s (ic2_conv_accepts_nhwc16 says which do)",
+                conv_choice_name(c, dtype, n, ho, wo, cin_p, cout_p));
   dtype = kdt;
   IgPlan& pl = c.pl;
   if (pl.splits > 1 && (workspace == nullptr || ws_bytes < (int64_t)pl.splits * M * cout_p * 4)) pl.splits = 1;
@@ -1637,6 +1666,7 @@
     a.in_gn = nullptr; a.in_slope = 0.f;
     a.x_pix = x_pix_of(dtype, cin_p);
     a.x_hb32 = x_hb32_of(dtype, cin_p);
+    ig_set_input_layout(a, false);
     const bool f16 = dtype == IC2_F16X2;
     const int nc = conv_chunk_n(dtype, n, h, w_, cin_p);
     const int64_t ntile = ceil_div(wo, 32) * ceil_div(ho, x3_gn_th(cout_p));
@@ -1683,6 +1713,7 @@
   a.o_base = 0;
   a.in_gn = in_gn; a.in_slope = in_slope;
   a.x_pix = cin_p; a.x_hb32 = 0;
+  ig_set_input_layout(a, false);
   if (fuse) {
     if (cin_p == 32 && cout_p == 32) launch_hconv<32, 32, true>(a, s);
     else if (cin_p == 32) launch_hconv<32, 64, true>(a, s);
diff --git a/image_compression_2_amd/csrc/wino.hip b/image_compression_2_amd/csrc/wino.hip
--- a/image_compression_2_amd/csrc/wino.hip
+++ b/image_compression_2_amd/csrc/wino.hip
@@ -90,8 +90,7 @@
     const int line = l / hp, idx = l - line * hp;
     const int iy = oy0 - a.pad + (line >> 1), ix = 2 * px0 - a.pad + 2 * idx + (line & 1);
     const bool ok = l < a.wx_nh && (unsigned)iy < (unsigned)a.h && (unsigned)ix < (unsigned)a.w_;
-    h_off[k] = ok ? (uint32_t)((((nn * a.h + iy) * a.w_ + ix) * a.cin_p + ((pch ^ (((idx >> 2) & 1) << 1)) << 3)) * 2)
-                  : kOob;
+    h_off[k] = ok ? ig_halo_off(a, nn, iy, ix, pch ^ (((idx >> 2) & 1) << 1)) : kOob;
   }
   int boff[2][3];
   const int ns = a.wx_ns;
@@ -108,6 +107,7 @@
   const int ky_step = 2 * hp * 64;
   const int aoff = wx_off(fr, fh) + half * 2 * 64 * 64;
   const int CB = a.cin_p >> 5;
+  const int x_cb = 2 * a.x_plane;
 
   auto issue_hs = [&](int cb, int j) {
     const __amdgpu_buffer_rsrc_t rs = __builtin_amdgcn_make_buffer_rsrc(
@@ -120,7 +120,7 @@
   };
   auto issue_hp = [&](int cb, int k) {
     const __amdgpu_buffer_rsrc_t rs =
-        __builtin_amdgcn_make_buffer_rsrc((void*)(xg + (int64_t)cb * 64), 0, cb < CB ? kOob : 0, kRsrcWord3);
+        __builtin_amdgcn_make_buffer_rsrc((void*)(xg + (int64_t)cb * x_cb), 0, cb < CB ? kOob : 0, kRsrcWord3);
     __builtin_amdgcn_raw_ptr_buffer_load_lds(
         rs, (__attribute__((address_space(3))) void*)(hal + (cb & 1) * WX_HALO + (wid + WX_NW * k) * 1024), 16,
         h_off[k], 0, 0, 0);
@@ -479,6 +479,11 @@
                              int out_layout, void* stream) {
   IC2_CHECK_ARG(x && u && y, "conv_wino: null pointer");
   IC2_CHECK_ARG(dtype == IC2_F16, "conv_wino: f16 operands only (dtype %d)", dtype);
+  const int act_flags = act, in_layout = IC2_ACT_IN_LAYOUT_OF(act_flags);
+  act = IC2_ACT_OF(act_flags);
+  IC2_CHECK_ARG(in_layout == IC2_LAYOUT_NHWC || in_layout == IC2_LAYOUT_NHWC16, "conv_wino: bad input layout %d",
+                in_layout);
+  const bool in_blocked = in_layout == IC2_LAYOUT_NHWC16;
   IC2_CHECK_ARG(out_dtype == IC2_F32 || out_dtype == IC2_BF16 ||
                     ((out_dtype == IC2_F16 || out_dtype == IC2_F16_IEEE) && out_layout != IC2_LAYOUT_NCHW),
                 "conv_wino: bad out dtype %d", out_dtype);
@@ -501,8 +506,8 @@
       const int nn = n - n0 < nc ? n - n0 : nc;
       const int rc = ic2_conv_wino(reinterpret_cast<const char*>(x) + n0 * x_img, u,
                                    reinterpret_cast<char*>(y) + n0 * y_img, dtype, out_dtype, nn, h, w_, cin_p, cout_p,
-                                   cout_valid, pad, ho, wo, oscale ? oscale + (int64_t)n0 * cout_p : nullptr, bias, act,
-                                   slope, act_gain, clamp, out_mul, out_layout, stream);
+                                   cout_valid, pad, ho, wo, oscale ? oscale + (int64_t)n0 * cout_p : nullptr, bias,
+                                   act_flags, slope, act_gain, clamp, out_mul, out_layout, stream);
       if (rc != IC2_OK) return rc;
     }
     return IC2_OK;
@@ -527,6 +532,7 @@
   a.out_layout = out_layout; a.out_dtype = out_dtype; a.out_ieee = out_ieee;
   a.gn_part = nullptr; a.gn_groups = 0; a.gn_c = 0; a.in_gn = nullptr; a.in_slope = 0.f;
   a.x_pix = cin_p; a.x_hb32 = 0;
+  ig_set_input_layout(a, in_blocked);
   a.wx_twp = t.twp; a.wx_th = t.th; a.wx_ns = t.ns; a.wx_hp = t.hp; a.wx_nh = t.nh; a.wx_tx = t.tx; a.wx_ty = t.ty;
   hipLaunchKernelGGL(wino_fx_f16_kernel, dim3((unsigned)t.blocks), dim3(64 * WX_NW), 0, as_stream(stream), a);
   IC2_CHECK_LAUNCH("conv_wino");
diff --git a/image_compression_2_amd/networks_stylegan3.py b/image_compression_2_amd/networks_stylegan3.py
--- a/image_compression_2_amd/networks_stylegan3.py
+++ b/image_compression_2_amd/networks_stylegan3.py
@@ -13,6 +13,7 @@
 from . import sg3_ops
 
 _FLR_BLOCKED = nv.knob("IC2_FLR_BLOCKED", 1) != 0
+_ACT_BLOCKED = nv.knob("IC2_ACT_BLOCKED", 1) != 0
 _MOD_BATCH_MAX = 512
 
 
@@ -318,7 +319,23 @@
                 rec.ctypes.data_as(ctypes.c_void_p), nv.stream_of(ws))
         return xs, os_
 
-    def run_nhwc(self, x, n, dt, oscale, post_scale, final_scale=None):
+    def takes_blocked_input(self, n, dt):
+        if not _ACT_BLOCKED or dt not in (torch.bfloat16, torch.float16):
+            return False
+        s_in, k = int(self.in_size[0]), self.conv_kernel
+        if self.is_torgb:
+            out_dt, layout = nv.F32, nv.NCHW
+        else:
+            out_dt, layout = nv.F16, (nv.NHWC16 if _FLR_BLOCKED else nv.NHWC)
+        return nv.conv_accepts_nhwc16(nv.dtype_code(dt), out_dt, layout, n, s_in, s_in, self.cin_p, self.cout_p,
+                                      self.out_channels, k, k, k - 1)
+
+    def writes_blocked_output(self, dt):
+        return (not self.is_torgb and dt in (torch.bfloat16, torch.float16) and self.up_factor in (2, 4)
+                and self.down_factor == 2 and self._fu is not None and self._fd is not None
+                and self._fu.shape[0] == 6 * self.up_factor and self._fd.shape[0] == 12)
+
+    def run_nhwc(self, x, n, dt, oscale, post_scale, final_scale=None, x_blocked=False, out_blocked=False):
         s_in = int(self.in_size[0])
         k = self.conv_kernel
         pad = k - 1
@@ -326,19 +343,20 @@
         wp, _, bp = self.packed(dt)
         stream = nv.stream_of(x)
         nv.note_flops(2 * n * conv * conv * self.out_channels * self.in_channels * k * k)
+        in_flag = nv.act_in_layout(nv.NHWC16) if x_blocked else 0
         if self.is_torgb:
             assert self.up_factor == 1 and self.down_factor == 1 and self.padding == [0, 0, 0, 0]
             out = torch.empty([n, self.out_channels, conv, conv], dtype=torch.float32, device=x.device)
             clamp = float(self.conv_clamp) if self.conv_clamp is not None else -1.0
             nv.conv_igemm(nv.ptr(x), nv.ptr(wp), nv.ptr(out), nv.dtype_code(dt), nv.F32, n, s_in, s_in, self.cin_p,
                           self.cout_p, self.out_channels, k, k, pad, conv, conv, nv.ptr(oscale), nv.ptr(bp),
-                          nv.ACT_LRELU, 1.0, 1.0, clamp, float(1.0 if final_scale is None else final_scale), nv.NCHW,
-                          stream, x.device)
+                          nv.ACT_LRELU | in_flag, 1.0, 1.0, clamp,
+                          float(1.0 if final_scale is None else final_scale), nv.NCHW, stream, x.device)
             return out
-        y, blocked = self.conv_nhwc(x, n, dt, oscale)
-        return self.flrelu_nhwc(y, dt, post_scale, blocked=blocked)
-
-    def conv_nhwc(self, x, n, dt, oscale):
+        y, blocked = self.conv_nhwc(x, n, dt, oscale, x_blocked=x_blocked)
+        return self.flrelu_nhwc(y, dt, post_scale, blocked=blocked, out_blocked=out_blocked)
+
+    def conv_nhwc(self, x, n, dt, oscale, x_blocked=False):
         s_in = int(self.in_size[0])
         k = self.conv_kernel
         pad = k - 1
@@ -352,14 +370,15 @@
         else:
             y = torch.empty([n, conv, conv, self.cout_p], dtype=ydt, device=x.device)
         layout = nv.NHWC16 if blocked else nv.NHWC
+        in_flag = nv.act_in_layout(nv.NHWC16) if x_blocked else 0
         if nv.wino_preferred(nv.dtype_code(dt), n, s_in, s_in, self.cin_p, self.cout_p, k, k, pad):
             nv.conv_wino(nv.ptr(x), nv.ptr(self.packed_wino()), nv.ptr(y), nv.F16, nv.dtype_code(ydt), n, s_in, s_in,
-                         self.cin_p, self.cout_p, self.out_channels, pad, conv, conv, nv.ptr(oscale), nv.ptr(bp), 0,
-                         0.0, 1.0, -1.0, 1.0, layout, stream)
+                         self.cin_p, self.cout_p, self.out_channels, pad, conv, conv, nv.ptr(oscale), nv.ptr(bp),
+                         in_flag, 0.0, 1.0, -1.0, 1.0, layout, stream)
         else:
             nv.conv_igemm(nv.ptr(x), nv.ptr(wp), nv.ptr(y), nv.dtype_code(dt), nv.dtype_code(ydt), n, s_in, s_in,
                           self.cin_p, self.cout_p, self.out_channels, k, k, pad, conv, conv, nv.ptr(oscale),
-                          nv.ptr(bp), 0, 0.0, 1.0, -1.0, 1.0, layout, stream, x.device)
+                          nv.ptr(bp), in_flag, 0.0, 1.0, -1.0, 1.0, layout, stream, x.device)
         return y, blocked
 
     def packed_wino(self):
@@ -374,16 +393,19 @@
         self._cache["wino"] = (key, u)
         return u
 
-    def flrelu_nhwc(self, y, dt_out, post_scale=None, blocked=False):
+    def flrelu_nhwc(self, y, dt_out, post_scale=None, blocked=False, out_blocked=False):
         n, conv = y.shape[0], y.shape[2 if blocked else 1]
         s_out = int(self.out_size[0])
-        out = torch.empty([n, s_out, s_out, self.cout_p], dtype=dt_out, device=y.device)
+        if out_blocked:
+            out = torch.empty([n, self.cout_p // 16, s_out, s_out, 16], dtype=dt_out, device=y.device)
+        else:
+            out = torch.empty([n, s_out, s_out, self.cout_p], dtype=dt_out, device=y.device)
         fu = self._fu
         fd = self._fd
         px0, px1, py0, py1 = self.padding
         clamp = float(self.conv_clamp) if self.conv_clamp is not None else -1.0
         nv.call("ic2_flrelu_nhwc16" if blocked else "ic2_flrelu_nhwc", nv.ptr(y), nv.ptr(out), nv.dtype_code(y.dtype),
-                nv.dtype_code(dt_out), n,
+                nv.dtype_code(dt_out) | (nv.flr_out_layout(nv.NHWC16) if out_blocked else 0), n,
                 self.cout_p, conv, conv, s_out, s_out, None if fu is None else fu.ctypes.data_as(ctypes.c_void_p),
                 1 if fu is None else fu.shape[0], None if fd is None else fd.ctypes.data_as(ctypes.c_void_p),
                 1 if fd is None else fd.shape[0], None, self.up_factor, self.down_factor, px0, px1, py0, py1,
@@ -572,9 +594,14 @@
         layers = self.layers()
         sc = self.scales_batched(ws, ldx, n, dt)
         x = self.input.run_nhwc(ws, ldx, n, dt, sc[0][0])
+        x_blocked = False
         for i, L in enumerate(layers):
             post = sc[i + 1][0] if i + 1 < len(layers) else None
-            x = L.run_nhwc(x, n, dt, sc[i][1], post, final_scale=self.output_scale if L.is_torgb else None)
+            out_blocked = (i + 1 < len(layers) and L.writes_blocked_output(dt)
+                           and layers[i + 1].takes_blocked_input(n, dt))
+            x = L.run_nhwc(x, n, dt, sc[i][1], post, final_scale=self.output_scale if L.is_torgb else None,
+                           x_blocked=x_blocked, out_blocked=out_blocked)
+            x_blocked = out_blocked
         return _refuse(self, x, ws_in)
 
     def scales_batched(self, ws, ldx, n, dt):
diff --git a/include/ic2ops.h b/include/ic2ops.h
--- a/include/ic2ops.h
+++ b/include/ic2ops.h
@@ -13,6 +13,12 @@
        IC2_F16_IEEE = 5 };
 enum { IC2_ACT_LINEAR = 0, IC2_ACT_LRELU = 1 };
 enum { IC2_LAYOUT_NHWC = 0, IC2_LAYOUT_NCHW = 1, IC2_LAYOUT_NHWC16 = 2 };
+#define IC2_ACT_IN_LAYOUT(layout) ((layout) << 4)
+#define IC2_ACT_IN_LAYOUT_OF(v) (((v) >> 4) & 15)
+#define IC2_ACT_OF(v) ((v) & 15)
+#define IC2_FLR_OUT_LAYOUT(layout) ((layout) << 4)
+#define IC2_FLR_OUT_LAYOUT_OF(v) (((v) >> 4) & 15)
+#define IC2_FLR_DTYPE_OF(v) ((v) & 15)
 
 const char* ic2_last_error(void);
 int ic2_abi_version(void);
@@ -79,6 +85,9 @@
 
 const char* ic2_conv_plan(int dtype, int out_dtype, int out_layout, int n, int h, int w, int cin_p, int cout_p,
                           int cout_valid, int kh, int kw, int pad);
+
+int ic2_conv_accepts_nhwc16(int dtype, int out_dtype, int out_layout, int n, int h, int w, int cin_p, int cout_p,
+                            int cout_valid, int kh, int kw, int pad);
 
 int ic2_dev_mode(void);
 
```

Measured after the change: 1541 images/s, median of 6. +1.5%, better.
